# AKASH2907/pi-consistency-activity-detection

Measured on AMD Instinct MI355X. Metric: train clips/sec (bs=8, 16×224×224, I3D+caps+bv cons) at 1/2/4/8 GPU, higher is better.
Workload: dtype f32 (fp32 operands and fp32 accumulation everywhere; 33 of the 79 conv / input-gradient launches and the 3x3x3 / 1x1x1 weight gradients multiply on the bf16 matrix cores: every fp32 operand as the exact sum of 3 bf16 terms, 6 products on v_mfma_f32_32x32x16_bf16, hi / lo fp32 accumulators -- error v

## Files before the change

include/picons.h:

```cpp
#ifndef PICONS_H
#define PICONS_H
#include <stdint.h>
#ifdef __cplusplus
extern "C" {
#endif

typedef void* pc_stream;

#define PC_OK            0
#define PC_E_ARG        -1
#define PC_E_LAUNCH     -2
#define PC_E_NODEVICE   -3

#define PC_ACT_NONE 0
#define PC_ACT_RELU 1
#define PC_ACT_SIGMOID 2

#define PC_F_ACCUM   1
#define PC_F_BIAS    2
#define PC_F_CSCALE  4
#define PC_F_BNPART  8
#define PC_F_NFAST   16
#define PC_F_TOUT    32
#define PC_F_CI3     64

#define PC_F_STRIPS  256
#define PC_F_X6      128

#define PC_VERSION 103
int         pc_version(void);
const char* pc_last_error(void);

typedef struct pc_conv_desc {
    int32_t N;
    int32_t Ti, Hi, Wi, Ci, ldi;
    int32_t Tq, Hq, Wq;
    int32_t To, Ho, Wo, Co, ldo;
    int32_t ostr[3], ooff[3];
    int32_t istr[3], ntap[3], ioff0[3], istep[3];
    int32_t wk0[3], wkstep[3];
    int32_t KT, KH, KW, ldw;
    int32_t act, flags;
    int32_t wgstride, bgstride;
    int32_t act_c0;
    int32_t groups;
} pc_conv_desc;

int pc_conv_fwd(const pc_conv_desc* d, const float* in, const float* w, const float* bias,
                const float* cscale, float* out, float* bnpart, pc_stream s);
int pc_conv_bnpart_rows(const pc_conv_desc* d);

int pc_conv_fwd_x6(const pc_conv_desc* d, const float* in, const uint16_t* wplanes, int64_t plane_stride, const float* bias,
                   const float* cscale, float* out, float* bnpart, pc_stream s);
int64_t pc_conv_x6_ws_floats(const pc_conv_desc* d);
int pc_conv_fwd_x6_ws(const pc_conv_desc* d, const float* in, const uint16_t* wplanes, int64_t plane_stride, const float* bias,
                      const float* cscale, float* out, float* bnpart, float* ws, int64_t ws_floats, pc_stream s);
int pc_conv_x6_ok(const pc_conv_desc* d);
int pc_split_planes(const float* src, uint16_t* planes, int64_t n, int64_t plane_stride, pc_stream s);
typedef struct pc_split_job {
    uint64_t src, planes;
    int64_t  n, plane_stride;
} pc_split_job;
int pc_split_planes_multi(const pc_split_job* jobs, int njobs, pc_stream s);
int pc_conv_work(const pc_conv_desc* d, int ci_real, int co_real, double* out);
int pc_conv_variant(const pc_conv_desc* d, int64_t ws_floats, char* buf, int cap);

typedef struct pc_wino_desc {
    int32_t N, T, H, W;
    int32_t Ci, ldi, Co, ldo;
    int32_t KT;
    int32_t act, flags;
    int32_t Ti;
    int32_t ta, tc, tden;
    int32_t m;
} pc_wino_desc;
int64_t pc_wino_u_floats(int O, int I, int KT);
int pc_wino_weights(const float* w, int64_t sO, int64_t sT, int64_t sI, int O, int I, int KT, int flip, float* U, pc_stream s);
int pc_wino_conv(const pc_wino_desc* d, const float* in, const float* U, const float* bias, float* out, float* bnpart, pc_stream s);
int64_t pc_wino4_u_floats(int O, int I, int KT);
int pc_wino4_weights(const float* w, int64_t sO, int64_t sT, int64_t sI, int O, int I, int KT, int flip, float* U, pc_stream s);
int pc_wino_bnpart_rows(const pc_wino_desc* d);
int pc_wino_work(const pc_wino_desc* d, double* out);
int pc_wino_variant(const pc_wino_desc* d, const float* out, char* buf, int cap);

typedef struct pc_wgrad_desc {
    int32_t N;
    int32_t Tq, Hq, Wq, Cd, ldd;
    int32_t Ts, Hs, Ws, Cs, lds;
    int32_t istr[3], ntap[3], ioff0[3], istep[3];
    int32_t wk0[3];
    int32_t KT, KH, KW;
    int32_t splitk;
    int32_t nbatch;
    int32_t dbstride, sbstride, gbstride;
    int32_t Td, Hd, Wd, doff[3];
    int32_t flags;
    int32_t ws_slices;
} pc_wgrad_desc;
#define PC_WG_CS3    1
#define PC_WG_X6     2
int pc_conv_wgrad(const pc_wgrad_desc* d, const float* D, const float* S, float* g, pc_stream s);
int pc_wgrad_slices(const pc_wgrad_desc* d);
int pc_wgrad_variant(const pc_wgrad_desc* d, char* buf, int cap);
int pc_wgrad_fold_group(void);
int pc_wgrad_fold(float* ws, int64_t image_floats, int nslices, pc_stream s);
int pc_wgrad_work(const pc_wgrad_desc* d, int cd_real, int cs_real, double* out);
int pc_wgrad_uses_x6(const pc_wgrad_desc* d);
typedef struct pc_wgrad_job {
    pc_wgrad_desc d;
    const float* D; const float* S; float* g;
} pc_wgrad_job;
int pc_conv_wgrad_multi(const pc_wgrad_job* jobs, int njobs, pc_stream s);

int pc_bn_finalize(const float* part, int nparts_per_group, int groups, int C, int64_t count_per_group,
                   const float* gamma, const float* beta, float eps, float momentum,
                   float* running_mean, float* running_var, float* stat, pc_stream s);
int64_t pc_bn_finalize_ws_floats(int nparts_per_group, int groups, int C);
int pc_bn_finalize_ws(const float* part, int nparts_per_group, int groups, int C, int64_t count_per_group,
                      const float* gamma, const float* beta, float eps, float momentum,
                      float* running_mean, float* running_var, float* stat, float* ws, pc_stream s);
int pc_bn_apply(const float* z, int ldz, const float* stat, int C, int64_t rows, int groups, float* y,
                int ldy, int relu, pc_stream s);
int pc_bn_finalize_apply_ok(int nparts_per_group, int C);
int pc_bn_finalize_apply(const float* part, int nparts_per_group, int groups, int C, int64_t count_per_group, const float* gamma, const float* beta,
                         float eps, float momentum, float* running_mean, float* running_var, float* stat, const float* z, int ldz, int64_t rows,
                         float* y, int ldy, int relu, pc_stream s);
int pc_bn_eval_stat(const float* gamma, const float* beta, const float* running_mean,
                    const float* running_var, float eps, int C, float* stat, pc_stream s);
int64_t pc_bn_bwd_ws_floats(int64_t rows, int C, int groups);
int pc_bn_bwd(const float* dy, int lddy, const float* z, int ldz, const float* stat, int C,
              int64_t rows, int groups, int relu, float* dz, int lddz, float* dgamma, float* dbeta,
              int accum, float* ws, pc_stream s);

typedef struct pc_pool_desc {
    int32_t N, Ti, Hi, Wi, C, ldi;
    int32_t To, Ho, Wo, ldo;
    int32_t k[3], s[3], padf[3];
} pc_pool_desc;
int pc_maxpool_fwd(const pc_pool_desc* d, const float* x, float* y, uint8_t* argmax, pc_stream s);
int pc_maxpool_bwd(const pc_pool_desc* d, const float* dy, const uint8_t* argmax, float* dx,
                   int accum, pc_stream s);

int pc_channel_scale(const float* x, int ldx, const float* scale, int N, int64_t pos_per_n, int C,
                     float* y, int ldy, int accum, pc_stream s);
int64_t pc_act_bwd_ws_floats(int64_t rows, int C);
int pc_act_bwd(const float* dy, int lddy, const float* y, int ldy, int act, int C, int64_t rows,
               float* dz, int lddz, float* dbias, int accum, float* ws, pc_stream s);
int pc_ncdhw_to_ndhwc(const void* src, int src_is_f64, int N, int C, int64_t thw, int W, int Cpad,
                      int flipw, float* dst, pc_stream s);
int pc_ndhwc_to_ncdhw(const float* src, int ld, int N, int C, int64_t thw, float* dst, pc_stream s);
int pc_transpose_batched(const float* src, int batch, int R, int Cc, int64_t src_batch_stride,
                         int src_ld, float* dst, int64_t dst_batch_stride, int dst_ld, int accum,
                         pc_stream s);
typedef struct pc_transpose_job {
    uint64_t src, dst;
    int64_t  src_batch_stride, dst_batch_stride;
    int32_t  batch, R, C, src_ld, dst_ld, accum;
    int32_t  nslices, reserved;
    int64_t  slice_stride;
} pc_transpose_job;
int pc_transpose_multi(const pc_transpose_job* jobs, int njobs, pc_stream s);
int pc_col2im(const float* cols, int N, int Ho, int Wo, int KH, int KW, int C, float* dx, int lddx,
              int accum, pc_stream s);
// ... 42 lines not shown
                     float* db4, float* dWp, float* dbp, int accum, float* ws, pc_stream s);

typedef struct pc_loss_desc {
    int32_t B, T, H, W;
    int32_t bv, gv, n_frames, predict_maps, jhmdb;
    float   lower_thresh, upper_thresh;
    float   bv_wt, gv_wt, wt_loc, wt_cons, wt_ramp;
} pc_loss_desc;
int64_t pc_loss_ws_floats(const pc_loss_desc* d);
int pc_consistency_loss(const pc_loss_desc* d, const float* output, const float* flip_op,
                        const float* seg, const int32_t* labeled, float* scalars, float* d_output,
                        float* d_flip_op, float* mask_bv, float* mask_gv, float* ws, pc_stream s);
int pc_var_mask(const float* pred, const float* flip_pred, int B, int T, int H, int W, int n_frames,
                int use_sig, float* mask, float* ws, pc_stream s);
int pc_grad_mask(const float* pred, int B, int T, int H, int W, float lower, float upper,
                 float* mask, float* ws, pc_stream s);
int pc_spread_loss(const float* x, const float* cls, const int32_t* labeled, int Bn, int C, float m,
                   float wt, float* out, float* dx, pc_stream s);

int pc_adam_step(float* p, const float* g, float* m, float* v, int64_t n, float lr, float b1,
                 float b2, float eps, int step, float gscale, pc_stream s);

typedef struct pc_axis_desc {
    int32_t R, I, O, C;
    int32_t in_split, out_split, act, act_c0, accum;
    int32_t in_sr, in_hi, in_lo, out_sr, out_hi, out_lo;
} pc_axis_desc;
int pc_axis_linear(const pc_axis_desc* d, const float* in, const float* M, const float* bias, float* out, pc_stream s);
int pc_wspec_fwd(const float* in, const float* tw, int A, int B, int KY, int KX, int U, int Ur, float* out, pc_stream s);
int pc_wspec_bwd(const float* dV, const float* tw, int A, int B, int KY, int KX, int U, int Ur, float* kg, pc_stream s);

int pc_wspec_master_fwd(const float* w, const float* tw, int Acnt, int a0, int Atot, int B, int KY, int KX, int U, int Ur,
                        float* out_f, float* out_t, pc_stream s);
int pc_wspec_master_planes(const float* w, const float* tw, int Acnt, int a0, int Atot, int B, int KY, int KX, int U, int Ur,
                           uint16_t* out_f, uint16_t* out_t, int64_t plane_stride, pc_stream s);
int pc_wspec_master_bwd(const float* dV, const float* tw, int Acnt, int a0, int Atot, int B, int KY, int KX, int U, int Ur,
                        float* dw, int accum, pc_stream s);

int pc_tail6_weights(const float* wf, int N, int Ci, float* W5f, float* W5t, pc_stream s);
int pc_tail6_gather(const float* cols, const float* bc, const float* bsm, int N, int It, int Ih, int Iw, float* out, pc_stream s);
int pc_tail6_scatter(const float* dout, int N, int It, int Ih, int Iw, float* dcols, pc_stream s);
int pc_tail6_wgrad_map(const float* dW5, int N, int Ci, float* Gc, pc_stream s);
int pc_tail6_wgrad_map_slices(float* ws, const int32_t* nslices8, int N, int Ci, float* Gc, pc_stream s);
int pc_tail6_bias_sums(const float* dout, int N, int It, int Ih, int Iw, float* sums, pc_stream s);
int64_t pc_tail6_bias_sums_ws_floats(int N, int It, int Ih, int Iw);
int pc_tail6_bias_sums_ws(const float* dout, int N, int It, int Ih, int Iw, float* sums, float* ws, pc_stream s);

typedef struct pc_op {
    int32_t  kind;
    int32_t  i[48];
    float    f[8];
    int32_t  lane;
    uint64_t p[12];
    int64_t  l[4];
} pc_op;
enum {
    PC_OP_CONV = 1, PC_OP_WGRAD, PC_OP_BN_FINALIZE, PC_OP_BN_APPLY, PC_OP_BN_EVAL_STAT, PC_OP_BN_BWD,
    PC_OP_POOL_FWD, PC_OP_POOL_BWD, PC_OP_CHSCALE, PC_OP_ACT_BWD, PC_OP_TO_NDHWC, PC_OP_TO_NCDHW,
    PC_OP_TRANSPOSE, PC_OP_FILL, PC_OP_AXPY, PC_OP_EM_FWD, PC_OP_EM_BWD, PC_OP_CMASK_FWD,
    PC_OP_CMASK_BWD, PC_OP_TAPSUM_FWD, PC_OP_TAPSUM_BWD, PC_OP_LOSS, PC_OP_SPREAD, PC_OP_ADAM,
    PC_OP_TAIL_COMBINE, PC_OP_TAIL_COLSUM, PC_OP_TAIL_GRADS, PC_OP_COL2IM,
    PC_OP_AXIS,
    PC_OP_WSPEC_FWD,
    PC_OP_WSPEC_BWD,
    PC_OP_WSPEC_MASTER_FWD,
    PC_OP_WSPEC_MASTER_BWD,
    PC_OP_TAIL6_WEIGHTS,
    PC_OP_TAIL6_GATHER,
    PC_OP_TAIL6_SCATTER,
    PC_OP_TAIL6_WGRAD_MAP,
    PC_OP_TAIL6_BIAS_SUMS,
    PC_OP_TRANSPOSE_MULTI,
    PC_OP_FORK,
    PC_OP_JOIN,
    PC_OP_WGRAD_MULTI,
    PC_OP_WINO_CONV,
    PC_OP_WINO_WEIGHTS,
    PC_OP_CONV_X6,
    PC_OP_SPLIT_PLANES,
    PC_OP_SPLIT_PLANES_MULTI,
    PC_OP_WSPEC_MASTER_PLANES,
    PC_OP_BN_FIN_APPLY,
    PC_OP_WGRAD_FOLD,
    PC_OP__COUNT
};
#define PC_MAX_LANES 8
int pc_run_ops(const pc_op* ops, int n, pc_stream s);
int pc_run_ops_lanes(const pc_op* ops, int n, const pc_stream* lanes, int nlanes);
int pc_streams_fanin(pc_stream target, const pc_stream* lanes, int nlanes);
int pc_release_thread_events(void);
int pc_run_ops_timed(const pc_op* ops, int n, int kind, float* ms, int* count, const pc_stream* lanes, int nlanes);
int pc_run_ops_timed_collect(float* ms, int* count);

#ifdef __cplusplus
}
#endif
#endif
```

pi-consistency-activity-detection_amd/capi.py:

```python
import ctypes as C
import os

import numpy as np

_HERE = os.path.dirname(os.path.abspath(__file__))
DIAG = os.environ.get("PICONS_DIAG_LIB", "0") not in ("", "0")
DIAG_SWITCHES = ("PICONS_CONV_ABLATE", "PICONS_WGRAD_ABLATE", "PICONS_WINO_VARIANT")
LIB_PATH = os.path.join(_HERE, "libpicons_diag.so" if DIAG else "libpicons.so")
if os.environ.get("PICONS_LIB_NAME"):
    LIB_PATH = os.path.join(_HERE, os.path.basename(os.environ["PICONS_LIB_NAME"]))
_lib = None

i32, i64, f32, vp = C.c_int32, C.c_int64, C.c_float, C.c_void_p


class ConvDesc(C.Structure):
    _fields_ = [(n, i32) for n in ("N", "Ti", "Hi", "Wi", "Ci", "ldi", "Tq", "Hq", "Wq", "To", "Ho", "Wo", "Co", "ldo")] + \
               [(n, i32 * 3) for n in ("ostr", "ooff", "istr", "ntap", "ioff0", "istep", "wk0", "wkstep")] + \
               [(n, i32) for n in ("KT", "KH", "KW", "ldw", "act", "flags", "wgstride", "bgstride", "act_c0", "groups")]


class WgradDesc(C.Structure):
    _fields_ = [(n, i32) for n in ("N", "Tq", "Hq", "Wq", "Cd", "ldd", "Ts", "Hs", "Ws", "Cs", "lds")] + \
               [(n, i32 * 3) for n in ("istr", "ntap", "ioff0", "istep", "wk0")] + [(n, i32) for n in ("KT", "KH", "KW", "splitk", "nbatch", "dbstride", "sbstride", "gbstride", "Td", "Hd", "Wd")] + [("doff", i32 * 3), ("flags", i32), ("ws_slices", i32)]


AXIS_FIELDS = ["R", "I", "O", "C", "in_split", "out_split", "act", "act_c0", "accum", "in_sr", "in_hi", "in_lo", "out_sr", "out_hi", "out_lo"]


class WinoDesc(C.Structure):
    _fields_ = [(n, i32) for n in ("N", "T", "H", "W", "Ci", "ldi", "Co", "ldo", "KT", "act", "flags", "Ti", "ta", "tc", "tden", "m")]


class AxisDesc(C.Structure):
    _fields_ = [(n, i32) for n in AXIS_FIELDS]


class PoolDesc(C.Structure):
    _fields_ = [(n, i32) for n in ("N", "Ti", "Hi", "Wi", "C", "ldi", "To", "Ho", "Wo", "ldo")] + \
               [(n, i32 * 3) for n in ("k", "s", "padf")]


class LossDesc(C.Structure):
    _fields_ = [(n, i32) for n in ("B", "T", "H", "W", "bv", "gv", "n_frames", "predict_maps", "jhmdb")] + \
               [(n, f32) for n in ("lower_thresh", "upper_thresh", "bv_wt", "gv_wt", "wt_loc", "wt_cons", "wt_ramp")]


OP_DTYPE = np.dtype([("kind", np.int32), ("i", np.int32, 48), ("f", np.float32, 8), ("lane", np.int32),
                     ("p", np.uint64, 12), ("l", np.int64, 4)], align=False)

(OP_CONV, OP_WGRAD, OP_BN_FINALIZE, OP_BN_APPLY, OP_BN_EVAL_STAT, OP_BN_BWD, OP_POOL_FWD, OP_POOL_BWD, OP_CHSCALE,
 OP_ACT_BWD, OP_TO_NDHWC, OP_TO_NCDHW, OP_TRANSPOSE, OP_FILL, OP_AXPY, OP_EM_FWD, OP_EM_BWD, OP_CMASK_FWD, OP_CMASK_BWD,
 OP_TAPSUM_FWD, OP_TAPSUM_BWD, OP_LOSS, OP_SPREAD, OP_ADAM, OP_TAIL_COMBINE, OP_TAIL_COLSUM, OP_TAIL_GRADS, OP_COL2IM,
 OP_AXIS, OP_WSPEC_FWD, OP_WSPEC_BWD, OP_WSPEC_MASTER_FWD, OP_WSPEC_MASTER_BWD, OP_TAIL6_WEIGHTS, OP_TAIL6_GATHER, OP_TAIL6_SCATTER, OP_TAIL6_WGRAD_MAP, OP_TAIL6_BIAS_SUMS,
 OP_TRANSPOSE_MULTI, OP_FORK, OP_JOIN, OP_WGRAD_MULTI, OP_WINO_CONV, OP_WINO_WEIGHTS, OP_CONV_X6, OP_SPLIT_PLANES, OP_SPLIT_PLANES_MULTI, OP_WSPEC_MASTER_PLANES, OP_BN_FIN_APPLY, OP_WGRAD_FOLD) = range(1, 51)
MAX_LANES = 8

WJOB_DTYPE = np.dtype([("d", np.int32, 42), ("D", np.uint64), ("S", np.uint64), ("g", np.uint64)], align=False)

TJOB_DTYPE = np.dtype([("src", np.uint64), ("dst", np.uint64), ("sbs", np.int64), ("dbs", np.int64), ("batch", np.int32), ("R", np.int32),
                       ("C", np.int32), ("sld", np.int32), ("dld", np.int32), ("accum", np.int32), ("nslices", np.int32), ("reserved", np.int32),
                       ("sst", np.int64)], align=False)

SJOB_DTYPE = np.dtype([("src", np.uint64), ("planes", np.uint64), ("n", np.int64), ("pstride", np.int64)], align=False)

ACT_NONE, ACT_RELU, ACT_SIGMOID = 0, 1, 2
F_ACCUM, F_BIAS, F_CSCALE, F_BNPART, F_NFAST, F_TOUT, F_CI3, F_X6, F_STRIPS = 1, 2, 4, 8, 16, 32, 64, 128, 256
WG_CS3, WG_X6 = 1, 2

ABI_VERSION = 103

_SIGS = {
    "pc_version": (i32, []),
    "pc_last_error": (C.c_char_p, []),
    "pc_conv_fwd": (i32, [C.POINTER(ConvDesc), vp, vp, vp, vp, vp, vp, vp]),
    "pc_conv_bnpart_rows": (i32, [C.POINTER(ConvDesc)]),
    "pc_conv_fwd_x6": (i32, [C.POINTER(ConvDesc), vp, vp, i64, vp, vp, vp, vp, vp]),
    "pc_conv_fwd_x6_ws": (i32, [C.POINTER(ConvDesc), vp, vp, i64, vp, vp, vp, vp, vp, i64, vp]),
    "pc_conv_x6_ws_floats": (i64, [C.POINTER(ConvDesc)]),
    "pc_conv_x6_ok": (i32, [C.POINTER(ConvDesc)]),
    "pc_split_planes": (i32, [vp, vp, i64, i64, vp]),
    "pc_split_planes_multi": (i32, [vp, i32, vp]),
    "pc_conv_work": (i32, [C.POINTER(ConvDesc), i32, i32, C.POINTER(C.c_double)]),
    "pc_conv_variant": (i32, [C.POINTER(ConvDesc), i64, C.c_char_p, i32]),
    "pc_wino_variant": (i32, [C.POINTER(WinoDesc), vp, C.c_char_p, i32]),
    "pc_wgrad_variant": (i32, [C.POINTER(WgradDesc), C.c_char_p, i32]),
    "pc_conv_wgrad": (i32, [C.POINTER(WgradDesc), vp, vp, vp, vp]),
    "pc_conv_wgrad_multi": (i32, [vp, i32, vp]),
    "pc_wgrad_slices": (i32, [C.POINTER(WgradDesc)]),
    "pc_wgrad_uses_x6": (i32, [C.POINTER(WgradDesc)]),
    "pc_wgrad_fold_group": (i32, []),
    "pc_wgrad_fold": (i32, [vp, i64, i32, vp]),
    "pc_wgrad_work": (i32, [C.POINTER(WgradDesc), i32, i32, C.POINTER(C.c_double)]),
    "pc_wino_u_floats": (i64, [i32, i32, i32]),
    "pc_wino_weights": (i32, [vp, i64, i64, i64, i32, i32, i32, i32, vp, vp]),
    "pc_wino_conv": (i32, [C.POINTER(WinoDesc), vp, vp, vp, vp, vp, vp]),
    "pc_wino4_u_floats": (i64, [i32, i32, i32]),
    "pc_wino4_weights": (i32, [vp, i64, i64, i64, i32, i32, i32, i32, vp, vp]),
    "pc_wino_bnpart_rows": (i32, [C.POINTER(WinoDesc)]),
    "pc_wino_work": (i32, [C.POINTER(WinoDesc), C.POINTER(C.c_double)]),
    "pc_bn_finalize": (i32, [vp, i32, i32, i32, i64, vp, vp, f32, f32, vp, vp, vp, vp]),
    "pc_bn_finalize_ws": (i32, [vp, i32, i32, i32, i64, vp, vp, f32, f32, vp, vp, vp, vp, vp]),
    "pc_bn_finalize_ws_floats": (i64, [i32, i32, i32]),
    "pc_bn_finalize_apply_ok": (i32, [i32, i32]),
    "pc_bn_finalize_apply": (i32, [vp, i32, i32, i32, i64, vp, vp, f32, f32, vp, vp, vp, vp, i32, i64, vp, i32, i32, vp]),
    "pc_bn_apply": (i32, [vp, i32, vp, i32, i64, i32, vp, i32, i32, vp]),
    "pc_bn_eval_stat": (i32, [vp, vp, vp, vp, f32, i32, vp, vp]),
    "pc_bn_bwd_ws_floats": (i64, [i64, i32, i32]),
    "pc_bn_bwd": (i32, [vp, i32, vp, i32, vp, i32, i64, i32, i32, vp, i32, vp, vp, i32, vp, vp]),
    "pc_maxpool_fwd": (i32, [C.POINTER(PoolDesc), vp, vp, vp, vp]),
    "pc_maxpool_bwd": (i32, [C.POINTER(PoolDesc), vp, vp, vp, i32, vp]),
    "pc_channel_scale": (i32, [vp, i32, vp, i32, i64, i32, vp, i32, i32, vp]),
    "pc_act_bwd_ws_floats": (i64, [i64, i32]),
    "pc_act_bwd": (i32, [vp, i32, vp, i32, i32, i32, i64, vp, i32, vp, i32, vp, vp]),
    "pc_ncdhw_to_ndhwc": (i32, [vp, i32, i32, i32, i64, i32, i32, i32, vp, vp]),
    "pc_ndhwc_to_ncdhw": (i32, [vp, i32, i32, i32, i64, vp, vp]),
    "pc_transpose_batched": (i32, [vp, i32, i32, i32, i64, i32, vp, i64, i32, i32, vp]),
    "pc_col2im": (i32, [vp, i32, i32, i32, i32, i32, i32, vp, i32, i32, vp]),
    "pc_seg_frame_counts": (i32, [vp, vp, i64, i64, vp, vp]),
    "pc_map_accumulate": (i32, [vp, i64, i32, i32, vp, vp, vp, vp, vp]),
    "pc_clip_from_u8": (i32, [vp, i32, i32, i32, C.POINTER(C.c_int32), i32, i32, i32, vp, i32, vp, vp, vp, vp]),
    "pc_clip_from_u8_ndhwc4": (i32, [vp, i32, i32, i32, C.POINTER(C.c_int32), i32, i32, i32, vp, i32, vp, vp, vp, vp]),
    "pc_clip_from_u8_masks": (i32, [vp, i32, i32, i32, C.POINTER(C.c_int32), i32, i32, i32, vp, C.POINTER(C.c_int32), vp, vp, vp, vp, vp]),
    "pc_resize_tables": (i64, [i32, i32, i32, i32, i32, vp, i64]),
    "pc_resize_u8": (i32, [vp, i32, i32, i32, i32, i32, i32, vp, i32, vp, vp]),
    "pc_fill": (i32, [vp, i64, f32, vp]),
    "pc_axpy": (i32, [vp, vp, i64, f32, vp]),
    "pc_em_ws_floats": (i64, [i32, i32, i32]),
    "pc_em_state_floats": (i64, [i32]),
    "pc_em_routing_fwd": (i32, [vp, vp, vp, vp, i32, i32, i32, vp, vp, vp]),
    "pc_em_routing_bwd": (i32, [vp, vp, vp, vp, vp, i32, i32, i32, vp, vp, vp, vp, vp, vp, vp]),
    "pc_class_mask_fwd": (i32, [vp, i32, i32, i32, vp, vp, i32, vp, vp, vp, vp]),
    "pc_class_mask_bwd": (i32, [vp, vp, vp, i32, i32, i32, vp, vp]),
    "pc_tapsum_fwd": (i32, [vp, i32, i32, i32, i32, vp, vp, vp]),
    "pc_tapsum_bwd": (i32, [vp, i32, i32, i32, i32, vp, vp]),
    "pc_loss_ws_floats": (i64, [C.POINTER(LossDesc)]),
    "pc_consistency_loss": (i32, [C.POINTER(LossDesc), vp, vp, vp, vp, vp, vp, vp, vp, vp, vp, vp]),
    "pc_var_mask": (i32, [vp, vp, i32, i32, i32, i32, i32, i32, vp, vp, vp]),
    "pc_grad_mask": (i32, [vp, i32, i32, i32, i32, f32, f32, vp, vp, vp]),
    "pc_spread_loss": (i32, [vp, vp, vp, i32, i32, f32, f32, vp, vp, vp]),
    "pc_adam_step": (i32, [vp, vp, vp, vp, i64, f32, f32, f32, f32, i32, f32, vp]),
    "pc_tail_combine": (i32, [vp, vp, vp, vp, i32, i32, i32, i32, i32, vp, vp, vp, vp]),
    "pc_tail_colsum": (i32, [vp, i32, i64, vp, vp]),
    "pc_tail_grads": (i32, [vp, vp, vp, vp, vp, vp, i32, i32, i32, i32, i32, i32, vp, vp, vp, vp, i32, vp]),
    "pc_tail_grads_ws_floats": (i64, [i32, i32, i32]),
    "pc_tail_grads_ws": (i32, [vp, vp, vp, vp, vp, vp, i32, i32, i32, i32, i32, i32, vp, vp, vp, vp, i32, vp, vp]),
    "pc_axis_linear": (i32, [vp, vp, vp, vp, vp, vp]),
    "pc_wspec_fwd": (i32, [vp, vp, i32, i32, i32, i32, i32, i32, vp, vp]),
    "pc_wspec_bwd": (i32, [vp, vp, i32, i32, i32, i32, i32, i32, vp, vp]),
    "pc_wspec_master_fwd": (i32, [vp, vp, i32, i32, i32, i32, i32, i32, i32, i32, vp, vp, vp]),
    "pc_wspec_master_planes": (i32, [vp, vp, i32, i32, i32, i32, i32, i32, i32, i32, vp, vp, i64, vp]),
    "pc_wspec_master_bwd": (i32, [vp, vp, i32, i32, i32, i32, i32, i32, i32, i32, vp, i32, vp]),
    "pc_tail6_weights": (i32, [vp, i32, i32, vp, vp, vp]),
    "pc_tail6_gather": (i32, [vp, vp, vp, i32, i32, i32, i32, vp, vp]),
    "pc_tail6_scatter": (i32, [vp, i32, i32, i32, i32, vp, vp]),
    "pc_tail6_wgrad_map": (i32, [vp, i32, i32, vp, vp]),
    "pc_tail6_bias_sums": (i32, [vp, i32, i32, i32, i32, vp, vp]),
    "pc_tail6_wgrad_map_slices": (i32, [vp, vp, i32, i32, vp, vp]),
    "pc_tail6_bias_sums_ws_floats": (i64, [i32, i32, i32, i32]),
    "pc_tail6_bias_sums_ws": (i32, [vp, i32, i32, i32, i32, vp, vp, vp]),
    "pc_transpose_multi": (i32, [vp, i32, vp]),
    "pc_run_ops": (i32, [vp, i32, vp]),
    "pc_run_ops_lanes": (i32, [vp, i32, vp, i32]),
    "pc_streams_fanin": (i32, [vp, vp, i32]),
    "pc_release_thread_events": (i32, []),
    "pc_run_ops_timed": (i32, [vp, i32, i32, C.POINTER(f32), C.POINTER(i32), vp, i32]),
    "pc_run_ops_timed_collect": (i32, [C.POINTER(f32), C.POINTER(i32)]),
}
EXPORTS = sorted(_SIGS)


def lib():
    global _lib
    if _lib is None:
        stray = [k for k in DIAG_SWITCHES if os.environ.get(k, "0") not in ("", "0")]
        if stray and not DIAG:
            raise RuntimeError("%s set, but these switches exist only in the diagnostic build of the library (results can be wrong by design): "
                               "`make -C pi-consistency-activity-detection_amd/csrc diag` and PICONS_DIAG_LIB=1, or unset them" % ", ".join(stray))
        if not os.path.exists(LIB_PATH):
            raise RuntimeError("libpicons.so not built (%s): run `python -c 'import __graft_entry__ as g; g.build()'` "
                               "or `make -C pi-consistency-activity-detection_amd/csrc`; there is no CPU fallback" % LIB_PATH)
        L = C.CDLL(LIB_PATH)
        for name, (res, args) in _SIGS.items():
            fn = getattr(L, name)
            fn.restype = res
            fn.argtypes = args
        if L.pc_version() != ABI_VERSION:
            raise RuntimeError("libpicons.so is ABI version %d, this package mirrors include/picons.h version %d: rebuild it "
                               "(`make -C pi-consistency-activity-detection_amd/csrc`)" % (L.pc_version(), ABI_VERSION))
        assert C.sizeof(ConvDesc) == 48 * 4 and OP_DTYPE.itemsize == 4 + 192 + 32 + 4 + 96 + 32
        assert C.sizeof(WgradDesc) == 168 and WJOB_DTYPE.itemsize == 192
        _lib = L
    return _lib


def check(rc):
    if rc != 0:
        raise RuntimeError("libpicons error %d: %s" % (rc, lib().pc_last_error().decode()))


def variant(name, desc, *args):
    buf = C.create_string_buffer(160)
    check(getattr(lib(), name)(desc, *args, buf, 160))
    return buf.value.decode()


def call(name, *args):
    check(getattr(lib(), name)(*args))
```

pi-consistency-activity-detection_amd/csrc/api.hip:

```cpp
#include "common.h"
#include <string.h>
#include <vector>

static thread_local char g_err[512] = "";

void pc_set_error(const char* fmt, ...) {
    va_list ap;
    va_start(ap, fmt);
    vsnprintf(g_err, sizeof(g_err), fmt, ap);
    va_end(ap);
}

extern "C" const char* pc_last_error(void) { return g_err; }
extern "C" int pc_version(void) { return PC_VERSION; }

extern "C" int pc_transpose_batched(const float*, int, int, int, int64_t, int, float*, int64_t, int, int, pc_stream);

#define P(T, k) ((T)(uintptr_t)op.p[k])

static int run_one(const pc_op& op, pc_stream s) {
    switch (op.kind) {
        case PC_OP_CONV: {
            pc_conv_desc d;
            memcpy(&d, op.i, sizeof(d));
// ... 61 lines not shown
            return pc_transpose_batched(P(const float*, 0), op.i[0], op.i[1], op.i[2], op.l[0], op.i[3], P(float*, 1), op.l[1], op.i[4], op.i[5], s);
        case PC_OP_FILL:
            return pc_fill(P(float*, 0), op.l[0], op.f[0], s);
        case PC_OP_AXPY:
            return pc_axpy(P(float*, 0), P(const float*, 1), op.l[0], op.f[0], s);
        case PC_OP_EM_FWD:
            return pc_em_routing_fwd(P(const float*, 0), P(const float*, 1), P(const float*, 2), P(const float*, 3), op.i[0], op.i[1], op.i[2], P(float*, 4), P(float*, 5), s);
        case PC_OP_EM_BWD:
            return pc_em_routing_bwd(P(const float*, 0), P(const float*, 1), P(const float*, 2), P(const float*, 3), P(const float*, 4), op.i[0], op.i[1],
                                     op.i[2], P(float*, 5), P(float*, 6), P(float*, 7), P(float*, 8), P(float*, 9), P(const float*, 10), s);
        case PC_OP_CMASK_FWD:
            return pc_class_mask_fwd(P(const float*, 0), op.i[0], op.i[1], op.i[2], P(const float*, 1), P(const int32_t*, 2), op.i[3], P(float*, 3),
                                     P(float*, 4), P(float*, 5), s);
        case PC_OP_CMASK_BWD:
            return pc_class_mask_bwd(P(const float*, 0), P(const float*, 1), P(const float*, 2), op.i[0], op.i[1], op.i[2], P(float*, 3), s);
        case PC_OP_TAPSUM_FWD:
            return pc_tapsum_fwd(P(const float*, 0), op.i[0], op.i[1], op.i[2], op.i[3], P(const float*, 1), P(float*, 2), s);
        case PC_OP_TAPSUM_BWD:
            return pc_tapsum_bwd(P(const float*, 0), op.i[0], op.i[1], op.i[2], op.i[3], P(float*, 1), s);
        case PC_OP_LOSS: {
            pc_loss_desc d;
            d.B = op.i[0]; d.T = op.i[1]; d.H = op.i[2]; d.W = op.i[3]; d.bv = op.i[4]; d.gv = op.i[5]; d.n_frames = op.i[6];
            d.predict_maps = op.i[7]; d.jhmdb = op.i[8];
            d.lower_thresh = op.f[0]; d.upper_thresh = op.f[1]; d.bv_wt = op.f[2]; d.gv_wt = op.f[3]; d.wt_loc = op.f[4];
            d.wt_cons = op.f[5]; d.wt_ramp = op.f[6];
            return pc_consistency_loss(&d, P(const float*, 0), P(const float*, 1), P(const float*, 2), P(const int32_t*, 3), P(float*, 4), P(float*, 5),
                                       P(float*, 6), P(float*, 7), P(float*, 8), P(float*, 9), s);
        }
        case PC_OP_SPREAD:
            return pc_spread_loss(P(const float*, 0), P(const float*, 1), P(const int32_t*, 2), op.i[0], op.i[1], op.f[0], op.f[1], P(float*, 3), P(float*, 4), s);
        case PC_OP_ADAM:
            return pc_adam_step(P(float*, 0), P(const float*, 1), P(float*, 2), P(float*, 3), op.l[0], op.f[0], op.f[1], op.f[2], op.f[3], op.i[0], op.f[4], s);
        case PC_OP_TAIL_COMBINE:
            return pc_tail_combine(P(const float*, 0), P(const float*, 1), P(const float*, 2), P(const float*, 3), op.i[0], op.i[1], op.i[2], op.i[3],
                                   op.i[4], P(float*, 4), P(float*, 5), P(float*, 6), s);
        case PC_OP_TAIL_COLSUM:
            return pc_tail_colsum(P(const float*, 0), op.i[0], op.l[0], P(float*, 1), s);
        case PC_OP_TAIL_GRADS:
            return pc_tail_grads_ws(P(const float*, 0), P(const float*, 1), P(const float*, 2), P(const float*, 3), P(const float*, 4), P(const float*, 5),
                                    op.i[0], op.i[1], op.i[2], op.i[3], op.i[4], op.i[5], P(float*, 6), P(float*, 7), P(float*, 8), P(float*, 9), op.i[6],
                                    P(float*, 10), s);
        case PC_OP_COL2IM:
            return pc_col2im(P(const float*, 0), op.i[0], op.i[1], op.i[2], op.i[3], op.i[4], op.i[5], P(float*, 1), op.i[6], op.i[7], s);
        case PC_OP_AXIS: {
            pc_axis_desc d;
            memcpy(&d, op.i, sizeof(d));
            return pc_axis_linear(&d, P(const float*, 0), P(const float*, 1), P(const float*, 2), P(float*, 3), s);
        }
        case PC_OP_WSPEC_FWD:
            return pc_wspec_fwd(P(const float*, 0), P(const float*, 1), op.i[0], op.i[1], op.i[2], op.i[3], op.i[4], op.i[5], P(float*, 2), s);
        case PC_OP_WSPEC_BWD:
            return pc_wspec_bwd(P(const float*, 0), P(const float*, 1), op.i[0], op.i[1], op.i[2], op.i[3], op.i[4], op.i[5], P(float*, 2), s);
        case PC_OP_WSPEC_MASTER_FWD:
            return pc_wspec_master_fwd(P(const float*, 0), P(const float*, 1), op.i[0], op.i[1], op.i[2], op.i[3], op.i[4], op.i[5], op.i[6], op.i[7],
                                       P(float*, 2), P(float*, 3), s);
        case PC_OP_WSPEC_MASTER_BWD:
            return pc_wspec_master_bwd(P(const float*, 0), P(const float*, 1), op.i[0], op.i[1], op.i[2], op.i[3], op.i[4], op.i[5], op.i[6], op.i[7],
                                       P(float*, 2), op.i[8], s);
        case PC_OP_TAIL6_WEIGHTS:
            return pc_tail6_weights(P(const float*, 0), op.i[0], op.i[1], P(float*, 1), P(float*, 2), s);
        case PC_OP_TAIL6_GATHER:
            return pc_tail6_gather(P(const float*, 0), P(const float*, 1), P(const float*, 2), op.i[0], op.i[1], op.i[2], op.i[3], P(float*, 3), s);
        case PC_OP_TAIL6_SCATTER:
            return pc_tail6_scatter(P(const float*, 0), op.i[0], op.i[1], op.i[2], op.i[3], P(float*, 1), s);
        case PC_OP_TAIL6_WGRAD_MAP:
            return op.i[2] ? pc_tail6_wgrad_map_slices(P(float*, 0), &op.i[3], op.i[0], op.i[1], P(float*, 1), s)
                           : pc_tail6_wgrad_map(P(const float*, 0), op.i[0], op.i[1], P(float*, 1), s);
        case PC_OP_TAIL6_BIAS_SUMS:
            return pc_tail6_bias_sums_ws(P(const float*, 0), op.i[0], op.i[1], op.i[2], op.i[3], P(float*, 1), P(float*, 2), s);
        case PC_OP_TRANSPOSE_MULTI:
            return pc_transpose_multi(P(const pc_transpose_job*, 0), op.i[0], s);
        case PC_OP_WGRAD_FOLD:
            return pc_wgrad_fold(P(float*, 0), op.l[0], op.i[0], s);
        case PC_OP_WGRAD_MULTI:
            return pc_conv_wgrad_multi(P(const pc_wgrad_job*, 0), op.i[0], s);
        case PC_OP_WINO_CONV: {
            pc_wino_desc d;
            memcpy(&d, op.i, sizeof(d));
            return pc_wino_conv(&d, P(const float*, 0), P(const float*, 1), P(const float*, 2), P(float*, 3), P(float*, 4), s);
        }
        case PC_OP_WINO_WEIGHTS:
            if (op.i[4] == 4) return pc_wino4_weights(P(const float*, 0), op.l[0], op.l[1], op.l[2], op.i[0], op.i[1], op.i[2], op.i[3], P(float*, 1), s);
            return pc_wino_weights(P(const float*, 0), op.l[0], op.l[1], op.l[2], op.i[0], op.i[1], op.i[2], op.i[3], P(float*, 1), s);
        default:
            pc_set_error("pc_run_ops: unknown op kind %d", op.kind);
            return PC_E_ARG;
    }
}

static thread_local hipEvent_t g_ev[PC_MAX_LANES];
static thread_local bool g_ev_init = false;

static thread_local std::vector<hipEvent_t> g_pending;
thread_local hipEvent_t pc_tl_ev_start = nullptr, pc_tl_ev_stop = nullptr;
static thread_local std::vector<hipEvent_t> g_ev_pool;
static hipEvent_t take_event() {
    if (!g_ev_pool.empty()) { hipEvent_t e = g_ev_pool.back(); g_ev_pool.pop_back(); return e; }
    hipEvent_t e = nullptr;
    (void)hipEventCreate(&e);
    return e;
}

static int run_list(const pc_op* ops, int n, const pc_stream* lanes, int nlanes, int kind, float* ms, int* count) {
    if (!ops && n > 0) { pc_set_error("pc_run_ops: null ops"); return PC_E_ARG; }
    if (nlanes < 1 || nlanes > PC_MAX_LANES || !lanes) { pc_set_error("pc_run_ops: nlanes=%d (1..%d)", nlanes, PC_MAX_LANES); return PC_E_ARG; }
    if (nlanes > 1 && !g_ev_init) {
        for (int i = 0; i < PC_MAX_LANES; ++i)
            if (hipEventCreateWithFlags(&g_ev[i], hipEventDisableTiming) != hipSuccess) { pc_set_error("hipEventCreate failed"); return PC_E_LAUNCH; }
        g_ev_init = true;
    }
    int cnt = 0;
    hipEvent_t* ev = nullptr;
    const int sub = kind > 0 ? kind >> 16 : 0;
    if (kind > 0) kind &= 0xffff;
    auto timed_op = [&](const pc_op& op) {
        if (kind <= 0 || op.kind != kind) return false;
        if (!sub || kind != PC_OP_WGRAD) return true;
        pc_wgrad_desc d;
        memcpy(&d, op.i, sizeof(d));
        const bool x6 = pc_wgrad_uses_x6(&d) != 0;
        return sub == 1 ? x6 : !x6;
    };
    if (kind > 0) {
        for (int k = 0; k < n; ++k) cnt += timed_op(ops[k]);
        ev = (hipEvent_t*)malloc(sizeof(hipEvent_t) * 2 * (cnt > 0 ? cnt : 1));
        for (int i = 0; i < 2 * cnt; ++i) ev[i] = take_event();
    }
    int j = 0, rc = PC_OK, k = 0;
    for (; k < n && rc == PC_OK; ++k) {
        const pc_op& op = ops[k];
        if (op.kind == PC_OP_FORK || op.kind == PC_OP_JOIN) {
            if (nlanes == 1) continue;
            const bool fork = op.kind == PC_OP_FORK;
            const int src = (fork && op.i[1] > 0 && op.i[1] < nlanes) ? op.i[1] : 0;
            hipError_t he = hipSuccess;
            if (fork) he = hipEventRecord(g_ev[src], (hipStream_t)lanes[src]);
            for (int q = 0; q < nlanes && he == hipSuccess; ++q) {
                if (!((op.i[0] >> q) & 1) || (fork && q == src) || (!fork && q == 0)) continue;
                if (fork) {
                    he = hipStreamWaitEvent((hipStream_t)lanes[q], g_ev[src], 0);
                } else {
                    he = hipEventRecord(g_ev[q], (hipStream_t)lanes[q]);
                    if (he == hipSuccess) he = hipStreamWaitEvent((hipStream_t)lanes[0], g_ev[q], 0);
                }
            }
            if (he != hipSuccess) { pc_set_error("%s: event record / wait failed: %s", fork ? "FORK" : "JOIN", hipGetErrorString(he)); rc = PC_E_LAUNCH; ++k; break; }
            continue;
        }
        const int ln = (op.lane > 0 && op.lane < nlanes) ? op.lane : 0;
        const pc_stream s = lanes[ln];
        const bool t = timed_op(op);
        const bool ext = t && (op.kind == PC_OP_CONV || op.kind == PC_OP_CONV_X6 || op.kind == PC_OP_WINO_CONV || op.kind == PC_OP_WGRAD);
        if (ext) { pc_tl_ev_start = ev[2 * j]; pc_tl_ev_stop = ev[2 * j + 1]; }
        else if (t) (void)hipEventRecord(ev[2 * j], (hipStream_t)s);
        rc = run_one(op, s);
        if (ext) { pc_tl_ev_start = pc_tl_ev_stop = nullptr; ++j; }
        else if (t) { (void)hipEventRecord(ev[2 * j + 1], (hipStream_t)s); ++j; }
    }
    if (rc != PC_OK) {
        char tmp[400];
        snprintf(tmp, sizeof(tmp), "%s", g_err);
        pc_set_error("op %d (kind %d): %s", k - 1, ops[k - 1].kind, tmp);
    }
    if (kind > 0 && !ms) {
        for (int i = 0; i < 2 * j; ++i) g_pending.push_back(ev[i]);
        for (int i = 2 * j; i < 2 * cnt; ++i) g_ev_pool.push_back(ev[i]);
// ... 73 lines not shown
```

pi-consistency-activity-detection_amd/csrc/conv_x6.hip:

```cpp
#include "conv_common.h"
#include <stdlib.h>
#include <type_traits>
#include <mutex>

namespace {

typedef __attribute__((ext_vector_type(8))) __bf16 bf16x8;
typedef __attribute__((ext_vector_type(4))) uint32_t u32x4;

__device__ __forceinline__ void split2(float x0, float x1, uint32_t& h, uint32_t& m, uint32_t& l) { x6_split2(x0, x1, h, m, l); }

__global__ __launch_bounds__(256) void split_planes_kernel(const float* __restrict__ src, uint16_t* __restrict__ dst, long long n, long long pstride) {
    for (long long i = ((long long)blockIdx.x * 256 + threadIdx.x) * 4; i < n; i += (long long)gridDim.x * 1024) {
        const f32x4 v = *(const f32x4*)(src + i);
        uint32_t h0, m0, l0, h1, m1, l1;
        split2(v[0], v[1], h0, m0, l0);
        split2(v[2], v[3], h1, m1, l1);
        *(uint2*)(dst + i) = make_uint2(h0, h1);
        *(uint2*)(dst + pstride + i) = make_uint2(m0, m1);
        *(uint2*)(dst + 2 * pstride + i) = make_uint2(l0, l1);
    }
}

constexpr int SP_JOBS = 48;
struct SplitJobK { const float* src; uint16_t* dst; long long n, pstride; };
struct SplitPack { SplitJobK j[SP_JOBS]; int first[SP_JOBS + 1]; int n; };
__global__ __launch_bounds__(256) void split_planes_multi_kernel(const SplitPack pk) {
    int k = 0;
    while (k + 1 < pk.n && (int)blockIdx.x >= pk.first[k + 1]) ++k;
    const SplitJobK& J = pk.j[k];
    const long long i = ((long long)(blockIdx.x - pk.first[k]) * 256 + threadIdx.x) * 4;
    if (i >= J.n) return;
    const f32x4 v = *(const f32x4*)(J.src + i);
    uint32_t h0, m0, l0, h1, m1, l1;
    split2(v[0], v[1], h0, m0, l0);
    split2(v[2], v[3], h1, m1, l1);
    *(uint2*)(J.dst + i) = make_uint2(h0, h1);
    *(uint2*)(J.dst + J.pstride + i) = make_uint2(m0, m1);
    *(uint2*)(J.dst + 2 * J.pstride + i) = make_uint2(l0, l1);
}

__device__ __forceinline__ dma_rsrc_t dma_rsrc_h(const uint16_t* base) {
    return __builtin_amdgcn_make_buffer_rsrc((void*)base, 0, (int)0xffffff00u, 0x00020000);
}
__device__ __forceinline__ void glds16h(dma_rsrc_t rs, unsigned voff, uint8_t* l) {
    __builtin_amdgcn_raw_ptr_buffer_load_lds(rs, (__attribute__((address_space(3))) void*)l, 16, voff, 0, 0, 0);
}

struct ConvX6 { ConvK k; const uint16_t* wp; long long wpstride; int full, rem, ksplit; float* ws; unsigned* ctr; int mfast; };

#define PC_MFX6(X, Y, Cc) Cc = __builtin_amdgcn_mfma_f32_32x32x16_bf16(__builtin_bit_cast(bf16x8, X), __builtin_bit_cast(bf16x8, Y), Cc, 0, 0, 0)

template <int BM, int BN, int WM, int WN>
__global__ __launch_bounds__(64 * WM * WN, 1) void conv_x6_kernel(const ConvX6 px) {
    const ConvK& p = px.k;
    constexpr int NW = WM * WN, NT = 64 * NW;
    constexpr int TM = BM / WM / 32, TN = BN / WN / 32, NM = 6 * TM * TN, NU = 4 * TM;
    static_assert(TM >= 1 && TN >= 1 && BM % (WM * 32) == 0 && BN % (WN * 32) == 0, "wave tiles");
    constexpr int APIECES = BM / 8, BPIECES = 3 * BN / 16;
    constexpr int AR = (APIECES + NW - 1) / NW, BR = (BPIECES + NW - 1) / NW;
    static_assert(APIECES % NW == 0, "A pieces per wave");
    constexpr int ABYTES = BM * BK * 4, BPLANE = BN * BK * 2, BBYTES = 3 * BPLANE;
    constexpr int OPBYTES = 2 * (ABYTES + BBYTES);
    constexpr int EH = (BM * BN * 4 <= OPBYTES) ? 1 : 2;
    static_assert(BM * BN * 4 / EH <= OPBYTES, "output tile fits the operand buffers");
    extern __shared__ __attribute__((aligned(16))) uint8_t smem8[];
    uint8_t* As0 = smem8;
    uint8_t* Bs0 = smem8 + 2 * ABYTES;
    int* rinfo = (int*)(smem8 + OPBYTES);
    int* rout = rinfo + BM * 4;
    unsigned* tile_or = (unsigned*)(rout + BM);

    const int tid = threadIdx.x, lane = tid & 63, wave = __builtin_amdgcn_readfirstlane(tid >> 6);
    const int wm = wave / WN, wn = wave % WN;
    int bid, ks = 0, tl = 0;
    const bool split = (int)blockIdx.x >= px.full;
    if (!split) bid = xcd_remap(blockIdx.x, px.full);
    else {
        const int q = xcd_remap((int)blockIdx.x - px.full, px.rem * px.ksplit);
        tl = q / px.ksplit; ks = q % px.ksplit;
        bid = px.full + tl;
    }
    int nt, g, lt;
    if (px.mfast) { lt = bid % p.mtiles_g; const int q = bid / p.mtiles_g; nt = q % p.ntiles; g = q / p.ntiles; }
    else { nt = bid % p.ntiles; const int mtl = bid / p.ntiles; g = mtl / p.mtiles_g; lt = mtl % p.mtiles_g; }
    const int n0 = nt * BN;
    const uint16_t* wbase = px.wp + (size_t)g * p.wgstride;
    const float* bbase = p.bias + (size_t)g * p.bgstride;
    if (tid == 0) *tile_or = 0u;

    for (int r = tid; r < BM; r += NT) {
        const int lm = lt * BM + r;
        int4 info = make_int4(-1, 0, 0, 0);
        int op = -1;
        if (lm < p.Mg) {
            int m = g * p.Mg + lm;
            int n = 0;
            if (p.flags & PC_F_NFAST) { const int ng = p.N / p.groups; n = g * ng + lm % ng; m = lm / ng; }
            const int wq = m % p.Wq; m /= p.Wq;
            const int hq = m % p.Hq; m /= p.Hq;
            const int tq = m % p.Tq;
            if (!(p.flags & PC_F_NFAST)) n = m / p.Tq;
            info = make_int4(n, tq * p.istr[0] + p.ioff0[0], hq * p.istr[1] + p.ioff0[1], wq * p.istr[2] + p.ioff0[2]);
            op = ((n * p.To + tq * p.ostr[0] + p.ooff[0]) * p.Ho + hq * p.ostr[1] + p.ooff[1]) * p.Wo + wq * p.ostr[2] + p.ooff[2];
        }
        ((int4*)rinfo)[r] = info;
        rout[r] = op;
    }
    __syncthreads();

    unsigned adma[AR], amask[AR], bdma[BR];
    const long long apos0 = ((long long)min(p.ioff0[0], 0) * p.Hi + min(p.ioff0[1], 0)) * p.Wi + min(p.ioff0[2], 0);
    const long long abias = -apos0 * p.ldi;
#pragma unroll
    for (int j = 0; j < AR; ++j) {
        const int row = (wave + NW * j) * 8 + (lane >> 3);
        const int4 ri = ((int4*)rinfo)[row];
        const int ks = ((lane & 7) ^ ((row >> 1) & 7)) * 4;
        unsigned m = 0;
        if (ri.x >= 0) {
            for (int a = 0; a < p.ntap[0]; ++a) m |= ((unsigned)(ri.y + a * p.istep[0]) < (unsigned)p.Ti ? 1u : 0u) << a;
            for (int a = 0; a < p.ntap[1]; ++a) m |= ((unsigned)(ri.z + a * p.istep[1]) < (unsigned)p.Hi ? 1u : 0u) << (10 + a);
            for (int a = 0; a < p.ntap[2]; ++a) m |= ((unsigned)(ri.w + a * p.istep[2]) < (unsigned)p.Wi ? 1u : 0u) << (20 + a);
        }
        amask[j] = m;
        const long long pos = ((long long)(ri.x * p.Ti + ri.y) * p.Hi + ri.z) * p.Wi + ri.w;
        adma[j] = (unsigned)(((pos - apos0) * p.ldi + ks) * 4);
    }
#pragma unroll
    for (int j = 0; j < BR; ++j) {
        const int pc = wave + NW * j, pl = pc / (BN / 16), q = pc % (BN / 16);
        const int row = q * 16 + (lane >> 2), co = n0 + row;
        const int sl = (lane & 3) ^ ((row >> 2) & 3);
        bdma[j] = (pc < BPIECES && co < p.Co) ? (unsigned)(((size_t)pl * px.wpstride + (size_t)co * p.wtaps * p.ldw + sl * 8) * 2) : DMA_OOB;
    }
    {
        unsigned mo = 0;
#pragma unroll
        for (int j = 0; j < AR; ++j) mo |= amask[j];
        atomicOr(tile_or, mo);
    }
    __syncthreads();
    const unsigned bo = __builtin_amdgcn_readfirstlane(*tile_or);
    const unsigned bt = bo & 0x3ffu, bh = (bo >> 10) & 0x3ffu, bw = (bo >> 20) & 0x3ffu;
    const bool any_tap = bt && bh && bw;
    const int a_lo = any_tap ? __builtin_ctz(bt) : 0, a_hi = any_tap ? 31 - __builtin_clz(bt) : -1;
    const int b_lo = any_tap ? __builtin_ctz(bh) : 0, b_hi = any_tap ? 31 - __builtin_clz(bh) : -1;
    const int c_lo = any_tap ? __builtin_ctz(bw) : 0, c_hi = any_tap ? 31 - __builtin_clz(bw) : -1;
    const int nb_ = b_hi - b_lo + 1, nc_ = c_hi - c_lo + 1;
    const int nchunks_tile = (a_hi - a_lo + 1) * nb_ * nc_ * (p.Ci / BK);
    struct Walk { int a, b, c, ci; };
    Walk wa = {a_lo, b_lo, c_lo, 0}, wb = wa;
    auto advance = [&](Walk& w) {
        w.ci += BK;
        if (w.ci >= p.Ci) { w.ci = 0; if (++w.c > c_hi) { w.c = c_lo; if (++w.b > b_hi) { w.b = b_lo; ++w.a; } } }
    };
    int nchunks = nchunks_tile;
    if (split) {
        const int c0 = (int)((long long)nchunks_tile * ks / px.ksplit), c1 = (int)((long long)nchunks_tile * (ks + 1) / px.ksplit);
        for (int i = 0; i < c0; ++i) advance(wa);
        wb = wa;
        nchunks = c1 - c0;
    }
    auto fetchA = [&](int buf) {
        const long long da = ((long long)(wa.a * p.istep[0] * p.Hi + wa.b * p.istep[1]) * p.Wi + wa.c * p.istep[2]) * p.ldi + wa.ci;
        const unsigned sel = (1u << wa.a) | (1u << (10 + wa.b)) | (1u << (20 + wa.c));
        const dma_rsrc_t ra = dma_rsrc(p.in + (da - abias));
#pragma unroll
        for (int j = 0; j < AR; ++j) glds16b(ra, ((amask[j] & sel) == sel) ? adma[j] : DMA_OOB, (float*)(As0 + buf * ABYTES + (wave + NW * j) * 1024));
        advance(wa);
    };
    auto fetchB = [&](int buf) {
        const int wtap = ((p.wk0[0] + wb.a * p.wkstep[0]) * p.KH + p.wk0[1] + wb.b * p.wkstep[1]) * p.KW + p.wk0[2] + wb.c * p.wkstep[2];
        const dma_rsrc_t rb = dma_rsrc_h(wbase + (long long)wtap * p.ldw + wb.ci);
#pragma unroll
        for (int j = 0; j < BR; ++j)
            if (BPIECES % NW == 0 || wave + NW * j < BPIECES) glds16h(rb, bdma[j], Bs0 + buf * BBYTES + (wave + NW * j) * 1024);
        advance(wb);
    };

    static_assert(TM == 1 && BM == 32 * WM, "one 32-row tile per wave (every configuration of pc_x6_tile)");
    const bool wave_live = __builtin_amdgcn_readfirstlane(lt * BM + wm * 32 < p.Mg ? 1 : 0) != 0;
    f32x16 acc_hi[TN], acc_lo[TN];
#pragma unroll
    for (int j = 0; j < TN; ++j)
#pragma unroll
        for (int r = 0; r < 16; ++r) { acc_hi[j][r] = 0.f; acc_lo[j][r] = 0.f; }

    const int kh = lane >> 5;
    unsigned abase, bbas[TN];
    {
        const int r = wm * (BM / WM) + (lane & 31);
        abase = (unsigned)(r * BK * 4) + (unsigned)(((kh * 2) ^ ((r >> 1) & 7)) << 4);
    }
#pragma unroll
    for (int j = 0; j < TN; ++j) {
        const int r = wn * (BN / WN) + (lane & 31) + j * 32;
        bbas[j] = (unsigned)(2 * ABYTES) + (unsigned)(r * 64) + (unsigned)((kh ^ ((r >> 2) & 3)) << 4);
    }
    f32x4 raw[2];
    u32x4 pa[2][3], pb[TN][3], pbl[2][3];
    auto rdA = [&](int half, int s, int buf) {
        raw[half] = *(const f32x4*)(smem8 + ((abase ^ (unsigned)(s * 64) ^ (unsigned)(half * 16)) + (unsigned)(buf * ABYTES)));
    };
    auto ldB = [&](int j, int pl, int s, int buf) {
        return *(const u32x4*)(smem8 + ((bbas[j] ^ (unsigned)(s * 32)) + (unsigned)(buf * BBYTES + pl * BPLANE)));
    };
    auto unit = [&](int q, int set) {
        float x0 = raw[q >> 1][(q & 1) * 2], x1 = raw[q >> 1][(q & 1) * 2 + 1];
        asm volatile("" : "+v"(x0), "+v"(x1));
        uint32_t h, m, l;
        split2(x0, x1, h, m, l);
        asm volatile("" : "+v"(h), "+v"(m), "+v"(l));
        pa[set][0][q] = h; pa[set][1][q] = m; pa[set][2][q] = l;
    };
    static_assert(NU == 4, "four split units per step");
    auto phase = [&](auto ph, int t) {
        constexpr int PH = decltype(ph)::value;
        constexpr int s = PH & 1, buf = PH >> 1, cur = PH & 1;
        constexpr int s1 = s ^ 1, b1 = s ? (buf ^ 1) : buf;
        if constexpr (s == 1) {
            PC_SYNC_DMA();
            if ((t + 3) / 2 < nchunks) { fetchA(buf); fetchB(buf); }
        }
        __builtin_amdgcn_sched_barrier(0);
        if (!wave_live) return;
#pragma unroll
        for (int m = 0; m < NM; ++m) {
            const int j = m / 6, pr = m % 6;
            constexpr int PA[6] = {0, 2, 1, 0, 1, 0}, PB[6] = {2, 0, 1, 1, 0, 0};
            if (j == TN - 1) {
                if (pr < 5) PC_MFX6(pa[cur][PA[pr]], pbl[cur][PB[pr]], acc_lo[j]);
                else PC_MFX6(pa[cur][PA[pr]], pbl[cur][PB[pr]], acc_hi[j]);
            } else {
                if (pr < 5) PC_MFX6(pa[cur][PA[pr]], pb[j][PB[pr]], acc_lo[j]);
                else PC_MFX6(pa[cur][PA[pr]], pb[j][PB[pr]], acc_hi[j]);
            }
            if (m < 2) rdA(m, s1, b1);
            if (m >= NM - 3) pbl[cur ^ 1][m - (NM - 3)] = ldB(TN - 1, m - (NM - 3), s1, b1);
            else if (m >= 6 && (m - 6) % 6 < 3 && (m - 6) / 6 < TN - 1) pb[(m - 6) / 6][(m - 6) % 6] = ldB((m - 6) / 6, (m - 6) % 6, s1, b1);
#pragma unroll
            for (int u = 0; u < 4; ++u)
                if (2 + (u * (NM - 2)) / 4 == m) unit(u, cur ^ 1);
            __builtin_amdgcn_sched_barrier(0);
        }
    };
    using P0 = std::integral_constant<int, 0>; using P1 = std::integral_constant<int, 1>;
    using P2 = std::integral_constant<int, 2>; using P3 = std::integral_constant<int, 3>;
    if (nchunks > 0) { fetchA(0); fetchB(0); }
    if (nchunks > 1) { fetchA(1); fetchB(1); }
    PC_SYNC_DMA();
    if (nchunks > 0 && wave_live) {
        rdA(0, 0, 0); rdA(1, 0, 0);
#pragma unroll
        for (int j = 0; j < TN - 1; ++j)
#pragma unroll
            for (int pl = 0; pl < 3; ++pl) pb[j][pl] = ldB(j, pl, 0, 0);
#pragma unroll
        for (int pl = 0; pl < 3; ++pl) pbl[0][pl] = ldB(TN - 1, pl, 0, 0);
#pragma unroll
        for (int u = 0; u < 4; ++u) unit(u, 0);
    }
    const int nph = 2 * nchunks;
    for (int t = 0; t < nph; t += 4) {
        phase(P0{}, t);
        phase(P1{}, t + 1);
        if (t + 2 < nph) {
            phase(P2{}, t + 2);
            phase(P3{}, t + 3);
        }
    }
    f32x16 acc[TM][TN];
#pragma unroll
    for (int j = 0; j < TN; ++j) acc[0][j] = acc_hi[j] + acc_lo[j];
    __syncthreads();
    if (split) {
        const dma_rsrc_t rsw = dma_rsrc(px.ws + (size_t)tl * px.ksplit * (BM * BN));
        const unsigned o_own = (unsigned)((ks * (BM * BN) + wave * (TN * 16 * 64) + lane) * 4);
#pragma unroll
        for (int j = 0; j < TN; ++j)
#pragma unroll
            for (int r = 0; r < 16; ++r) {
                const float v = acc[0][j][r];
                __builtin_amdgcn_raw_buffer_store_b32(__float_as_int(v), rsw, o_own + (unsigned)((j * 16 + r) * 256), 0, 17);
            }
        asm volatile("s_waitcnt vmcnt(0)" ::: "memory");
        __syncthreads();
        if (tid == 0) *tile_or = __hip_atomic_fetch_add(px.ctr + tl, 1u, __ATOMIC_RELAXED, __HIP_MEMORY_SCOPE_AGENT) == (unsigned)(px.ksplit - 1) ? 1u : 0u;
        __syncthreads();
        if (!*tile_or) return;
        const unsigned o_all = (unsigned)((wave * (TN * 16 * 64) + lane) * 4);
#pragma unroll
        for (int j = 0; j < TN; ++j) {
            f32x16 sum;
#pragma unroll
            for (int r = 0; r < 16; ++r) sum[r] = 0.f;
            for (int k = 0; k < px.ksplit; ++k) {
                float t[16];
#pragma unroll
                for (int r = 0; r < 16; ++r)
                    t[r] = __int_as_float(__builtin_amdgcn_raw_buffer_load_b32(rsw, o_all + (unsigned)(k * (BM * BN) * 4 + (j * 16 + r) * 256), 0, 17));
#pragma unroll
                for (int r = 0; r < 16; ++r) sum[r] += t[r];
            }
            acc[0][j] = sum;
        }
        if (tid == 0) __hip_atomic_store(px.ctr + tl, 0u, __ATOMIC_RELAXED, __HIP_MEMORY_SCOPE_AGENT);
        __syncthreads();
    }

    const bool has_bias = p.flags & PC_F_BIAS, has_cs = p.flags & PC_F_CSCALE, accum = p.flags & PC_F_ACCUM;
    if (p.flags & PC_F_BNPART) {
        float* part = p.bnpart + ((size_t)(g * p.mtiles_g + lt) * WM + wm) * 2 * p.Co;
#pragma unroll
        for (int j = 0; j < TN; ++j) {
            float s = 0.f, s2 = 0.f;
#pragma unroll
            for (int i = 0; i < TM; ++i)
#pragma unroll
                for (int r = 0; r < 16; ++r) { const float v = acc[i][j][r]; s += v; s2 += v * v; }
            s += __shfl_xor(s, 32, 64);
            s2 += __shfl_xor(s2, 32, 64);
            const int col = n0 + wn * (BN / WN) + j * 32 + (lane & 31);
            if (lane < 32 && col < p.Co) { part[col] = s; part[p.Co + col] = s2; }
        }
    }
    float* T = (float*)smem8;
    if (p.flags & PC_F_TOUT) { store_tile_cols<BM, BN, WM, WN, TM, TN, NT, EH>(acc, T, rout, rinfo, p, n0, wm, wn, lane, tid); return; }
    if (store_tile_rows<BM, BN, WM, WN, TM, TN, NT, EH>(acc, T, rout, rinfo, p, bbase, n0, wm, wn, lane, tid)) return;
#pragma unroll
    for (int i = 0; i < TM; ++i) {
#pragma unroll
        for (int r = 0; r < 16; ++r) {
            const int row = wm * (BM / WM) + i * 32 + (r & 3) + 8 * (r >> 2) + 4 * (lane >> 5);
            const int op = rout[row];
            if (op < 0) continue;
            const int nb = rinfo[row * 4];
#pragma unroll
            for (int j = 0; j < TN; ++j) {
                const int col = n0 + wn * (BN / WN) + j * 32 + (lane & 31);
                if (col >= p.Co) continue;
                float v = acc[i][j][r];
                if (has_bias) v += bbase[col];
                if (col >= p.act_c0) {
                    if (p.act == PC_ACT_RELU) v = fmaxf(v, 0.f);
                    else if (p.act == PC_ACT_SIGMOID) v = 1.0f / (1.0f + expf(-v));
                }
                if (has_cs) v *= p.cscale[(size_t)nb * p.Co + col];
                float* o = p.out + (size_t)op * p.ldo + col;
                if (accum) v += *o;
                *o = v;
            }
        }
    }
}

inline bool x6_mfast(int mtiles_g, int K, int bn) {
    return mtiles_g <= 8 && mtiles_g > 1 && (long long)K * bn * 6 >= (2ll << 20);
}

template <int BM, int BN, int WM, int WN>
int launch_x6(const ConvX6& kx, hipStream_t s) {
    constexpr int OPBYTES = 2 * (BM * BK * 4 + 3 * BN * BK * 2);
    const size_t lds = (size_t)OPBYTES + (size_t)(BM * 5 + 4) * sizeof(int);
    PC_SET_LDS_ONCE((conv_x6_kernel<BM, BN, WM, WN>), lds, "conv_x6_kernel");
    ConvX6 p = kx;
    p.k.mtiles_g = cdiv(p.k.Mg, BM);
    p.k.ntiles = cdiv(p.k.Co, BN);
    const int tiles = p.k.groups * p.k.mtiles_g * p.k.ntiles;
    if (p.ksplit <= 1 || p.rem <= 0 || !p.ws) { p.full = tiles; p.rem = 0; p.ksplit = 1; }
    p.mfast = x6_mfast(p.k.mtiles_g, p.k.K, BN);
    const dim3 grid(p.full + p.rem * p.ksplit), block(64 * WM * WN);
    if (pc_tl_ev_start) hipExtLaunchKernelGGL((conv_x6_kernel<BM, BN, WM, WN>), grid, block, lds, s, pc_tl_ev_start, pc_tl_ev_stop, 0, p);
    else hipLaunchKernelGGL((conv_x6_kernel<BM, BN, WM, WN>), grid, block, lds, s, p);
    PC_CHECK_LAUNCH("conv_x6_kernel");
    return PC_OK;
}

inline int x6_slots(const X6Tile& t) { return 256 * (t.bm == 256 ? 1 : (t.bm == 64 && t.bn == 64 ? 3 : 2)); }

struct X6Split { int tiles, full, rem, ksplit; long long ws_floats; };
inline X6Split x6_split(const pc_conv_desc* d, int groups, const X6Tile& t) {
    const long long Mg = (long long)(d->N / groups) * d->Tq * d->Hq * d->Wq;
    X6Split r;
    r.tiles = (int)(groups * cdiv(Mg, t.bm) * cdiv(d->Co, t.bn));
    r.full = r.tiles; r.rem = 0; r.ksplit = 1; r.ws_floats = 0;
    const int S = x6_slots(t);
    const int rem = r.tiles % S;
    if (rem == 0 || rem * 10 > S * 6) return r;
    const int chunks = d->ntap[0] * d->ntap[1] * d->ntap[2] * (d->Ci / BK);
    int ks = S / rem;
    if (ks > 8) ks = 8;
    if (ks > chunks / 12) ks = chunks / 12;
    if (ks < 2) return r;
    r.full = r.tiles - rem; r.rem = rem; r.ksplit = ks;
    r.ws_floats = (long long)rem * ks * t.bm * t.bn + ((rem + 3) / 4) * 4;
    return r;
}

inline bool x6_splits(const X6Split& sp, bool have_ws) { return have_ws && sp.ksplit > 1; }

}

X6Tile pc_x6_tile(const pc_conv_desc* d, int groups) {
    const long long Mg = (long long)(d->N / groups) * d->Tq * d->Hq * d->Wq;
    bool rows64 = false;
    if (d->flags & PC_F_NFAST) {
        const long long per_row = (long long)d->Wq * (d->N / groups);
        rows64 = per_row % 128 != 0 && per_row % 64 == 0;
    }
    if (d->Co <= 32 && !rows64) return X6Tile{128, 32, 4, 1};
    struct Cand { X6Tile t; int bpc; double eff; };
    const Cand cand[] = {{{256, 128, 8, 1}, 1, 1.0}, {{128, 64, 4, 1}, 2, 0.9}, {{64, 128, 2, 2}, 2, 0.85}, {{64, 64, 2, 2}, 3, 0.7}};
    double best = 1e300;
    X6Tile bt = cand[3].t;
    for (const Cand& c : cand) {
        if (rows64 && c.t.bm != 64) continue;
        if (c.t.bn == 128 && d->Co <= 64) continue;
        const long long blocks = (long long)groups * cdiv(Mg, c.t.bm) * cdiv(d->Co, c.t.bn);
        const long long per_round = 256ll * c.bpc;
        const long long full = blocks / per_round, rem = blocks % per_round;
        const double t = (double)(full * c.bpc + cdiv(rem, 256)) * c.t.bm * c.t.bn / c.eff;
        if (t < best) { best = t; bt = c.t; }
    }
    return bt;
}

bool pc_x6_eligible(const pc_conv_desc* d) {
    return d && (d->flags & PC_F_X6) && d->Ci % BK == 0 && d->Ci >= BK && d->ldi % 4 == 0 && d->ldw % 8 == 0 && d->ntap[0] >= 1 && d->ntap[0] <= 10 &&
           d->ntap[1] >= 1 && d->ntap[1] <= 10 && d->ntap[2] >= 1 && d->ntap[2] <= 10 && d->N % (d->groups > 0 ? d->groups : 1) == 0;
}

extern "C" int pc_conv_x6_ok(const pc_conv_desc* d) {
    if (!pc_x6_eligible(d)) return 0;
    const int groups = d->groups > 0 ? d->groups : 1;
    const X6Tile t = pc_x6_tile(d, groups);
    const long long Mg = (long long)(d->N / groups) * d->Tq * d->Hq * d->Wq;
    const int chunks = d->ntap[0] * d->ntap[1] * d->ntap[2] * (d->Ci / BK);
    if (chunks < 5 && t.bm != 256) return 0;
    return (long long)groups * cdiv(Mg, t.bm) * cdiv(d->Co, t.bn) >= 150 ? 1 : 0;
}

extern "C" int pc_split_planes(const float* src, uint16_t* planes, int64_t n, int64_t plane_stride, pc_stream s) {
    PC_CHECK_ARG(src && planes && n > 0 && n % 4 == 0 && plane_stride >= n && plane_stride % 4 == 0, "pc_split_planes: n and the plane stride must be multiples of 4 (n=%lld stride=%lld)",
                 (long long)n, (long long)plane_stride);
    PC_CHECK_ARG(((uintptr_t)src % 16 == 0) && ((uintptr_t)planes % 8 == 0), "pc_split_planes: src must be 16-byte, planes 8-byte aligned");
    const long long blocks = (n / 4 + 255) / 256;
    hipLaunchKernelGGL(split_planes_kernel, dim3((unsigned)(blocks < 4096 ? blocks : 4096)), dim3(256), 0, (hipStream_t)s, src, planes, (long long)n, (long long)plane_stride);
    PC_CHECK_LAUNCH("split_planes_kernel");
    return PC_OK;
}

extern "C" int pc_split_planes_multi(const pc_split_job* jobs, int njobs, pc_stream s) {
    PC_CHECK_ARG(jobs && njobs >= 1, "pc_split_planes_multi: bad args");
    for (int j0 = 0; j0 < njobs; j0 += SP_JOBS) {
        SplitPack pk;
        pk.n = njobs - j0 < SP_JOBS ? njobs - j0 : SP_JOBS;
        long long blocks = 0;
        for (int q = 0; q < pk.n; ++q) {
            const pc_split_job& a = jobs[j0 + q];
            PC_CHECK_ARG(a.src && a.planes && a.n > 0 && a.n % 4 == 0 && a.plane_stride >= a.n && a.plane_stride % 4 == 0 && a.src % 16 == 0 && a.planes % 8 == 0,
                         "pc_split_planes_multi: bad job %d (n=%lld stride=%lld)", j0 + q, (long long)a.n, (long long)a.plane_stride);
            pk.j[q].src = (const float*)(uintptr_t)a.src; pk.j[q].dst = (uint16_t*)(uintptr_t)a.planes; pk.j[q].n = a.n; pk.j[q].pstride = a.plane_stride;
            pk.first[q] = (int)blocks;
            blocks += (a.n / 4 + 255) / 256;
            PC_CHECK_ARG(blocks < (1ll << 31), "pc_split_planes_multi: too many elements");
        }
        pk.first[pk.n] = (int)blocks;
        hipLaunchKernelGGL(split_planes_multi_kernel, dim3((unsigned)blocks), dim3(256), 0, (hipStream_t)s, pk);
        PC_CHECK_LAUNCH("split_planes_multi_kernel");
    }
    return PC_OK;
}

extern "C" int64_t pc_conv_x6_ws_floats(const pc_conv_desc* d) {
    if (!pc_x6_eligible(d)) return 0;
    const int groups = d->groups > 0 ? d->groups : 1;
    return x6_split(d, groups, pc_x6_tile(d, groups)).ws_floats;
}

int pc_x6_variant(const pc_conv_desc* d, int64_t ws_floats, char* buf, int cap) {
    PC_CHECK_ARG(pc_x6_eligible(d), "pc_conv_variant: the descriptor does not take the bf16-split kernel (Ci=%d ldi=%d ldw=%d flags=%d)", d->Ci, d->ldi, d->ldw, d->flags);
    const int groups = d->groups > 0 ? d->groups : 1;
    const X6Tile c = pc_x6_tile(d, groups);
    const X6Split sp = x6_split(d, groups, c);
    const bool split = x6_splits(sp, ws_floats > 0);
    PC_CHECK_ARG(!split || ws_floats >= sp.ws_floats, "pc_conv_variant: the workspace holds %lld floats, this launch needs %lld (pc_conv_x6_ws_floats)",
                 (long long)ws_floats, (long long)sp.ws_floats);
    const long long Mg = (long long)(d->N / groups) * d->Tq * d->Hq * d->Wq;
    const bool mfast = x6_mfast((int)cdiv(Mg, c.bm), d->ntap[0] * d->ntap[1] * d->ntap[2] * d->Ci, c.bn);
    const int n = snprintf(buf, (size_t)cap, "x6:%dx%d:w%dx%d:ks%d%s", c.bm, c.bn, c.wm, c.wn, split ? sp.ksplit : 1, mfast ? ":mfast" : "");
    PC_CHECK_ARG(n > 0 && n < cap, "pc_conv_variant: the buffer holds %d bytes", cap);
    return PC_OK;
}

extern "C" int pc_conv_fwd_x6(const pc_conv_desc* d, const float* in, const uint16_t* wplanes, int64_t plane_stride, const float* bias,
                              const float* cscale, float* out, float* bnpart, pc_stream s) {
    return pc_conv_fwd_x6_ws(d, in, wplanes, plane_stride, bias, cscale, out, bnpart, nullptr, 0, s);
}

extern "C" int pc_conv_fwd_x6_ws(const pc_conv_desc* d, const float* in, const uint16_t* wplanes, int64_t plane_stride, const float* bias,
                                 const float* cscale, float* out, float* bnpart, float* ws, int64_t ws_floats, pc_stream s) {
    PC_CHECK_ARG(d && in && wplanes && out, "pc_conv_fwd_x6: null pointer");
    PC_CHECK_ARG(pc_x6_eligible(d), "pc_conv_fwd_x6: the descriptor does not take the bf16-split kernel (PC_F_X6, Ci %% 32 == 0, ldw %% 8 == 0, <= 10 taps per dimension; "
                 "Ci=%d ldi=%d ldw=%d flags=%d)", d->Ci, d->ldi, d->ldw, d->flags);
    const int groups = d->groups > 0 ? d->groups : 1;
    PC_CHECK_ARG(d->N % groups == 0, "pc_conv_fwd_x6: N %% groups");
    PC_CHECK_ARG(!(d->flags & PC_F_BIAS) || bias, "pc_conv_fwd_x6: bias flag without pointer");
    PC_CHECK_ARG(!(d->flags & PC_F_CSCALE) || cscale, "pc_conv_fwd_x6: cscale flag without pointer");
    PC_CHECK_ARG(!(d->flags & PC_F_BNPART) || bnpart, "pc_conv_fwd_x6: bnpart flag without pointer");
    PC_CHECK_ARG(!(d->flags & PC_F_NFAST) || !(d->flags & (PC_F_BNPART | PC_F_CSCALE)), "pc_conv_fwd_x6: NFAST cannot be combined with BN partials / cscale");
    PC_CHECK_ARG(!(d->flags & PC_F_TOUT) || (!(d->flags & (PC_F_BNPART | PC_F_CSCALE | PC_F_BIAS | PC_F_ACCUM | PC_F_NFAST)) && d->act == PC_ACT_NONE),
                 "pc_conv_fwd_x6: channel-major output (PC_F_TOUT) is for plain launches only");
    PC_CHECK_ARG(((uintptr_t)in % 16 == 0) && ((uintptr_t)wplanes % 16 == 0) && plane_stride % 8 == 0 && d->wgstride % 8 == 0,
                 "pc_conv_fwd_x6: in / wplanes must be 16-byte aligned, plane and group strides multiples of 8 elements");
    ConvX6 kx;
    ConvK& k = kx.k;
    kx.wp = wplanes; kx.wpstride = plane_stride;
    k.in = in; k.w = nullptr; k.bias = bias; k.cscale = cscale; k.out = out; k.bnpart = bnpart;
    k.N = d->N; k.Ti = d->Ti; k.Hi = d->Hi; k.Wi = d->Wi; k.Ci = d->Ci; k.ldi = d->ldi;
    k.Tq = d->Tq; k.Hq = d->Hq; k.Wq = d->Wq; k.To = d->To; k.Ho = d->Ho; k.Wo = d->Wo; k.Co = d->Co; k.ldo = d->ldo;
    for (int i = 0; i < 3; ++i) {
        k.ostr[i] = d->ostr[i]; k.ooff[i] = d->ooff[i]; k.istr[i] = d->istr[i]; k.ntap[i] = d->ntap[i];
        k.ioff0[i] = d->ioff0[i]; k.istep[i] = d->istep[i]; k.wk0[i] = d->wk0[i]; k.wkstep[i] = d->wkstep[i];
    }
    k.KH = d->KH; k.KW = d->KW; k.wtaps = d->KT * d->KH * d->KW; k.ldw = d->ldw;
    k.K = d->ntap[0] * d->ntap[1] * d->ntap[2] * d->Ci;
    const int64_t M = (int64_t)d->N * d->Tq * d->Hq * d->Wq;
    PC_CHECK_ARG(M > 0 && M < (1ll << 31) && (int64_t)d->N * d->To * d->Ho * d->Wo < (1ll << 31) && (int64_t)d->N * d->Ti * d->Hi * d->Wi < (1ll << 31), "pc_conv_fwd_x6: position count out of range");
    k.M = (int)M; k.groups = groups; k.Mg = (int)(M / groups);
    k.act = d->act; k.flags = d->flags & ~F_SCALAR_EPI; k.act_c0 = d->act_c0; k.wgstride = d->wgstride; k.bgstride = d->bgstride;
    {
        const long long halo = ((long long)(k.ioff0[0] < 0 ? -k.ioff0[0] : 0) * k.Hi + (k.ioff0[1] < 0 ? -k.ioff0[1] : 0)) * k.Wi + (k.ioff0[2] < 0 ? -k.ioff0[2] : 0);
        const long long in_bytes = ((long long)k.N * k.Ti * k.Hi * k.Wi + 2 * halo) * k.ldi * 4;
        const long long w_bytes = (2 * plane_stride + (long long)k.Co * k.wtaps * k.ldw) * 2;
        PC_CHECK_ARG(in_bytes < DMA_MAX_BYTES && w_bytes < DMA_MAX_BYTES,
                     "pc_conv_fwd_x6: input (%lld B) or weight planes (%lld B per group) exceed the 4 GiB the LDS-DMA gather addresses", in_bytes, w_bytes);
    }
    const X6Tile c = pc_x6_tile(d, groups);
    const X6Split sp = x6_split(d, groups, c);
    kx.full = sp.tiles; kx.rem = 0; kx.ksplit = 1; kx.ws = nullptr; kx.ctr = nullptr;
    if (x6_splits(sp, ws != nullptr)) {
        PC_CHECK_ARG(ws_floats >= sp.ws_floats && (uintptr_t)ws % 16 == 0, "pc_conv_fwd_x6_ws: the workspace holds %lld floats, this launch needs %lld (pc_conv_x6_ws_floats)",
                     (long long)ws_floats, (long long)sp.ws_floats);
        kx.full = sp.full; kx.rem = sp.rem; kx.ksplit = sp.ksplit; kx.ws = ws;
        kx.ctr = (unsigned*)(ws + (long long)sp.rem * sp.ksplit * c.bm * c.bn);
    }
    if (c.bm == 256) return launch_x6<256, 128, 8, 1>(kx, (hipStream_t)s);
    if (c.bm == 128 && c.bn == 64) return launch_x6<128, 64, 4, 1>(kx, (hipStream_t)s);
    if (c.bm == 128 && c.bn == 32) return launch_x6<128, 32, 4, 1>(kx, (hipStream_t)s);
    if (c.bm == 64 && c.bn == 128) return launch_x6<64, 128, 2, 2>(kx, (hipStream_t)s);
    return launch_x6<64, 64, 2, 2>(kx, (hipStream_t)s);
}
```

pi-consistency-activity-detection_amd/csrc/wino.hip:

```cpp
#include "common.h"
#include <stdlib.h>
#include <type_traits>

namespace {

constexpr unsigned DMA_OOB = 0xffffffffu;
typedef __amdgpu_buffer_rsrc_t dma_rsrc_t;
__device__ __forceinline__ dma_rsrc_t dma_rsrc(const float* base) {
    return __builtin_amdgcn_make_buffer_rsrc((void*)base, 0, (int)0xffffff00u, 0x00020000);
}
template <bool ON = true>
__device__ __forceinline__ void glds16b(dma_rsrc_t rs, unsigned voff, float* l) {
    if (ON) __builtin_amdgcn_raw_ptr_buffer_load_lds(rs, (__attribute__((address_space(3))) void*)l, 16, voff, 0, 0, 0);
}

__host__ __device__ inline bool wino_vec_epilogue(int ldo, int Co, uintptr_t out, int scalar_epi) { return !scalar_epi && ldo % 4 == 0 && Co % 4 == 0 && out % 16 == 0; }

struct WinoK {
    const float* in; const float* U; const float* bias; float* out; float* bnpart;
    int N, T, H, W, Ci, ldi, Co, ldo;
    int TH, TW, BTH, BTW, nbh, nbw, nct, nc8;
    int scalar_epi;
    int KT, act, flags;
    int Ti, ta, tc, tden;
    int btw_magic;
    int rpitch, rhalf;
    int strip, nsp;
};

constexpr int WT = 64;
constexpr int WC = 64;
constexpr int WK = 8;
constexpr int PLANE = 16 * 2 * 64 * 4;

__global__ void wino_weights_kernel(const float* __restrict__ w, long long sO, long long sT, long long sI, int O, int I, int KT, int flip,
                                    float* __restrict__ U, int nct, int nc8) {
    const long long e = (long long)blockIdx.x * blockDim.x + threadIdx.x;
    const long long total = (long long)KT * nct * 64 * I;
    if (e >= total) return;
    const int i = (int)(e % I);
    long long r = e / I;
    const int o = (int)(r % (nct * 64));
    const int kt = (int)(r / (nct * 64));
    float g[3][3];
#pragma unroll
    for (int a = 0; a < 3; ++a)
#pragma unroll
        for (int b = 0; b < 3; ++b) {
            const int ks = flip ? KT - 1 - kt : kt, as = flip ? 2 - a : a, bs = flip ? 2 - b : b;
            g[a][b] = o < O ? w[(long long)o * sO + (long long)((ks * 3 + as) * 3 + bs) * sT + (long long)i * sI] : 0.f;
        }
    float t[4][3];
#pragma unroll
    for (int b = 0; b < 3; ++b) {
        t[0][b] = g[0][b];
        t[1][b] = 0.5f * (g[0][b] + g[1][b] + g[2][b]);
        t[2][b] = 0.5f * (g[0][b] - g[1][b] + g[2][b]);
        t[3][b] = g[2][b];
    }
    float* dst = U + ((((long long)kt * nct + o / 64) * nc8 + i / 8) * 16) * (2 * 64 * 4) + ((long long)((i & 7) >> 2) * 64 + (o & 63)) * 4 + (i & 3);
#pragma unroll
    for (int x = 0; x < 4; ++x) {
        const float u0 = t[x][0], u1 = 0.5f * (t[x][0] + t[x][1] + t[x][2]), u2 = 0.5f * (t[x][0] - t[x][1] + t[x][2]), u3 = t[x][2];
        dst[(x * 4 + 0) * (2 * 64 * 4)] = u0;
        dst[(x * 4 + 1) * (2 * 64 * 4)] = u1;
        dst[(x * 4 + 2) * (2 * 64 * 4)] = u2;
        dst[(x * 4 + 3) * (2 * 64 * 4)] = u3;
    }
}

constexpr int RMAX = 12;
constexpr int RPLANE = RMAX * 256;

template <int VAR, bool STRIP = false>
__global__ __launch_bounds__(256, 1) void wino_conv_kernel(const WinoK p) {
    extern __shared__ __attribute__((aligned(16))) float smem[];
    float* Vs = smem;
    float* Us = smem + 2 * PLANE;
    float* Rs = smem + 4 * PLANE;
    const int tid = threadIdx.x, lane = tid & 63;
    const int wave = __builtin_amdgcn_readfirstlane(tid >> 6);
    const int wm = wave >> 1, wn = wave & 1;
    int sb = xcd_remap(blockIdx.x, gridDim.x);
    const int ct = sb % p.nct; sb /= p.nct;
    const int sblock = sb;
    const int bw = sb % p.nbw; sb /= p.nbw;
    int bh = 0, t, n, dn = 0, tia = 0, tib = 0;
    if constexpr (STRIP) {
        const int sp = sb % p.nsp; sb /= p.nsp;
        t = sb % p.T;
        const int ga = 2 * sp, gb = ga + 1, pa = ga >= p.nsp ? 1 : 0, pb = gb >= p.nsp ? 1 : 0;
        n = 2 * (sb / p.T) + pa; dn = pb - pa;
        tia = 2 * (ga - pa * p.nsp); tib = 2 * (gb - pb * p.nsp);
    } else {
        bh = sb % p.nbh; sb /= p.nbh;
        t = sb % p.T; n = sb / p.T;
    }
    const int PW = 2 * p.BTW + 2, PH = STRIP ? 12 : 2 * p.BTH + 2, npos = PH * PW;
    const int h0 = 2 * bh * p.BTH - 1, w0 = 2 * bw * p.BTW - 1;
    const unsigned dn_in = (unsigned)((size_t)dn * p.Ti * p.H * p.W * p.ldi * 4);

    unsigned roff[3];
#pragma unroll
    for (int j = 0; j < 3; ++j) {
        const int q = (wave + 4 * j) * 32 + (lane >> 1);
        const int pr = q / p.rpitch, rem = q - pr * p.rpitch;
        const int odd = rem >= p.rhalf ? 1 : 0, idx = rem - odd * p.rhalf;
        const int pc = 2 * idx + odd;
        const int second = (STRIP && pr >= 6) ? 1 : 0;
        const int h = STRIP ? 2 * (second ? tib : tia) - 1 + (pr - 6 * second) : h0 + pr, w = w0 + pc;
        const bool ok = pr < PH && idx < p.BTW + 1 && (unsigned)h < (unsigned)p.H && (unsigned)w < (unsigned)p.W;
        roff[j] = ok ? (unsigned)(((h * p.W + w) * p.ldi + (lane & 1) * 4) * 4) + (second ? dn_in : 0u) : DMA_OOB;
    }
    const unsigned uoff = lane * 16;

    const int ttile = (wave & 1) * 32 + (lane >> 1), tkh = lane & 1, thalf = wave >> 1;
    const int tli = ttile / p.BTW, tlj = ttile - tli * p.BTW;
    const bool tval = ttile < p.BTH * p.BTW;
    const int rbase = tval ? (((2 * tli + thalf + (STRIP ? 2 * (tli >> 1) : 0)) * p.rpitch + tlj) * 2 + tkh) * 4 : tkh * 4;
    int nkt = 0, ktl0 = 0, ktl1 = 0, ktl2 = 0, ttl0 = 0, ttl1 = 0, ttl2 = 0;
    for (int kt = 0; kt < p.KT; ++kt) {
        const int num = t * p.ta + kt + p.tc;
        if (num < 0 || num % p.tden) continue;
        const int tt = num / p.tden;
        if (tt >= p.Ti) continue;
        if (nkt == 0) { ktl0 = kt; ttl0 = tt; } else if (nkt == 1) { ktl1 = kt; ttl1 = tt; } else { ktl2 = kt; ttl2 = tt; }
        ++nkt;
    }
    const int nchunks = nkt * p.nc8;
    const size_t plane_in = (size_t)p.H * p.W * p.ldi;
    const float* rtap0 = p.in + ((size_t)n * p.Ti + ttl0) * plane_in;
    const float* rtap1 = p.in + ((size_t)n * p.Ti + ttl1) * plane_in;
    const float* rtap2 = p.in + ((size_t)n * p.Ti + ttl2) * plane_in;
    const float* utap0 = p.U + (((size_t)ktl0 * p.nct + ct) * p.nc8) * PLANE + wave * 8 * 256;
    const float* utap1 = p.U + (((size_t)ktl1 * p.nct + ct) * p.nc8) * PLANE + wave * 8 * 256;
    const float* utap2 = p.U + (((size_t)ktl2 * p.nct + ct) * p.nc8) * PLANE + wave * 8 * 256;
    auto advance = [&](int& q, int& c8) {
        const bool wrap = c8 + 1 == p.nc8, last = wrap && q + 1 >= nkt;
        c8 = last ? c8 : (wrap ? 0 : c8 + 1);
        q = (wrap && !last) ? q + 1 : q;
    };
    auto r_base = [&](int q, int c8) -> const float* { return (q == 0 ? rtap0 : (q == 1 ? rtap1 : rtap2)) + c8 * WK; };
    auto u_base = [&](int q, int c8) -> const float* { return (q == 0 ? utap0 : (q == 1 ? utap1 : utap2)) + (size_t)c8 * PLANE; };
    int uq = 0, uc8 = 0, rq = 0, rc8 = 0;

    const float* rnext = nullptr;
    auto issue_r = [&](const float* base, int rb) {
        float* rl = Rs + rb * RPLANE + wave * 256;
        const dma_rsrc_t rs = dma_rsrc(base);
#pragma unroll
        for (int j = 0; j < 3; ++j) glds16b<!(VAR & 1)>(rs, roff[j], rl + j * 4 * 256);
// ... 367 lines not shown
```

pi-consistency-activity-detection_amd/csrc/wino4.hip:

```cpp
#include "common.h"
#include <stdlib.h>
#include <type_traits>

namespace {

constexpr unsigned DMA_OOB = 0xffffffffu;
typedef __amdgpu_buffer_rsrc_t dma_rsrc_t;
__device__ __forceinline__ dma_rsrc_t dma_rsrc(const float* base) {
    return __builtin_amdgcn_make_buffer_rsrc((void*)base, 0, (int)0xffffff00u, 0x00020000);
}
template <bool ON = true>
__device__ __forceinline__ void glds16b(dma_rsrc_t rs, unsigned voff, float* l) {
    if (ON) __builtin_amdgcn_raw_ptr_buffer_load_lds(rs, (__attribute__((address_space(3))) void*)l, 16, voff, 0, 0, 0);
}

typedef float f32x2 __attribute__((ext_vector_type(2)));

template <int N, class F>
__device__ __forceinline__ void static_for(F&& f) {
    if constexpr (N > 0) {
        static_for<N - 1>(f);
        f(std::integral_constant<int, N - 1>{});
    }
}

__host__ __device__ inline bool wino4_vec_epilogue(int ldo, int Co, uintptr_t out) { return ldo % 4 == 0 && Co % 4 == 0 && out % 16 == 0; }

struct Wino4K {
    const float* in; const float* U; const float* bias; float* out; float* bnpart;
    int N, T, H, W, Ci, ldi, Co, ldo;
    int TH, TW, BTH, BTW, nbh, nbw, nct, nc4;
    int KT, act, flags;
    int Ti, ta, tc, tden;
    int btw_magic;
    int rpitch, rq;
};

constexpr float PA = 0.70710678118654752f, PB = 1.41421356237309505f;
constexpr float PA2 = PA * PA, PB2 = PB * PB, PA3 = PA2 * PA, PB3 = PB2 * PB, P0 = PA2 * PB2, PS = PA2 + PB2;
constexpr int XT = 32;
constexpr int XC = 64;
constexpr int XK = 4;
constexpr int VPLANE = 18 * 2 * XT * 4;
constexpr int UPLANE = 18 * 2 * XC * 4;
constexpr int RPIECES = 12;
constexpr int RPLANE = RPIECES * 256;

__global__ void wino4_weights_kernel(const float* __restrict__ w, long long sO, long long sT, long long sI, int O, int I, int KT, int flip,
                                     float* __restrict__ U, int nct, int nc4) {
    const long long e = (long long)blockIdx.x * blockDim.x + threadIdx.x;
    const long long total = (long long)KT * nct * 64 * I;
    if (e >= total) return;
    const int i = (int)(e % I);
    long long r = e / I;
    const int o = (int)(r % (nct * 64));
    const int kt = (int)(r / (nct * 64));
    double g[3][3];
#pragma unroll
    for (int a = 0; a < 3; ++a)
#pragma unroll
        for (int b = 0; b < 3; ++b) {
            const int ks = flip ? KT - 1 - kt : kt, as = flip ? 2 - a : a, bs = flip ? 2 - b : b;
            g[a][b] = o < O ? (double)w[(long long)o * sO + (long long)((ks * 3 + as) * 3 + bs) * sT + (long long)i * sI] : 0.0;
        }
    constexpr double A_ = 0.70710678118654752440, B_ = 1.41421356237309504880, A2 = 0.5, B2 = 2.0;
    constexpr double g0 = 1.0 / (A2 * B2), na = 1.0 / (2.0 * A2 * (A2 - B2)), nb = 1.0 / (2.0 * B2 * (B2 - A2));
    static_assert(PA2 > 0.4999f && PA2 < 0.5001f && PB2 > 1.9999f && PB2 < 2.0001f, "wino4_weights_kernel holds a = 1/sqrt(2), b = sqrt(2) in double");
    double t[6][3];
#pragma unroll
    for (int b = 0; b < 3; ++b) {
        t[0][b] = g0 * g[0][b];
        t[1][b] = na * (g[0][b] + A_ * g[1][b] + A2 * g[2][b]);
        t[2][b] = na * (g[0][b] - A_ * g[1][b] + A2 * g[2][b]);
        t[3][b] = nb * (g[0][b] + B_ * g[1][b] + B2 * g[2][b]);
        t[4][b] = nb * (g[0][b] - B_ * g[1][b] + B2 * g[2][b]);
        t[5][b] = g[2][b];
    }
    const int k = i & 3;
    float* dst = U + (((long long)kt * nct + o / 64) * nc4 + i / 4) * UPLANE + ((long long)(k >> 1) * 64 + (o & 63)) * 4 + (k & 1);
#pragma unroll
    for (int x = 0; x < 6; ++x) {
        double u[6];
        u[0] = g0 * t[x][0];
        u[1] = na * (t[x][0] + A_ * t[x][1] + A2 * t[x][2]);
        u[2] = na * (t[x][0] - A_ * t[x][1] + A2 * t[x][2]);
        u[3] = nb * (t[x][0] + B_ * t[x][1] + B2 * t[x][2]);
        u[4] = nb * (t[x][0] - B_ * t[x][1] + B2 * t[x][2]);
        u[5] = t[x][2];
#pragma unroll
        for (int nu = 0; nu < 6; ++nu) {
            const int P = (nu / 3) * 18 + x * 3 + nu % 3;
            dst[(P >> 1) * (2 * 64 * 4) + (P & 1) * 2] = (float)u[nu];
        }
    }
}

template <int VAR>
__global__ __launch_bounds__(256, 1) void wino4_conv_kernel(const Wino4K p) {
    extern __shared__ __attribute__((aligned(16))) float smem[];
    float* Rs = smem;
    float* Vs = smem + 2 * RPLANE;
    const int tid = threadIdx.x, lane = tid & 63;
    const int wave = __builtin_amdgcn_readfirstlane(tid >> 6);
    const int nh = wave >> 1, wn = wave & 1;
    int sb = xcd_remap(blockIdx.x, gridDim.x);
    const int ct = sb % p.nct; sb /= p.nct;
    const int sblock = sb;
    const int bw = sb % p.nbw; sb /= p.nbw;
    const int bh = sb % p.nbh; sb /= p.nbh;
    const int t = sb % p.T, n = sb / p.T;
    const int PW = 4 * p.BTW + 2, PH = 4 * p.BTH + 2;
    const int h0 = 4 * bh * p.BTH - 1, w0 = 4 * bw * p.BTW - 1;

    unsigned roff[RPIECES];
#pragma unroll
    for (int i = 0; i < RPIECES; ++i) {
        const int q = i * 64 + lane;
        const int pr = q / p.rpitch, rem = q - pr * p.rpitch;
        const int cm = rem / p.rq, idx = rem - cm * p.rq;
        const int pc = 4 * idx + cm;
        const int h = h0 + pr, w = w0 + pc;
        const bool ok = pr < PH && cm < 4 && pc < PW && (unsigned)h < (unsigned)p.H && (unsigned)w < (unsigned)p.W;
        roff[i] = ok ? (unsigned)(((h * p.W + w) * p.ldi) * 4) : DMA_OOB;
    }
    const unsigned uoff = (unsigned)(((nh * 18 + (lane >> 5)) * XC + wn * 32 + (lane & 31)) * 16);

    const int ttile = lane & 31;
    const int xi = wave == 2 ? (lane >> 5) * 5 : 1 + 2 * (wave & 1) + (lane >> 5);
    const int tli = ttile / p.BTW, tlj = ttile - tli * p.BTW;
    const bool tval = ttile < p.BTH * p.BTW;
    int prow[4];
    float ca[4];
    {
        const bool edge = xi == 0 || xi == 5;
        const int r0 = xi == 0 ? 0 : 1, rs = edge ? 2 : 1;
        prow[0] = r0; prow[1] = r0 + rs; prow[2] = r0 + 2 * rs; prow[3] = edge ? r0 + 2 * rs : r0 + 3;
        ca[0] = edge ? P0 : (xi == 1 ? -PA * PB2 : (xi == 2 ? PA * PB2 : (xi == 3 ? -PA2 * PB : PA2 * PB)));
        ca[1] = edge ? -PS : (xi <= 2 ? -PB2 : -PA2);
        ca[2] = edge ? 1.f : (xi == 1 ? PA : (xi == 2 ? -PA : (xi == 3 ? PB : -PB)));
        ca[3] = edge ? 0.f : 1.f;
    }
    int ro[4];
#pragma unroll
    for (int i = 0; i < 4; ++i) ro[i] = tval ? ((4 * tli + prow[i]) * p.rpitch + tlj) * 4 : 0;
    int colo[6];
#pragma unroll
    for (int c = 0; c < 6; ++c) colo[c] = ((c & 3) * p.rq + (c >> 2)) * 4;
    int vo[6];
#pragma unroll
    for (int nu = 0; nu < 6; ++nu) {
        const int P = (nu / 3) * 18 + xi * 3 + nu % 3;
        vo[nu] = ((P >> 1) * 2 * XT + ttile) * 4 + (P & 1) * 2;
    }

    int nkt = 0, ktl0 = 0, ktl1 = 0, ktl2 = 0, ttl0 = 0, ttl1 = 0, ttl2 = 0;
    for (int kt = 0; kt < p.KT; ++kt) {
        const int num = t * p.ta + kt + p.tc;
        if (num < 0 || num % p.tden) continue;
        const int tt = num / p.tden;
        if (tt >= p.Ti) continue;
        if (nkt == 0) { ktl0 = kt; ttl0 = tt; } else if (nkt == 1) { ktl1 = kt; ttl1 = tt; } else { ktl2 = kt; ttl2 = tt; }
        ++nkt;
    }
    const int nchunks = nkt * p.nc4;
    const size_t plane_in = (size_t)p.H * p.W * p.ldi;
    const float* rtap0 = p.in + ((size_t)n * p.Ti + ttl0) * plane_in;
    const float* rtap1 = p.in + ((size_t)n * p.Ti + ttl1) * plane_in;
    const float* rtap2 = p.in + ((size_t)n * p.Ti + ttl2) * plane_in;
    const float* utap0 = p.U + (((size_t)ktl0 * p.nct + ct) * p.nc4) * UPLANE;
    const float* utap1 = p.U + (((size_t)ktl1 * p.nct + ct) * p.nc4) * UPLANE;
    const float* utap2 = p.U + (((size_t)ktl2 * p.nct + ct) * p.nc4) * UPLANE;
    auto advance = [&](int& q, int& c4) {
        const bool wrap = c4 + 1 == p.nc4, last = wrap && q + 1 >= nkt;
        c4 = last ? c4 : (wrap ? 0 : c4 + 1);
        q = (wrap && !last) ? q + 1 : q;
    };
    auto r_base = [&](int q, int c4) -> const float* { return (q == 0 ? rtap0 : (q == 1 ? rtap1 : rtap2)) + c4 * XK; };
// ... 279 lines not shown
        float* part = p.bnpart + ((size_t)sblock * 2 + nh) * 2 * p.Co;
        if (lane < 32 && cval) { part[co] = s1; part[p.Co + co] = s2; }
    }
}

void choose_block(int TH, int TW, int& bth, int& btw) {
    double best = 1e30;
    bth = 4; btw = 8;
    for (int w = 1; w <= XT && w <= TW; ++w) {
        int h = XT / w;
        if (h > TH) h = TH;
        if (h < 1) continue;
        if ((4 * h + 2) * (4 * (w + 1)) > RPIECES * 64) continue;
        const double blocks = (double)cdiv(TH, h) * cdiv(TW, w);
        const double waste = blocks * XT / ((double)TH * TW);
        const double aspect = (double)(4 * w + 2) * (4 * h + 2) / (16.0 * w * h);
        const double cost = waste * (1.0 + 0.05 * aspect);
        if (cost < best - 1e-9) { best = cost; bth = h; btw = w; }
    }
}

void choose_pitch(int bth, int btw, int& rpitch, int& rq) {
    const int PH = 4 * bth + 2;
    rq = btw + 1;
    static const int lanes[2][16] = {{0, 1, 2, 3, 12, 13, 14, 15, 20, 21, 22, 23, 24, 25, 26, 27}, {4, 5, 6, 7, 8, 9, 10, 11, 16, 17, 18, 19, 28, 29, 30, 31}};
    int best = 1 << 30;
    rpitch = 4 * rq;
    for (int pitch = 4 * rq; pitch <= 4 * rq + 15 && PH * pitch <= RPIECES * 64; ++pitch) {
        int cost = 0;
        for (int gset = 0; gset < 2; ++gset) {
            int cnt[16] = {0}, mx = 0;
            for (int q = 0; q < 16; ++q) {
                const int tile = lanes[gset][q];
                if (tile >= bth * btw) continue;
                const int ti = tile / btw, tj = tile - ti * btw;
                const int c = ++cnt[(4 * ti * pitch + tj) & 15];
                mx = c > mx ? c : mx;
            }
            cost += mx > 1 ? mx - 1 : 0;
        }
        if (cost < best) { best = cost; rpitch = pitch; }
    }
}

int fill(const pc_wino_desc* d, Wino4K& k) {
    PC_CHECK_ARG(d, "pc_wino: null descriptor");
    PC_CHECK_ARG(d->N >= 1 && d->T >= 1 && d->H >= 4 && d->W >= 4 && d->H % 4 == 0 && d->W % 4 == 0, "pc_wino (m = 4): H, W must be multiples of 4 (H=%d W=%d)", d->H, d->W);
    PC_CHECK_ARG(d->Ci >= 8 && d->Ci % 8 == 0 && d->ldi % 4 == 0 && d->ldi >= d->Ci && d->Co >= 1 && d->ldo >= d->Co,
                 "pc_wino (m = 4): Ci %% 8, ldi %% 4, ldi >= Ci, ldo >= Co (Ci=%d ldi=%d Co=%d ldo=%d)", d->Ci, d->ldi, d->Co, d->ldo);
    PC_CHECK_ARG(d->KT == 1 || d->KT == 3, "pc_wino: KT must be 1 or 3");
    PC_CHECK_ARG((int64_t)d->N * (d->T > d->Ti ? d->T : d->Ti) * d->H * d->W * (int64_t)(d->ldi > d->ldo ? d->ldi : d->ldo) < (1ll << 40), "pc_wino: tensor too large");
    PC_CHECK_ARG((int64_t)d->H * d->W * d->ldi * 4 < 0xff000000ll, "pc_wino: plane too large (the LDS-DMA lane offsets are 32-bit byte offsets inside one frame)");
    k.N = d->N; k.T = d->T; k.H = d->H; k.W = d->W; k.Ci = d->Ci; k.ldi = d->ldi; k.Co = d->Co; k.ldo = d->ldo;
    k.TH = d->H / 4; k.TW = d->W / 4;
    choose_block(k.TH, k.TW, k.BTH, k.BTW);
    choose_pitch(k.BTH, k.BTW, k.rpitch, k.rq);
    PC_CHECK_ARG((4 * k.BTH + 2) * k.rpitch <= RPIECES * 64, "pc_wino (m = 4): no block rectangle fits H=%d W=%d", d->H, d->W);
    k.nbh = cdiv(k.TH, k.BTH); k.nbw = cdiv(k.TW, k.BTW);
    k.btw_magic = (65536 + k.BTW - 1) / k.BTW;
    k.nct = cdiv(d->Co, XC); k.nc4 = d->Ci / XK;
    k.KT = d->KT; k.act = d->act; k.flags = d->flags;
    PC_CHECK_ARG(d->Ti >= 1 && d->ta >= 1 && d->tden >= 1, "pc_wino: Ti / ta / tden must be >= 1 (Ti=%d ta=%d tden=%d)", d->Ti, d->ta, d->tden);
    k.Ti = d->Ti; k.ta = d->ta; k.tc = d->tc; k.tden = d->tden;
    return PC_OK;
}

}

extern "C" int64_t pc_wino4_u_floats(int O, int I, int KT) {
    if (O < 1 || I < 8 || I % 8 || (KT != 1 && KT != 3)) return -1;
    return (int64_t)KT * cdiv(O, XC) * (I / XK) * UPLANE;
}

extern "C" int pc_wino4_weights(const float* w, int64_t sO, int64_t sT, int64_t sI, int O, int I, int KT, int flip, float* U, pc_stream s) {
    PC_CHECK_ARG(w && U, "pc_wino4_weights: null pointer");
    PC_CHECK_ARG(O >= 1 && I >= 8 && I % 8 == 0 && (KT == 1 || KT == 3), "pc_wino4_weights: O=%d I=%d KT=%d", O, I, KT);
    const int nct = cdiv(O, XC), nc4 = I / XK;
    const long long total = (long long)KT * nct * 64 * I;
    hipLaunchKernelGGL(wino4_weights_kernel, dim3((unsigned)((total + 255) / 256)), dim3(256), 0, (hipStream_t)s, w, (long long)sO, (long long)sT, (long long)sI, O, I, KT, flip, U, nct, nc4);
    PC_CHECK_LAUNCH("wino4_weights_kernel");
    return PC_OK;
}

int pc_wino4_bnpart_rows_impl(const pc_wino_desc* d) {
    Wino4K k;
    if (fill(d, k) != PC_OK) return -1;
    return k.N * k.T * k.nbh * k.nbw * 2;
}

int pc_wino4_work_impl(const pc_wino_desc* d, double* out) {
    Wino4K k;
    const int rc = fill(d, k);
    if (rc != PC_OK) return rc;
    PC_CHECK_ARG(out, "pc_wino_work: null pointer");
    double taps = 0;
    for (int t = 0; t < k.T; ++t)
        for (int a = 0; a < k.KT; ++a) { const int num = t * k.ta + a + k.tc; taps += num >= 0 && num % k.tden == 0 && num / k.tden < k.Ti; }
    const double blocks = (double)k.N * k.nbh * k.nbw * k.nct;
    out[0] = blocks * taps * 36.0 * XT * XC * k.Ci;
    out[1] = (double)k.N * taps * 36.0 * ((double)k.TH * k.TW) * k.Co * k.Ci;
    out[2] = blocks * k.T;
    return PC_OK;
}

int pc_wino4_variant_impl(const pc_wino_desc* d, const float* out, char* buf, int cap) {
    Wino4K k;
    const int rc = fill(d, k);
    if (rc != PC_OK) return rc;
    const int n = snprintf(buf, (size_t)cap, "wino4:%dx%d:%s", k.BTH, k.BTW, wino4_vec_epilogue(k.ldo, k.Co, (uintptr_t)out) ? "vec" : "scalar");
    PC_CHECK_ARG(n > 0 && n < cap, "pc_wino_variant: the buffer holds %d bytes", cap);
    return PC_OK;
}

int pc_wino4_conv_impl(const pc_wino_desc* d, const float* in, const float* U, const float* bias, float* out, float* bnpart, pc_stream s) {
    Wino4K k;
    const int rc = fill(d, k);
    if (rc != PC_OK) return rc;
    PC_CHECK_ARG(in && U && out, "pc_wino_conv: null pointer");
    PC_CHECK_ARG(((uintptr_t)in % 16 == 0) && ((uintptr_t)U % 16 == 0), "pc_wino_conv: in / U must be 16-byte aligned");
    PC_CHECK_ARG(!(d->flags & PC_F_BIAS) || bias, "pc_wino_conv: bias flag without pointer");
    PC_CHECK_ARG(!(d->flags & PC_F_BNPART) || bnpart, "pc_wino_conv: bnpart flag without pointer");
    PC_CHECK_ARG(!(d->flags & ~(PC_F_BIAS | PC_F_ACCUM | PC_F_BNPART)), "pc_wino_conv: unsupported flag");
    PC_CHECK_ARG(d->act == PC_ACT_NONE || d->act == PC_ACT_RELU, "pc_wino_conv: activation");
    k.in = in; k.U = U; k.bias = bias; k.out = out; k.bnpart = bnpart;
#ifdef PICONS_DIAG
    static const int var = getenv("PICONS_WINO_VARIANT") ? atoi(getenv("PICONS_WINO_VARIANT")) : 0;
    PC_CHECK_ARG(var != 32 || bnpart, "pc_wino_conv: variant 32 writes its stamps through bnpart");
#endif
    const size_t lds = (size_t)(16 * XT * XC) * sizeof(float);
    static_assert(2 * RPLANE + 2 * VPLANE <= 16 * XT * XC, "the operand images must fit the staging image");
    const dim3 grid((unsigned)((int64_t)k.N * k.T * k.nbh * k.nbw * k.nct));
#define WINO_LAUNCH(V)                                                                                                            \
    {                                                                                                                             \
        PC_SET_LDS_ONCE(wino4_conv_kernel<V>, lds, "wino4_conv_kernel");                                                          \
        if (pc_tl_ev_start) hipExtLaunchKernelGGL(wino4_conv_kernel<V>, grid, dim3(256), lds, (hipStream_t)s, pc_tl_ev_start, pc_tl_ev_stop, 0, k); \
        else hipLaunchKernelGGL(wino4_conv_kernel<V>, grid, dim3(256), lds, (hipStream_t)s, k);                                  \
    }
#ifdef PICONS_DIAG
    switch (var) {
        case 1: WINO_LAUNCH(1) break;
        case 2: WINO_LAUNCH(2) break;
        case 3: WINO_LAUNCH(3) break;
        case 4: WINO_LAUNCH(4) break;
        case 7: WINO_LAUNCH(7) break;
        case 8: WINO_LAUNCH(8) break;
        case 15: WINO_LAUNCH(15) break;
        case 32: WINO_LAUNCH(32) break;
        case 64: WINO_LAUNCH(64) break;
        default: WINO_LAUNCH(0) break;
    }
#else
    WINO_LAUNCH(0)
#endif
#undef WINO_LAUNCH
    PC_CHECK_LAUNCH("wino4_conv_kernel");
    return PC_OK;
}
```

pi-consistency-activity-detection_amd/ops.py:

```python
import ctypes as C

import numpy as np
import torch

from . import capi, desc as D


def stream():
    return C.c_void_p(torch.cuda.current_stream().cuda_stream)


def ptr(t):
    if t is None:
        return None
    if not t.is_cuda:
        raise RuntimeError("picons ops need CUDA/HIP tensors (no CPU fallback)")
    return C.c_void_p(t.data_ptr())


def _fill_struct(st, d):
    for name, ctype in st._fields_:
        v = d[name]
        if isinstance(v, (list, tuple)):
            setattr(st, name, (C.c_int32 * 3)(*[int(x) for x in v]))
        else:
            setattr(st, name, ctype(v))
    return st


def conv_desc(d):
    return _fill_struct(capi.ConvDesc(), d)


def conv_bnpart_rows(d):
    return capi.lib().pc_conv_bnpart_rows(C.byref(conv_desc(d)))


def conv_fwd(d, x, w, out, bias=None, cscale=None, bnpart=None):
    capi.call("pc_conv_fwd", C.byref(conv_desc(d)), ptr(x), ptr(w), ptr(bias), ptr(cscale), ptr(out), ptr(bnpart), stream())
    return out


def split_planes(w):
    n = w.numel()
    planes = torch.empty(3, n, device=w.device, dtype=torch.int16)
    capi.call("pc_split_planes", ptr(w), ptr(planes), n, n, stream())
    return planes


def conv_x6_ws_floats(d):
    dd = dict(d)
    dd["flags"] = int(dd.get("flags", 0)) | capi.F_X6
    return int(capi.lib().pc_conv_x6_ws_floats(C.byref(conv_desc(dd))))


def conv_fwd_x6(d, x, wplanes, out, bias=None, cscale=None, bnpart=None, ws=None):
    dd = dict(d)
    dd["flags"] = int(dd.get("flags", 0)) | capi.F_X6
    if ws is None:
        capi.call("pc_conv_fwd_x6", C.byref(conv_desc(dd)), ptr(x), ptr(wplanes), wplanes.shape[1], ptr(bias), ptr(cscale), ptr(out), ptr(bnpart), stream())
    else:
        capi.call("pc_conv_fwd_x6_ws", C.byref(conv_desc(dd)), ptr(x), ptr(wplanes), wplanes.shape[1], ptr(bias), ptr(cscale), ptr(out), ptr(bnpart),
                  ptr(ws), ws.numel(), stream())
    return out


def wino_desc(N, T, H, W, Ci, ldi, Co, ldo, KT=3, act=0, flags=0, Ti=None, ta=1, tc=None, tden=1, m=2):
    st = capi.WinoDesc()
    st.m = m
    st.N, st.T, st.H, st.W, st.Ci, st.ldi, st.Co, st.ldo, st.KT, st.act, st.flags = N, T, H, W, Ci, ldi, Co, ldo, KT, act, flags
    st.Ti, st.ta, st.tc, st.tden = (T if Ti is None else Ti), ta, (-(KT // 2) if tc is None else tc), tden
    return st


def wino_weights(w, O, I, KT=3, flip=False, strides=None, out=None, m=2):
    sO, sT, sI = strides if strides is not None else (I * KT * 9, 1, KT * 9)
    fam = "pc_wino4" if m == 4 else "pc_wino"
    n = getattr(capi.lib(), fam + "_u_floats")(O, I, KT)
    U = out if out is not None else torch.empty(n, device=w.device, dtype=torch.float32)
    capi.call(fam + "_weights", ptr(w), int(sO), int(sT), int(sI), O, I, KT, int(flip), ptr(U), stream())
    return U


def wino_conv(d, x, U, out, bias=None, bnpart=None):
    capi.call("pc_wino_conv", C.byref(d), ptr(x), ptr(U), ptr(bias), ptr(out), ptr(bnpart), stream())
    return out


def conv_wgrad(d, Dt, St, g):
    capi.call("pc_conv_wgrad", C.byref(_fill_struct(capi.WgradDesc(), d)), ptr(Dt), ptr(St), ptr(g), stream())
    return g


def wgrad_slices(d):
    n = capi.lib().pc_wgrad_slices(C.byref(_fill_struct(capi.WgradDesc(), dict(d, ws_slices=0))))
    if n < 1:
        raise RuntimeError("pc_wgrad_slices: %s" % capi.lib().pc_last_error().decode())
    return int(n)


def conv_wgrad_ordered(d, Dt, St, ws=None):
    n = wgrad_slices(d)
    taps = d["KT"] * d["KH"] * d["KW"]
    image = d["gbstride"] * d["nbatch"] if d.get("nbatch", 0) > 1 else d["Cd"] * taps * d["Cs"]
    if ws is None:
        ws = torch.zeros(n * image, device=Dt.device, dtype=torch.float32)
    conv_wgrad(dict(d, ws_slices=n), Dt, St, ws)
    g = ws.view(n, image)[0].clone()
    for k in range(1, n):
        g += ws.view(n, image)[k]
    return g, ws


def wgrad_fold(ws, image_floats, nslices):
    capi.call("pc_wgrad_fold", ptr(ws), int(image_floats), int(nslices), stream())
    return ws


def wgrad_job_table(jobs):
    tab = np.zeros(len(jobs), dtype=capi.WJOB_DTYPE)
    for q, (d, Dp, Sp, gp) in enumerate(jobs):
        tab[q]["d"][:] = D.flatten(d, D.WGRAD_FIELDS)
        tab[q]["D"], tab[q]["S"], tab[q]["g"] = Dp, Sp, gp
    return tab


def conv_wgrad_multi(jobs):
    tab = wgrad_job_table([(d, Dt.data_ptr(), St.data_ptr(), g.data_ptr()) for d, Dt, St, g in jobs])
    for _d, Dt, St, g in jobs:
        ptr(Dt); ptr(St); ptr(g)
    capi.call("pc_conv_wgrad_multi", C.c_void_p(tab.ctypes.data), len(jobs), stream())


def bn_finalize(part, npg, groups, C_, count, gamma, beta, eps, momentum, rmean=None, rvar=None, two_stage=False):
    stat = torch.empty(groups, 4, C_, device=part.device, dtype=torch.float32)
    if two_stage:
        n = capi.lib().pc_bn_finalize_ws_floats(npg, groups, C_)
        ws = torch.empty(max(int(n), 1), device=part.device, dtype=torch.float32)
        capi.call("pc_bn_finalize_ws", ptr(part), npg, groups, C_, int(count), ptr(gamma), ptr(beta), eps, momentum, ptr(rmean), ptr(rvar),
                  ptr(stat), ptr(ws) if n > 0 else None, stream())
    else:
        capi.call("pc_bn_finalize", ptr(part), npg, groups, C_, int(count), ptr(gamma), ptr(beta), eps, momentum, ptr(rmean), ptr(rvar),
                  ptr(stat), stream())
    return stat


def bn_finalize_apply(part, npg, groups, C_, count, gamma, beta, eps, momentum, rmean, rvar, z, ldz, rows, y, ldy, relu=True):
    stat = torch.empty(groups, 4, C_, device=part.device, dtype=torch.float32)
    capi.call("pc_bn_finalize_apply", ptr(part), npg, groups, C_, int(count), ptr(gamma), ptr(beta), eps, momentum, ptr(rmean), ptr(rvar), ptr(stat),
              ptr(z), ldz, int(rows), ptr(y), ldy, int(relu), stream())
    return stat


def bn_apply(z, ldz, stat, C_, rows, groups, y, ldy, relu=True):
    capi.call("pc_bn_apply", ptr(z), ldz, ptr(stat), C_, int(rows), groups, ptr(y), ldy, int(relu), stream())
    return y


def bn_eval_stat(gamma, beta, rm, rv, eps):
    stat = torch.empty(1, 4, gamma.numel(), device=gamma.device, dtype=torch.float32)
    capi.call("pc_bn_eval_stat", ptr(gamma), ptr(beta), ptr(rm), ptr(rv), eps, gamma.numel(), ptr(stat), stream())
    return stat


# ... 323 lines not shown
```

pi-consistency-activity-detection_amd/plan.py:

```python
from dataclasses import dataclass, field

import os

import numpy as np

from . import capi, desc as D, spec, spectral, switches as sw, tail6

ALIGN = 256


@dataclass
class TR:
    ref: tuple
    N: int
    thw: tuple
    C: int
    ld: int
    name: str = ""

    @property
    def rows(self):
        return self.N * self.thw[0] * self.thw[1] * self.thw[2]

    def slice(self, c0, c):
# ... 814 lines not shown
            dxpl = self.alloc(SL.G * SL.x_g)
            self.alg_dgrad(SL.flops())
            self.conv_op(SL.dgrad(), dtpl, w["wvt"], dxpl, alg=0)
            self.emit(capi.OP_AXIS, i=D.flatten(SL.planes_to_dx(dx.ld, acc), capi.AXIS_FIELDS), p=[dxpl, sm["Ft"], None, dx.ref])
        self.tape.append(bwd)

    def build_forward(self):
        N, hw, C = self.N, self.hw, self.C
        self.cur = "fwd"
        T = spec.FRAMES
        self.in_data = self.alloc(self.n * 3 * T * hw * hw)
        self.in_aug = self.alloc(self.n * 3 * T * hw * hw)
        self.in_cls = self.alloc(N)
        self.in_labeled = self.alloc(N)
        self.in_drop832 = self.alloc(N * spec.TRUNK_OUT_CH)
        self.in_drop128 = self.alloc(N * 128)
        x = self.tensor(N, (T, hw, hw), 4, "img")
        self.img = x
        self.op_to_ndhwc = []
        for g in range(self.groups):
            self.op_to_ndhwc.append(len(self.lists["fwd"]))
            src = self.in_data if g == 0 else self.in_aug
            self.emit(capi.OP_TO_NDHWC, i=[0, self.n, 3, hw, 4, 0], l=[T * hw * hw], p=[src, off(x.ref, g * self.n * T * hw * hw * 4)])
        out56 = out112 = None
        first = True
        s28e = hw // 8
        if self.skip_lane:
            cat56 = self.tensor(N, (2, 2 * s28e, 2 * s28e), 128, "cat56")
            cat112 = self.tensor(N, (4, 4 * s28e, 4 * s28e), 128, "cat112")
        pending_skip, skip_after = [], sw.exp("PICONS_SKIP_FWD_AFTER", "", self.exp)
        for ent in spec.TRUNK:
            name = "conv1." + ent[0]
            if ent[0] == "Mixed_3b" and self.late_prep:
                self.join(1 << self.wg_lane)
            if ent[1] == "conv":
                x = self.unit3d(name, x, ent[3], ent[4], ent[5], need_dx=not first)
                first = False
            elif ent[1] == "pool":
                x = self.maxpool(x, ent[2], ent[3], name)
            else:
                x = self.inception(name, x, ent[3])
            if ent[0] == "Conv3d_2c_3x3":
                out56 = x
                if self.skip_lane:
                    pending_skip.append(("conv56", out56, cat56))
            if ent[0] == "Conv3d_1a_7x7":
                out112 = x
                if self.skip_lane:
                    pending_skip.append(("conv112", out112, cat112))
            if pending_skip and (not skip_after or ent[0] == skip_after or ent is spec.TRUNK[-1]):
                for nm_, t_, c_ in pending_skip:
                    self._skip_conv(nm_, t_, c_)
                pending_skip = []
            if ent[0] == "MaxPool3d_3a_3x3" and self.skip_lane:
                inner = self.tape.pop()
                self.tape.append(lambda inner=inner: (self.join(1 << self.skip_lane), inner()))
        self.named["trunk_out"] = x
        s28 = x.thw[1]
        if self.training:
            xd = self.tensor(N, x.thw, x.C, "x832d")
            self.emit(capi.OP_CHSCALE, i=[x.ld, N, x.C, xd.ld, 0], l=[x.rows // N], p=[x.ref, self.in_drop832, xd.ref])
            xin = x

            def bwd_drop():
                dxd = self.grad_of(xd)
                dx, acc = self.grad_for_write(xin)
                self.emit(capi.OP_CHSCALE, i=[dxd.ld, N, xin.C, dx.ld, int(acc)], l=[xin.rows // N], p=[dxd.ref, self.in_drop832, dx.ref])
            self.tape.append(bwd_drop)
        else:
            xd = x
        cat28 = self.tensor(N, (1, s28, s28), 128, "cat28")
        conv28_early = bool(self.conv28_aside and self.skip_lane)
        if conv28_early:
            self.fork(1 << self.skip_lane)
            self.lane = self.skip_lane
            self.conv_layer("conv28", xd, 64, (1, 3, 3), (0, 1, 1), capi.ACT_RELU, cat28.slice(64, 64))
            self.lane = 0
            self.skip_bwd["conv28"] = self.tape.pop()
        KP = spec.PRIMARY_K
        s20 = s28 - KP + 1
        npose = spec.IN_CAPS * spec.POSE
        caps_in = self.tensor(N, (1, s20, s20), npose + spec.IN_CAPS, "caps_in")
        spectral_pc = self.spectral_pc and xd.thw[0] == 1
        Cpc = npose + spec.IN_CAPS
        pc_names = [("primary_caps.pose.weight", 0, npose), ("primary_caps.a.weight", npose, spec.IN_CAPS)]
        if spectral_pc:
            SL = spectral.Layout(N, xd.thw[1], xd.thw[2], xd.C, xd.ld, Cpc, caps_in.ld, KP, KP)
            sm = {k: self.const(v) for k, v in spectral.matrices(xd.thw[2], KP).items()}
            pl = self.next_prep_lane()
            nW = SL.G * SL.w_g
            x6_pc = self.x6 and sw.get("PICONS_SPLIT_SPECTRAL", "1") != "0" and all(capi.lib().pc_conv_x6_ok(_cdesc(dict(D.trim_conv(dd), flags=dd["flags"] | capi.F_X6))) for dd in [SL.conv()] + SL.dgrad())
            if x6_pc:
                wpc = dict(wv=("V", 0), wvt=("V", 4 * nW))
                pf, pt = self.alloc((3 * nW + 1) // 2), self.alloc((3 * nW + 1) // 2)
                self.wbufs.append(dict(ref=wpc["wv"], n=nW, lst=None, lane=None, planes=pf))
                self.wbufs.append(dict(ref=wpc["wvt"], n=nW, lst=None, lane=None, planes=pt))
                for nm, a0, cnt in pc_names:
                    self.emit(capi.OP_WSPEC_MASTER_PLANES, i=[cnt, a0, Cpc, xd.C, KP, KP, SL.nu, SL.Ur], l=[nW], p=[self.P(nm), sm["tw"], pf, pt],
                              lst=self.prep_target, lane=pl)
            else:
                wpc = dict(wv=self.alloc(nW),
                           wvt=self.alloc(nW))
                for nm, a0, cnt in pc_names:
                    self.emit(capi.OP_WSPEC_MASTER_FWD, i=[cnt, a0, Cpc, xd.C, KP, KP, SL.nu, SL.Ur], p=[self.P(nm), sm["tw"], wpc["wv"], wpc["wvt"]],
                              lst=self.prep_target, lane=pl)
        else:
            wpc = self.prep_conv_weight([nm for nm, _a, _c in pc_names], [cnt for _n, _a, cnt in pc_names], xd.C, (1, KP, KP), True)
            wpc["tio"] = self.alloc(KP * KP * xd.C * Cpc)
            self.emit(capi.OP_TRANSPOSE, i=[1, Cpc, KP * KP * xd.C, KP * KP * xd.C, Cpc, 0], l=[0, 0],
                      p=[wpc["fwd"], wpc["tio"]], lst=self.prep_target)
        pc_bias = self.alloc(npose + spec.IN_CAPS)
        self.emit(capi.OP_TRANSPOSE, i=[1, 1, npose, npose, 1, 0], l=[0, 0], p=[self.P("primary_caps.pose.bias"), pc_bias], lst=self.prep_target)
        self.emit(capi.OP_TRANSPOSE, i=[1, 1, spec.IN_CAPS, spec.IN_CAPS, 1, 0], l=[0, 0], p=[self.P("primary_caps.a.bias"), off(pc_bias, npose)], lst=self.prep_target)
        pc_dbias = self.alloc(npose + spec.IN_CAPS)
        if spectral_pc:
            xpl = self.alloc(SL.G * SL.x_g)
            tpl = self.alloc(SL.G * SL.t_g)
            self.emit(capi.OP_AXIS, i=D.flatten(SL.x_to_planes(), capi.AXIS_FIELDS), p=[xd.ref, sm["F"], None, xpl])
            self.conv_op(SL.conv(), xpl, wpc["wv"], tpl)
            self.emit(capi.OP_AXIS, i=D.flatten(SL.planes_to_y(capi.ACT_SIGMOID, npose), capi.AXIS_FIELDS), p=[tpl, sm["G"], pc_bias, caps_in.ref])
        else:
            self.conv_bias_act("", xd, Cpc, (1, KP, KP), (0, 0, 0), capi.ACT_SIGMOID, caps_in, act_c0=npose,
                               bias_ref=pc_bias, wkey="primary_caps.pose.weight")
        npos = N * s20 * s20
        comb = self.tensor(N, (1, s20, s20), C * 17, "comb")
        Wc, bu, ba = self.P("conv_caps.weights"), self.P("conv_caps.beta_u"), self.P("conv_caps.beta_a")
        em_state = self.alloc(capi.lib().pc_em_state_floats(int(npos))) if self.training else None
        self.emit(capi.OP_EM_FWD, i=[npos, spec.IN_CAPS, C], p=[caps_in.ref, Wc, bu, ba, comb.ref, em_state])
        self.pred = self.alloc(N * C)
        cmask = self.alloc(N * C)
        masked = self.tensor(N, (1, s20, s20), C * 16, "masked")
        self.op_cmask = len(self.lists["fwd"])
        self.emit(capi.OP_CMASK_FWD, i=[N, s20 * s20, C, 0 if self.training else 2], p=[comb.ref, self.in_cls, self.in_labeled, self.pred, cmask, masked.ref])

        def bwd_caps():
            dmasked = self.grad_of(masked)
            dcomb = self.tensor(N, (1, s20, s20), C * 17, "d_comb")
            self.emit(capi.OP_CMASK_BWD, i=[N, s20 * s20, C], p=[dmasked.ref, self.dpred, cmask, dcomb.ref])
            dcaps = self.tensor(N, (1, s20, s20), npose + spec.IN_CAPS, "d_caps_in")
            ws = self.alloc(_em_ws(npos, spec.IN_CAPS, C))
            for nm in ("conv_caps.weights", "conv_caps.beta_u", "conv_caps.beta_a"):
                if not self.acc:
                    self.emit(capi.OP_FILL, p=[self.G(nm)], l=[int(np.prod(self.pshape[nm]))], f=[0.0])
            self.emit(capi.OP_EM_BWD, i=[npos, spec.IN_CAPS, C],
                      p=[caps_in.ref, Wc, bu, ba, dcomb.ref, dcaps.ref, self.G("conv_caps.weights"), self.G("conv_caps.beta_u"), self.G("conv_caps.beta_a"), ws, em_state])
            self.release_deferred()
            ws2 = self.alloc(_act_bwd_ws(caps_in.rows, npose))
            a_sl, da_sl = caps_in.slice(npose, spec.IN_CAPS), dcaps.slice(npose, spec.IN_CAPS)
            self.emit(capi.OP_ACT_BWD, i=[dcaps.ld, caps_in.ld, capi.ACT_SIGMOID, spec.IN_CAPS, dcaps.ld, self.acc], l=[caps_in.rows],
                      p=[da_sl.ref, a_sl.ref, da_sl.ref, self.G("primary_caps.a.bias"), ws2])
            self.emit(capi.OP_ACT_BWD, i=[dcaps.ld, caps_in.ld, capi.ACT_NONE, npose, dcaps.ld, self.acc], l=[caps_in.rows],
                      p=[dcaps.ref, caps_in.ref, None, self.G("primary_caps.pose.bias"), ws2])
            if spectral_pc:
                dtpl = self.alloc(SL.G * SL.t_g)
                dwv = self.alloc(SL.G * SL.w_g)
                self.emit(capi.OP_AXIS, i=D.flatten(SL.dy_to_planes(dcaps.ld), capi.AXIS_FIELDS), p=[dcaps.ref, sm["Gt"], None, dtpl])
                def pc_wgrad():
                    self.wgrad_op(SL.wgrad(), [dtpl, xpl, dwv])
                    for nm, a0, cnt in pc_names:
                        self.emit(capi.OP_WSPEC_MASTER_BWD, i=[cnt, a0, Cpc, xd.C, KP, KP, SL.nu, SL.Ur, self.acc], p=[dwv, sm["tw"], self.G(nm)])
                    self.mark_final(*[nm for nm, _a, _c in pc_names])
                self.on_wgrad_lane(pc_wgrad)
            else:
                self.wgrad_op(D.trim_wgrad(D.wgrad(N, caps_in.thw, caps_in.C, dcaps.ld, xd.thw, xd.C, xd.ld, (1, KP, KP), (1, 1, 1), (0, 0, 0))),
                              [dcaps.ref, xd.ref, wpc["kg"]], wpc)
            if not spectral_pc:
                self.flush_grad(wpc)
            self.mark_final("conv_caps.weights", "conv_caps.beta_u", "conv_caps.beta_a", "primary_caps.pose.bias", "primary_caps.a.bias")
            dx, acc = self.grad_for_write(xd)
            F_pc = 2 * caps_in.rows * caps_in.C * xd.C * KP * KP
            if spectral_pc:
                dxpl = self.alloc(SL.G * SL.x_g)
                self.alg_dgrad(SL.flops())
                for dd in SL.dgrad():
                    self.conv_op(dd, dtpl, wpc["wvt"], dxpl, alg=0)
                self.emit(capi.OP_AXIS, i=D.flatten(SL.planes_to_dx(dx.ld, acc), capi.AXIS_FIELDS), p=[dxpl, sm["Ft"], None, dx.ref])
            elif xd.thw[0] == 1 and caps_in.thw[1] + KP - 1 == xd.thw[1]:
                cols = self.alloc(caps_in.rows * KP * KP * xd.C)
                dg = D.conv_fwd(N, caps_in.thw, caps_in.C, dcaps.ld, KP * KP * xd.C, KP * KP * xd.C, (1, 1, 1), (1, 1, 1), (0, 0, 0),
                                caps_in.thw, ldw=caps_in.C)
                self.conv_op(dg, dcaps.ref, wpc["tio"], cols, alg=F_pc)
                self.emit(capi.OP_COL2IM, i=[N, caps_in.thw[1], caps_in.thw[2], KP, KP, xd.C, dx.ld, int(acc)], p=[cols, dx.ref])
            else:
                self.alg_dgrad(F_pc)
                for dd in D.transposed_classes(N, caps_in.thw, caps_in.C, dcaps.ld, xd.thw, xd.C, dx.ld, (1, KP, KP), (1, 1, 1), (0, 0, 0),
                                               flags=(capi.F_ACCUM if acc else 0) | capi.F_NFAST, ldw=caps_in.C):
                    self.conv_op(dd, dcaps.ref, wpc["tr"], dx.ref, alg=0)
        self.tape.append(bwd_caps)
        self.convT_layer("upsample1", masked, 64, (1, KP, KP), (1, 1, 1), (0, 0, 0), (0, 0, 0), capi.ACT_RELU, cat28.slice(0, 64))
        if conv28_early:
            self.tape.append(self.skip_bwd["conv28"])
            self.join(1 << self.skip_lane)
        else:
            self.conv_layer("conv28", xd, 64, (1, 3, 3), (0, 1, 1), capi.ACT_RELU, cat28.slice(64, 64))
        if not self.skip_lane:
            cat56 = self.tensor(N, (2, 2 * s28, 2 * s28), 128, "cat56")
        self.convT_layer("upsample2", cat28, 64, (3, 3, 3), (2, 2, 2), (1, 1, 1), (1, 1, 1), capi.ACT_RELU, cat56.slice(0, 64))
        if self.skip_lane:
            self.tape.append(self._on_skip_lane(self.skip_bwd["conv56"]))
            self.join(1 << self.skip_lane)
        else:
            self.conv_layer("conv56", out56, 64, (3, 3, 3), (1, 1, 1), capi.ACT_RELU, cat56.slice(64, 64))
            cat112 = self.tensor(N, (4, 4 * s28, 4 * s28), 128, "cat112")
        self.convT_layer("upsample3", cat56, 64, (3, 3, 3), (2, 2, 2), (1, 1, 1), (1, 1, 1), capi.ACT_RELU, cat112.slice(0, 64))
        if self.skip_lane:
            self.tape.append(self._on_skip_lane(self.skip_bwd["conv112"]))
        else:
            self.conv_layer("conv112", out112, 64, (3, 3, 3), (1, 1, 1), capi.ACT_RELU, cat112.slice(64, 64))
        othw = (8, 8 * s28, 8 * s28)
        k3, s2, p1 = (3, 3, 3), (2, 2, 2), (1, 1, 1)
        J = 27
        wt = self.alloc(N * 128 * 27 * 32)
        wf = self.alloc(N * 32 * 27 * 128)
        bc = self.alloc(N * 32)
        cs_ref = self.in_drop128 if self.training else None
        W4, b4, Wp = self.P("upsample4.weight"), self.P("upsample4.bias"), self.P("smooth.weight")
        self.emit(capi.OP_TAIL_COMBINE, i=[N, 128, 128, 27, J], p=[W4, b4, cs_ref, Wp, wt, wf, bc])
        if self.merged_tail:
            return self._merged_tail(cat112, othw, wf, bc, cs_ref, W4, b4, Wp, J)
        proj = self.tensor(N, othw, 32, "proj")
        F_tail = 0
        for dd in D.transposed_classes(N, cat112.thw, 128, cat112.ld, othw, 32, 32, k3, s2, p1, flags=capi.F_BIAS, groups=N):
            dd["wgstride"] = 32 * 27 * 128
            dd["bgstride"] = 32
            dd["Co_real"] = J
            F_tail += _conv_flops(dd)
            self.conv_op(dd, cat112.ref, wf, proj.ref, bias=bc)
        out = self.tensor(N, othw, 1, "out")
        self.emit(capi.OP_TAPSUM_FWD, i=[N, othw[0], othw[1], othw[2]], p=[proj.ref, self.P("smooth.bias"), out.ref])
        self.out = out

        def bwd_smooth():
            dproj = self.tensor(N, othw, 32, "d_proj")
            self.emit(capi.OP_TAPSUM_BWD, i=[N, othw[0], othw[1], othw[2]], p=[self.dout, dproj.ref])
            sums = self.alloc(N * 32)
            per_n = othw[0] * othw[1] * othw[2]
            self.emit(capi.OP_TAIL_COLSUM, i=[N], l=[per_n], p=[dproj.ref, sums])
            Gc = self.alloc(N * 128 * 27 * 32)
            self.emit(capi.OP_FILL, p=[Gc], l=[N * 128 * 27 * 32], f=[0.0])
            xin_per = cat112.thw[0] * cat112.thw[1] * cat112.thw[2] * cat112.ld
            wd = D.trim_wgrad(D.wgrad(1, cat112.thw, 128, cat112.ld, othw, 32, 32, k3, s2, p1))
            wd.update(nbatch=N, dbstride=xin_per, sbstride=per_n * 32, gbstride=128 * 27 * 32, Cs_real=J)
            self.wgrad_op(wd, [cat112.ref, dproj.ref, Gc])
            self.emit(capi.OP_TAIL_GRADS, i=[N, 128, 128, 27, J, 13, self.acc],
                      p=[Gc, sums, W4, b4, cs_ref, Wp, self.G("upsample4.weight"), self.G("upsample4.bias"), self.G("smooth.weight"), self.G("smooth.bias")])
            self.mark_final("upsample4.weight", "upsample4.bias", "smooth.weight", "smooth.bias")
            dx, acc = self.grad_for_write(cat112)
            dd = D.conv_fwd(N, othw, 32, 32, 128, dx.ld, k3, s2, p1, cat112.thw, flags=capi.F_ACCUM if acc else 0, groups=N, ldw=32)
            dd["wgstride"] = 128 * 27 * 32
            dd["Ci_real"] = J
            self.conv_op(dd, dproj.ref, wt, dx.ref, alg=F_tail)
        self.tape.append(bwd_smooth)
        return out

    def _merged_tail(self, cat112, othw, wf, bc, cs_ref, W4, b4, Wp, J):
        N = cat112.N
        It, Ih, Iw = cat112.thw
# ... 190 lines not shown
            if j is None:
                raise RuntimeError("gradient of %s is finalised on lane %d and never joined" % (nm, lane))
            return j
        buckets, cur_end, cur_ready, cur_size = [], self.nparams, 0, 0
        for nm in reversed(names):
            cur_ready = max(cur_ready, ready_of(nm))
            cur_size = cur_end - self.poff[nm]
            if cur_size >= target_floats:
                buckets.append((cur_ready, self.poff[nm], cur_end))
                cur_end, cur_ready = self.poff[nm], 0
        if cur_end > 0:
            buckets.append((max(cur_ready, max(ready_of(nm) for nm in names) if cur_ready == 0 else cur_ready), 0, cur_end))
        buckets.sort(key=lambda b: b[0])
        return buckets

    def build_adam(self):
        self.op_adam = 0
        self.emit(capi.OP_ADAM, i=[1], f=[1e-4, 0.9, 0.999, 1e-6, 1.0], l=[self.nparams], p=[("P", 0), ("G", 0), ("M", 0), ("V", 0)], lst="adam")

    def finalize(self):
        lst = self.lists["prep"]
        if self.lanes > 1 and lst and lst[0][0] != capi.OP_FORK:
            first = lambda op: op[0] == capi.OP_FILL or op[3][0][0] == "P"
            lvl0 = [op for op in lst if first(op)]
            lvl1 = [op[:5] + (0,) for op in lst if not first(op)]
            mask = [(1 << self.lanes) - 2]
            lst[:] = [(capi.OP_FORK, mask, [], [], [], 0)] + lvl0 + [(capi.OP_JOIN, mask, [], [], [], 0)] + lvl1
        late = self.lists["prep_late"]
        if late and late[0][0] != capi.OP_FORK:
            mine = set()
            for nm in ("conv56.weight", "conv112.weight"):
                if nm in self.kw:
                    mine |= {self.kw[nm].get("fwd"), self.kw[nm].get("tr"), self.kw[nm].get("wino_fwd"), self.kw[nm].get("wino_tr")}
            mine.discard(None)
            lane_of = lambda op: self.skip_lane if (self.skip_lane and any(r in mine for r in op[3] if r is not None)) else self.wg_lane
            late[:] = [(capi.OP_FORK, [(1 << self.wg_lane | 1 << self.skip_lane) & ~1, 0], [], [], [], 0)] + [op[:5] + (lane_of(op),) for op in late]

    def resolve(self, bases):
        self.finalize()
        out = {}
        keep = out["_tjobs"] = []
        for name, lst in self.lists.items():
            if name in ("prep", "prep_late"):
                lst = self._merge_prep_transposes(lst, bases, keep)
            arr = np.zeros(len(lst), dtype=capi.OP_DTYPE)
            for j, (kind, i, f, p, l, lane) in enumerate(lst):
                arr[j]["kind"] = kind
                arr[j]["lane"] = lane
                arr[j]["i"][:len(i)] = i
                arr[j]["f"][:len(f)] = f
                arr[j]["l"][:len(l)] = l
                for q, r in enumerate(p):
                    if r is not None and r[0] == "JOBS":
                        tab = self._job_table(self.multi_jobs[r[1]], bases)
                        keep.append(tab)
                        r = ("HOST", tab.ctypes.data)
                    if r is not None and r[0] == "SJOBS":
                        tab = np.zeros(len(r[1]), dtype=capi.SJOB_DTYPE)
                        for w, (src, dst, n_, ps) in enumerate(r[1]):
                            tab[w] = (bases[src[0]] + src[1], bases[dst[0]] + dst[1], n_, ps)
                        keep.append(tab)
                        r = ("HOST", tab.ctypes.data)
                    if r is not None and r[0] == "WJOBS":
                        tab = np.zeros(len(self.wjobs[r[1]]), dtype=capi.WJOB_DTYPE)
                        for w, (wd, wp) in enumerate(self.wjobs[r[1]]):
                            tab[w]["d"][:] = D.flatten(wd, D.WGRAD_FIELDS)
                            tab[w]["D"], tab[w]["S"], tab[w]["g"] = [bases[x[0]] + x[1] for x in wp]
                        keep.append(tab)
                        r = ("HOST", tab.ctypes.data)
                    arr[j]["p"][q] = 0 if r is None else (r[1] if r[0] == "HOST" else bases[r[0]] + r[1])
            out[name] = arr
        return out

    @staticmethod
    def _job_table(jobs, bases):
        tab = np.zeros(len(jobs), dtype=capi.TJOB_DTYPE)
        for q, op in enumerate(jobs):
            _kind, i, _f, p, l = op[:5]
            ns, sst = (i[6], l[2]) if len(i) > 6 else (0, 0)
            tab[q] = (bases[p[0][0]] + p[0][1], bases[p[1][0]] + p[1][1], l[0], l[1], i[0], i[1], i[2], i[3], i[4], i[5], ns, 0, sst)
        return tab

    def _merge_prep_transposes(self, lst, bases, keep):
        res, pending, splits = [], {}, {}

        def flush():
            for lane in sorted(pending):
                jobs = pending[lane]
                tab = self._job_table(jobs, bases)
                keep.append(tab)
                res.append((capi.OP_TRANSPOSE_MULTI, [len(jobs)], [], [("HOST", tab.ctypes.data)], [], lane))
            pending.clear()
            for lane in sorted(splits):
                res.append((capi.OP_SPLIT_PLANES_MULTI, [len(splits[lane])], [], [("SJOBS", splits[lane])], [], lane))
            splits.clear()
        for op in lst:
            if op[0] == capi.OP_SPLIT_PLANES:
                splits.setdefault(op[5], []).append((op[3][0], op[3][1], op[4][0], op[4][1]))
            elif op[0] == capi.OP_TRANSPOSE and op[3][0][0] == "P":
                pending.setdefault(op[5], []).append(op)
            elif op[0] in (capi.OP_FILL, capi.OP_FORK, capi.OP_WSPEC_MASTER_FWD, capi.OP_WSPEC_MASTER_PLANES, capi.OP_WINO_WEIGHTS):
                res.append(op)
            else:
                flush()
                res.append(op)
        flush()
        return res

    def conv_flops_executed(self):
        return {name: {k: self.work.get((name, k), 0) for k in ("mfma", "executed", "valid")} for name in self.lists}

    def x6_flops_executed(self):
        return {name: {k: self.work.get((name, "x6_" + k), 0) for k in ("mfma", "executed", "valid")} for name in self.lists}

    def wgrad_flops_executed(self):
        return {name: {k: self.work.get((name, "wg_" + k), 0) for k in ("mfma", "executed", "valid")} for name in self.lists}

    def wgrad_flops_by_family(self):
        return tuple({k: sum(self.work.get((name, pre + k), 0) for name in self.lists) for k in ("mfma", "executed", "valid")} for pre in ("wgx6_", "wgf32_"))

    def flops(self, only_kind=None):
        kinds = (capi.OP_CONV, capi.OP_WGRAD) if only_kind is None else (only_kind,)
        return {name: sum(self.issued.get((name, k), 0) for k in kinds) for name in self.lists}

    def flops_reference_counted(self):
        return {name: self.alg_flops.get(name, 0) for name in self.lists}

    def flops_reference_counted_wino(self):
        return {name: self.alg_flops_wino.get(name, 0) for name in self.lists}


def _conv_flops(d):
    return 2 * d["N"] * d["Tq"] * d["Hq"] * d["Wq"] * d.get("Co_real", d["Co"]) * d.get("Ci_real", d["Ci"]) * d["ntap"][0] * d["ntap"][1] * d["ntap"][2]


def conv_work(d):
    import ctypes as C
    out = (C.c_double * 7)()
    capi.check(capi.lib().pc_conv_work(_cdesc(d), int(d.get("Ci_real", 0)), int(d.get("Co_real", 0)), out))
    return dict(issued=out[0], executed=out[1], valid=out[2], blocks=int(out[3]), bm=int(out[4]), bn=int(out[5]), glds=bool(out[6]))


def _wdesc(d):
    import ctypes as C
    st = capi.WgradDesc()
    for name, ctype in st._fields_:
        v = d.get(name, 0)
        setattr(st, name, (C.c_int32 * 3)(*[int(x) for x in v]) if isinstance(v, (list, tuple)) else ctype(v))
    return C.byref(st)


def wgrad_work(d):
    import ctypes as C
    out = (C.c_double * 5)()
    capi.check(capi.lib().pc_wgrad_work(_wdesc(d), int(d.get("Cd_real", 0)), int(d.get("Cs_real", 0)), out))
    return dict(issued=out[0], executed=out[1], valid=out[2], route=int(out[3]), launches=int(out[4]))


def _wgrad_flops(d):
    return (2 * d["N"] * d["Tq"] * d["Hq"] * d["Wq"] * d.get("Cd_real", d["Cd"]) * d.get("Cs_real", d["Cs"]) * d["ntap"][0] * d["ntap"][1] * d["ntap"][2]
            * max(1, d.get("nbatch", 0)))


def _bnpart_rows(d):
    return capi.lib().pc_conv_bnpart_rows(_cdesc(d))


def _cdesc(d):
    import ctypes as C
    st = capi.ConvDesc()
    for name, ctype in st._fields_:
        v = d[name]
        setattr(st, name, (C.c_int32 * 3)(*[int(x) for x in v]) if isinstance(v, (list, tuple)) else ctype(v))
    return C.byref(st)


def _bn_bwd_ws(rows, C_, groups):
    return capi.lib().pc_bn_bwd_ws_floats(int(rows), int(C_), int(groups))


def _act_bwd_ws(rows, C_):
    return capi.lib().pc_act_bwd_ws_floats(int(rows), int(C_))

# ... 11 lines not shown
```

pi-consistency-activity-detection_amd/spectral.py:

```python
import numpy as np

from . import capi, desc as D


def n_freq(P):
    return P // 2 + 1


def dft_matrix(P):
    u = np.arange(n_freq(P), dtype=np.float64)[:, None]
    x = np.arange(P, dtype=np.float64)[None, :]
    th = 2.0 * np.pi * u * x / P
    F = np.empty((2 * n_freq(P), P), dtype=np.float64)
    F[0::2] = np.cos(th)
    F[1::2] = -np.sin(th)
    return F


def twiddles(P, KX):
    F = dft_matrix(P)[:, :KX]
    return np.stack([F[0::2], F[1::2]], axis=-1).astype(np.float32)


def idft_matrix(P, OW):
# ... 9 lines not shown
    G[:, 0::2] = c * np.cos(th) / P
    G[:, 1::2] = -c * np.sin(th) / P
    return G


def freq_order(P):
    nu = n_freq(P)
    real = [0] + ([nu - 1] if P % 2 == 0 else [])
    cplx = [u for u in range(nu) if u not in real]
    return cplx, real


def n_planes(P):
    c, r = freq_order(P)
    return 3 * len(c) + len(r)


def matrices(P, KX):
    OW = P - KX + 1
    cplx, real = freq_order(P)
    F2, G2 = dft_matrix(P), idft_matrix(P, OW)
    Fr, Fi = F2[0::2], F2[1::2]
    Gr, Gi = G2[:, 0::2], G2[:, 1::2]
    Frows, Gcols = [], []
    for u in cplx:
        Frows += [Fr[u] + Fi[u], Fi[u], Fr[u]]
        Gcols += [Gr[:, u] + Gi[:, u], -Gr[:, u], -Gi[:, u]]
    for u in real:
        Frows.append(Fr[u])
        Gcols.append(Gr[:, u])
    F = np.stack(Frows, 0)
    G = np.stack(Gcols, 1)
    tw = twiddles(P, KX)[cplx + real]
    f32 = lambda a: np.ascontiguousarray(a, dtype=np.float32)
    return dict(F=f32(F), Ft=f32(F.T), G=f32(G), Gt=f32(G.T), tw=f32(tw))


def matrices_full(P, W, KX):
    assert W + KX - 1 == P
    m = matrices(P, 1)
    F = np.ascontiguousarray(m["F"][:, :W])
    cplx, real = freq_order(P)
    tw = twiddles(P, KX)[cplx + real].copy()
    tw[..., 1] = -tw[..., 1]
    return dict(F=F, Ft=np.ascontiguousarray(F.T), G=m["G"], Gt=m["Gt"], tw=np.ascontiguousarray(tw, dtype=np.float32))


def axis(R, I, O, C, in_sr, in_hi, in_lo, in_split, out_sr, out_hi, out_lo, out_split, act=0, act_c0=0, accum=0):
    return dict(R=R, I=I, O=O, C=C, in_split=in_split, out_split=out_split, act=act, act_c0=act_c0, accum=accum,
                in_sr=in_sr, in_hi=in_hi, in_lo=in_lo, out_sr=out_sr, out_hi=out_hi, out_lo=out_lo)


class Layout:

    def __init__(self, N, H, W, Ci, ldx, Co, ldy, KY, KX):
        self.N, self.H, self.W, self.Ci, self.ldx, self.Co, self.ldy, self.KY, self.KX = N, H, W, Ci, ldx, Co, ldy, KY, KX
        self.OH, self.OW = H - KY + 1, W - KX + 1
        self.nu = n_freq(W)
        self.Ur = len(freq_order(W)[1])
        self.G = n_planes(W)
        self.x_g = N * H * Ci
        self.t_g = N * self.OH * Co
        self.w_g = Co * KY * Ci

    def x_to_planes(self):
        return axis(self.N * self.H, self.W, self.G, self.Ci, self.W * self.ldx, self.ldx, 0, 1, self.Ci, self.x_g, 0, 1)

    def planes_to_y(self, act, act_c0):
        return axis(self.N * self.OH, self.G, self.OW, self.Co, self.Co, self.t_g, 0, 1, self.OW * self.ldy, self.ldy, 0, 1,
                    act=act, act_c0=act_c0)

    def dy_to_planes(self, lddy):
        return axis(self.N * self.OH, self.OW, self.G, self.Co, self.OW * lddy, lddy, 0, 1, self.Co, self.t_g, 0, 1)

    def planes_to_dx(self, lddx, accum):
        return axis(self.N * self.H, self.G, self.W, self.Ci, self.Ci, self.x_g, 0, 1, self.W * lddx, lddx, 0, 1, accum=int(accum))

    def conv(self):
        d = D.conv_fwd(self.G * self.N, (1, self.H, 1), self.Ci, self.Ci, self.Co, self.Co, (1, self.KY, 1), (1, 1, 1), (0, 0, 0),
                       (1, self.OH, 1), groups=self.G)
        d["wgstride"] = self.w_g
        return d

    def dgrad(self):
        out = D.transposed_classes(self.G * self.N, (1, self.OH, 1), self.Co, self.Co, (1, self.H, 1), self.Ci, self.Ci,
                                   (1, self.KY, 1), (1, 1, 1), (0, 0, 0), groups=self.G, ldw=self.Co, flags=capi.F_NFAST)
        for d in out:
            d["wgstride"] = self.w_g
        return out

    def wgrad(self):
        d = D.wgrad(self.N, (1, 1, self.OH), self.Co, self.Co, (1, 1, self.H), self.Ci, self.Ci, (1, 1, self.KY), (1, 1, 1), (0, 0, 0),
                    splitk=-1)
        d.update(nbatch=self.G, dbstride=self.t_g, sbstride=self.x_g, gbstride=self.w_g)
        return d

    def flops(self):
        return 2 * self.G * self.N * self.OH * self.Co * self.KY * self.Ci


class LayoutT:

    def __init__(self, N, H, W, Ci, ldx, Co, ldy, KY, KX):
        self.N, self.H, self.W, self.Ci, self.ldx, self.Co, self.ldy, self.KY, self.KX = N, H, W, Ci, ldx, Co, ldy, KY, KX
        self.OH, self.OW = H + KY - 1, W + KX - 1
        self.P = self.OW
        self.nu = n_freq(self.P)
        self.Ur = len(freq_order(self.P)[1])
        self.G = n_planes(self.P)
        self.x_g = N * H * Ci
        self.t_g = N * self.OH * Co
        self.w_g = Co * KY * Ci

    def matrices(self):
        return matrices_full(self.P, self.W, self.KX)

    def x_to_planes(self):
        return axis(self.N * self.H, self.W, self.G, self.Ci, self.W * self.ldx, self.ldx, 0, 1, self.Ci, self.x_g, 0, 1)

    def planes_to_y(self, act, act_c0):
        return axis(self.N * self.OH, self.G, self.OW, self.Co, self.Co, self.t_g, 0, 1, self.OW * self.ldy, self.ldy, 0, 1,
                    act=act, act_c0=act_c0)

    def dy_to_planes(self, lddy):
        return axis(self.N * self.OH, self.OW, self.G, self.Co, self.OW * lddy, lddy, 0, 1, self.Co, self.t_g, 0, 1)

    def planes_to_dx(self, lddx, accum):
        return axis(self.N * self.H, self.G, self.W, self.Ci, self.Ci, self.x_g, 0, 1, self.W * lddx, lddx, 0, 1, accum=int(accum))

    def convT(self):
        out = D.transposed_classes(self.G * self.N, (1, self.H, 1), self.Ci, self.Ci, (1, self.OH, 1), self.Co, self.Co,
                                   (1, self.KY, 1), (1, 1, 1), (0, 0, 0), groups=self.G, flags=capi.F_NFAST)
        for d in out:
            d["wgstride"] = self.w_g
        return out

    def dgrad(self):
        d = D.conv_fwd(self.G * self.N, (1, self.OH, 1), self.Co, self.Co, self.Ci, self.Ci, (1, self.KY, 1), (1, 1, 1), (0, 0, 0),
                       (1, self.H, 1), groups=self.G, ldw=self.Co)
        d["wgstride"] = self.w_g
        return d

    def wgrad(self):
        d = D.wgrad(self.N, (1, 1, self.H), self.Ci, self.Ci, (1, 1, self.OH), self.Co, self.Co, (1, 1, self.KY), (1, 1, 1), (0, 0, 0),
                    splitk=-1)
        d.update(nbatch=self.G, dbstride=self.x_g, sbstride=self.t_g, gbstride=self.w_g)
        return d

    def flops(self):
        return 2 * self.G * self.N * self.H * self.Co * self.KY * self.Ci


def conv_transpose_fwd_bwd(x, w, bias, dy):
    import torch
    from . import ops
    dev = x.device
    N, H, W, Ci = x.shape
    _, Co, KY, KX = w.shape
    L = LayoutT(N, H, W, Ci, Ci, Co, Co, KY, KX)
    m = {k: torch.from_numpy(v).to(dev) for k, v in L.matrices().items()}
    wf = w.reshape(Ci, Co, KY * KX).permute(1, 2, 0).contiguous()
    wt = w.reshape(Ci, Co, KY * KX).permute(0, 2, 1).contiguous()
    f32 = dict(device=dev, dtype=torch.float32)
    xp = torch.empty(L.G * L.x_g, **f32)
    ops.axis_linear(L.x_to_planes(), x, m["F"], xp)
    wv = torch.empty(L.G * L.w_g, **f32)
    ops.wspec_fwd(wf, m["tw"], Co, Ci, KY, KX, L.nu, L.Ur, wv)
    tp = torch.zeros(L.G * L.t_g, **f32)
    for dd in L.convT():
# ... 54 lines not shown
```

Before: 429.1.

## Read forward weight planes K-major in spectral dgrad and batch Winograd weight transforms

Adds a K-major B-tile mode to the bf16-split conv kernel. It loads weight planes with transposed LDS reads (ds_read_tr16), so the spectral primary-caps input-gradient can reuse the forward weight planes. This drops the separately built transposed plane buffer along with its master-plane writes and memory. Separately, per-layer Winograd weight-transform launches in the prep list are merged into a single multi-job kernel to cut launch count. The cost is a new kernel template variant with different LDS access patterns, restricted to three tile shapes and Co%8==0.

```diff
diff --git a/include/picons.h b/include/picons.h
--- a/include/picons.h
+++ b/include/picons.h
@@ -26,8 +26,9 @@
 
 #define PC_F_STRIPS  256
 #define PC_F_X6      128
-
-#define PC_VERSION 103
+#define PC_F_BKMAJOR 512
+
+#define PC_VERSION 104
 int         pc_version(void);
 const char* pc_last_error(void);
 
@@ -79,6 +80,12 @@
 int pc_wino_conv(const pc_wino_desc* d, const float* in, const float* U, const float* bias, float* out, float* bnpart, pc_stream s);
 int64_t pc_wino4_u_floats(int O, int I, int KT);
 int pc_wino4_weights(const float* w, int64_t sO, int64_t sT, int64_t sI, int O, int I, int KT, int flip, float* U, pc_stream s);
+typedef struct pc_wino_weights_job {
+    uint64_t w, U;
+    int64_t  sO, sT, sI;
+    int32_t  O, I, KT, flip, m, reserved;
+} pc_wino_weights_job;
+int pc_wino_weights_multi(const pc_wino_weights_job* jobs, int njobs, pc_stream s);
 int pc_wino_bnpart_rows(const pc_wino_desc* d);
 int pc_wino_work(const pc_wino_desc* d, double* out);
 int pc_wino_variant(const pc_wino_desc* d, const float* out, char* buf, int cap);
@@ -287,6 +294,7 @@
     PC_OP_WSPEC_MASTER_PLANES,
     PC_OP_BN_FIN_APPLY,
     PC_OP_WGRAD_FOLD,
+    PC_OP_WINO_WEIGHTS_MULTI,
     PC_OP__COUNT
 };
 #define PC_MAX_LANES 8
diff --git a/pi-consistency-activity-detection_amd/capi.py b/pi-consistency-activity-detection_amd/capi.py
--- a/pi-consistency-activity-detection_amd/capi.py
+++ b/pi-consistency-activity-detection_amd/capi.py
@@ -53,7 +53,7 @@
  OP_ACT_BWD, OP_TO_NDHWC, OP_TO_NCDHW, OP_TRANSPOSE, OP_FILL, OP_AXPY, OP_EM_FWD, OP_EM_BWD, OP_CMASK_FWD, OP_CMASK_BWD,
  OP_TAPSUM_FWD, OP_TAPSUM_BWD, OP_LOSS, OP_SPREAD, OP_ADAM, OP_TAIL_COMBINE, OP_TAIL_COLSUM, OP_TAIL_GRADS, OP_COL2IM,
  OP_AXIS, OP_WSPEC_FWD, OP_WSPEC_BWD, OP_WSPEC_MASTER_FWD, OP_WSPEC_MASTER_BWD, OP_TAIL6_WEIGHTS, OP_TAIL6_GATHER, OP_TAIL6_SCATTER, OP_TAIL6_WGRAD_MAP, OP_TAIL6_BIAS_SUMS,
- OP_TRANSPOSE_MULTI, OP_FORK, OP_JOIN, OP_WGRAD_MULTI, OP_WINO_CONV, OP_WINO_WEIGHTS, OP_CONV_X6, OP_SPLIT_PLANES, OP_SPLIT_PLANES_MULTI, OP_WSPEC_MASTER_PLANES, OP_BN_FIN_APPLY, OP_WGRAD_FOLD) = range(1, 51)
+ OP_TRANSPOSE_MULTI, OP_FORK, OP_JOIN, OP_WGRAD_MULTI, OP_WINO_CONV, OP_WINO_WEIGHTS, OP_CONV_X6, OP_SPLIT_PLANES, OP_SPLIT_PLANES_MULTI, OP_WSPEC_MASTER_PLANES, OP_BN_FIN_APPLY, OP_WGRAD_FOLD, OP_WINO_WEIGHTS_MULTI) = range(1, 52)
 MAX_LANES = 8
 
 WJOB_DTYPE = np.dtype([("d", np.int32, 42), ("D", np.uint64), ("S", np.uint64), ("g", np.uint64)], align=False)
@@ -64,11 +64,15 @@
 
 SJOB_DTYPE = np.dtype([("src", np.uint64), ("planes", np.uint64), ("n", np.int64), ("pstride", np.int64)], align=False)
 
+WWJOB_DTYPE = np.dtype([("w", np.uint64), ("U", np.uint64), ("sO", np.int64), ("sT", np.int64), ("sI", np.int64), ("O", np.int32), ("I", np.int32),
+                        ("KT", np.int32), ("flip", np.int32), ("m", np.int32), ("reserved", np.int32)], align=False)
+
 ACT_NONE, ACT_RELU, ACT_SIGMOID = 0, 1, 2
 F_ACCUM, F_BIAS, F_CSCALE, F_BNPART, F_NFAST, F_TOUT, F_CI3, F_X6, F_STRIPS = 1, 2, 4, 8, 16, 32, 64, 128, 256
+F_BKMAJOR = 512
 WG_CS3, WG_X6 = 1, 2
 
-ABI_VERSION = 103
+ABI_VERSION = 104
 
 _SIGS = {
     "pc_version": (i32, []),
@@ -94,6 +98,7 @@
     "pc_wgrad_work": (i32, [C.POINTER(WgradDesc), i32, i32, C.POINTER(C.c_double)]),
     "pc_wino_u_floats": (i64, [i32, i32, i32]),
     "pc_wino_weights": (i32, [vp, i64, i64, i64, i32, i32, i32, i32, vp, vp]),
+    "pc_wino_weights_multi": (i32, [vp, i32, vp]),
     "pc_wino_conv": (i32, [C.POINTER(WinoDesc), vp, vp, vp, vp, vp, vp]),
     "pc_wino4_u_floats": (i64, [i32, i32, i32]),
     "pc_wino4_weights": (i32, [vp, i64, i64, i64, i32, i32, i32, i32, vp, vp]),
@@ -189,7 +194,7 @@
             raise RuntimeError("libpicons.so is ABI version %d, this package mirrors include/picons.h version %d: rebuild it "
                                "(`make -C pi-consistency-activity-detection_amd/csrc`)" % (L.pc_version(), ABI_VERSION))
         assert C.sizeof(ConvDesc) == 48 * 4 and OP_DTYPE.itemsize == 4 + 192 + 32 + 4 + 96 + 32
-        assert C.sizeof(WgradDesc) == 168 and WJOB_DTYPE.itemsize == 192
+        assert C.sizeof(WgradDesc) == 168 and WJOB_DTYPE.itemsize == 192 and WWJOB_DTYPE.itemsize == 64
         _lib = L
     return _lib
 
@@ -205,5 +210,9 @@
     return buf.value.decode()
 
 
+def variant_ok(name, desc, *args):
+    return getattr(lib(), name)(desc, *args, C.create_string_buffer(160), 160) == 0
+
+
 def call(name, *args):
     check(getattr(lib(), name)(*args))
diff --git a/pi-consistency-activity-detection_amd/csrc/api.hip b/pi-consistency-activity-detection_amd/csrc/api.hip
--- a/pi-consistency-activity-detection_amd/csrc/api.hip
+++ b/pi-consistency-activity-detection_amd/csrc/api.hip
@@ -167,6 +167,8 @@
         case PC_OP_WINO_WEIGHTS:
             if (op.i[4] == 4) return pc_wino4_weights(P(const float*, 0), op.l[0], op.l[1], op.l[2], op.i[0], op.i[1], op.i[2], op.i[3], P(float*, 1), s);
             return pc_wino_weights(P(const float*, 0), op.l[0], op.l[1], op.l[2], op.i[0], op.i[1], op.i[2], op.i[3], P(float*, 1), s);
+        case PC_OP_WINO_WEIGHTS_MULTI:
+            return pc_wino_weights_multi(P(const pc_wino_weights_job*, 0), op.i[0], s);
         default:
             pc_set_error("pc_run_ops: unknown op kind %d", op.kind);
             return PC_E_ARG;
diff --git a/pi-consistency-activity-detection_amd/csrc/conv_x6.hip b/pi-consistency-activity-detection_amd/csrc/conv_x6.hip
--- a/pi-consistency-activity-detection_amd/csrc/conv_x6.hip
+++ b/pi-consistency-activity-detection_amd/csrc/conv_x6.hip
@@ -7,6 +7,7 @@
 
 typedef __attribute__((ext_vector_type(8))) __bf16 bf16x8;
 typedef __attribute__((ext_vector_type(4))) uint32_t u32x4;
+typedef __attribute__((ext_vector_type(4))) short v4s16;
 
 __device__ __forceinline__ void split2(float x0, float x1, uint32_t& h, uint32_t& m, uint32_t& l) { x6_split2(x0, x1, h, m, l); }
 
@@ -51,7 +52,7 @@
 
 #define PC_MFX6(X, Y, Cc) Cc = __builtin_amdgcn_mfma_f32_32x32x16_bf16(__builtin_bit_cast(bf16x8, X), __builtin_bit_cast(bf16x8, Y), Cc, 0, 0, 0)
 
-template <int BM, int BN, int WM, int WN>
+template <int BM, int BN, int WM, int WN, bool KM = false>
 __global__ __launch_bounds__(64 * WM * WN, 1) void conv_x6_kernel(const ConvX6 px) {
     const ConvK& p = px.k;
     constexpr int NW = WM * WN, NT = 64 * NW;
@@ -67,6 +68,9 @@
     extern __shared__ __attribute__((aligned(16))) uint8_t smem8[];
     uint8_t* As0 = smem8;
     uint8_t* Bs0 = smem8 + 2 * ABYTES;
+    constexpr int RB = 2 * BN;
+    static_assert(!KM || BN == 64 || BN == 128, "K-major B tiles: 128- or 256-byte rows");
+    auto km_swz = [](int k) { return BN == 128 ? (k & 3) << 2 : ((k >> 1) & 1) << 2; };
     int* rinfo = (int*)(smem8 + OPBYTES);
     int* rout = rinfo + BM * 4;
     unsigned* tile_or = (unsigned*)(rout + BM);
@@ -130,9 +134,14 @@
 #pragma unroll
     for (int j = 0; j < BR; ++j) {
         const int pc = wave + NW * j, pl = pc / (BN / 16), q = pc % (BN / 16);
-        const int row = q * 16 + (lane >> 2), co = n0 + row;
-        const int sl = (lane & 3) ^ ((row >> 2) & 3);
-        bdma[j] = (pc < BPIECES && co < p.Co) ? (unsigned)(((size_t)pl * px.wpstride + (size_t)co * p.wtaps * p.ldw + sl * 8) * 2) : DMA_OOB;
+        if constexpr (KM) {
+            const int k = q * (1024 / RB) + lane / (BN / 8), co = n0 + ((lane % (BN / 8)) ^ km_swz(k)) * 8;
+            bdma[j] = (pc < BPIECES && co < p.Co) ? (unsigned)(((size_t)pl * px.wpstride + (size_t)k * p.wtaps * p.ldw + co) * 2) : DMA_OOB;
+        } else {
+            const int row = q * 16 + (lane >> 2), co = n0 + row;
+            const int sl = (lane & 3) ^ ((row >> 2) & 3);
+            bdma[j] = (pc < BPIECES && co < p.Co) ? (unsigned)(((size_t)pl * px.wpstride + (size_t)co * p.wtaps * p.ldw + sl * 8) * 2) : DMA_OOB;
+        }
     }
     {
         unsigned mo = 0;
@@ -172,7 +181,7 @@
     };
     auto fetchB = [&](int buf) {
         const int wtap = ((p.wk0[0] + wb.a * p.wkstep[0]) * p.KH + p.wk0[1] + wb.b * p.wkstep[1]) * p.KW + p.wk0[2] + wb.c * p.wkstep[2];
-        const dma_rsrc_t rb = dma_rsrc_h(wbase + (long long)wtap * p.ldw + wb.ci);
+        const dma_rsrc_t rb = dma_rsrc_h(wbase + (KM ? ((long long)wb.ci * p.wtaps + wtap) * p.ldw : (long long)wtap * p.ldw + wb.ci));
 #pragma unroll
         for (int j = 0; j < BR; ++j)
             if (BPIECES % NW == 0 || wave + NW * j < BPIECES) glds16h(rb, bdma[j], Bs0 + buf * BBYTES + (wave + NW * j) * 1024);
@@ -195,8 +204,14 @@
     }
 #pragma unroll
     for (int j = 0; j < TN; ++j) {
-        const int r = wn * (BN / WN) + (lane & 31) + j * 32;
-        bbas[j] = (unsigned)(2 * ABYTES) + (unsigned)(r * 64) + (unsigned)((kh ^ ((r >> 2) & 3)) << 4);
+        if constexpr (KM) {
+            const int gq = lane >> 4, q = (lane >> 2) & 3, pp = lane & 3;
+            const int k = 8 * (gq >> 1) + q, ch = (wn * (BN / WN) + j * 32 + 16 * (gq & 1)) / 8 + (pp >> 1);
+            bbas[j] = (unsigned)(2 * ABYTES) + (unsigned)(k * RB) + (unsigned)((ch ^ km_swz(k)) << 4) + (unsigned)((pp & 1) << 3);
+        } else {
+            const int r = wn * (BN / WN) + (lane & 31) + j * 32;
+            bbas[j] = (unsigned)(2 * ABYTES) + (unsigned)(r * 64) + (unsigned)((kh ^ ((r >> 2) & 3)) << 4);
+        }
     }
     f32x4 raw[2];
     u32x4 pa[2][3], pb[TN][3], pbl[2][3];
@@ -204,7 +219,16 @@
         raw[half] = *(const f32x4*)(smem8 + ((abase ^ (unsigned)(s * 64) ^ (unsigned)(half * 16)) + (unsigned)(buf * ABYTES)));
     };
     auto ldB = [&](int j, int pl, int s, int buf) {
-        return *(const u32x4*)(smem8 + ((bbas[j] ^ (unsigned)(s * 32)) + (unsigned)(buf * BBYTES + pl * BPLANE)));
+        if constexpr (KM) {
+            typedef __attribute__((address_space(3))) v4s16* lp_t;
+            const unsigned a = bbas[j] + (unsigned)(buf * BBYTES + pl * BPLANE + s * 16 * RB);
+            const uint2 lo = __builtin_bit_cast(uint2, __builtin_amdgcn_ds_read_tr16_b64_v4i16((lp_t)(smem8 + a)));
+            const uint2 hi = __builtin_bit_cast(uint2, __builtin_amdgcn_ds_read_tr16_b64_v4i16((lp_t)(smem8 + a + 4 * RB)));
+            u32x4 r;
+            r[0] = lo.x; r[1] = lo.y; r[2] = hi.x; r[3] = hi.y;
+            return r;
+        } else
+            return *(const u32x4*)(smem8 + ((bbas[j] ^ (unsigned)(s * 32)) + (unsigned)(buf * BBYTES + pl * BPLANE)));
     };
     auto unit = [&](int q, int set) {
         float x0 = raw[q >> 1][(q & 1) * 2], x1 = raw[q >> 1][(q & 1) * 2 + 1];
@@ -359,11 +383,11 @@
     return mtiles_g <= 8 && mtiles_g > 1 && (long long)K * bn * 6 >= (2ll << 20);
 }
 
-template <int BM, int BN, int WM, int WN>
+template <int BM, int BN, int WM, int WN, bool KM = false>
 int launch_x6(const ConvX6& kx, hipStream_t s) {
     constexpr int OPBYTES = 2 * (BM * BK * 4 + 3 * BN * BK * 2);
     const size_t lds = (size_t)OPBYTES + (size_t)(BM * 5 + 4) * sizeof(int);
-    PC_SET_LDS_ONCE((conv_x6_kernel<BM, BN, WM, WN>), lds, "conv_x6_kernel");
+    PC_SET_LDS_ONCE((conv_x6_kernel<BM, BN, WM, WN, KM>), lds, "conv_x6_kernel");
     ConvX6 p = kx;
     p.k.mtiles_g = cdiv(p.k.Mg, BM);
     p.k.ntiles = cdiv(p.k.Co, BN);
@@ -371,8 +395,8 @@
     if (p.ksplit <= 1 || p.rem <= 0 || !p.ws) { p.full = tiles; p.rem = 0; p.ksplit = 1; }
     p.mfast = x6_mfast(p.k.mtiles_g, p.k.K, BN);
     const dim3 grid(p.full + p.rem * p.ksplit), block(64 * WM * WN);
-    if (pc_tl_ev_start) hipExtLaunchKernelGGL((conv_x6_kernel<BM, BN, WM, WN>), grid, block, lds, s, pc_tl_ev_start, pc_tl_ev_stop, 0, p);
-    else hipLaunchKernelGGL((conv_x6_kernel<BM, BN, WM, WN>), grid, block, lds, s, p);
+    if (pc_tl_ev_start) hipExtLaunchKernelGGL((conv_x6_kernel<BM, BN, WM, WN, KM>), grid, block, lds, s, pc_tl_ev_start, pc_tl_ev_stop, 0, p);
+    else hipLaunchKernelGGL((conv_x6_kernel<BM, BN, WM, WN, KM>), grid, block, lds, s, p);
     PC_CHECK_LAUNCH("conv_x6_kernel");
     return PC_OK;
 }
@@ -398,6 +422,13 @@
     return r;
 }
 
+inline bool x6_bkmajor_tile(const X6Tile& t) { return (t.bm == 64 && t.bn == 128) || (t.bm == 128 && t.bn == 64) || (t.bm == 64 && t.bn == 64); }
+inline int x6_bkmajor_check(const pc_conv_desc* d, const X6Tile& t, const char* who) {
+    PC_CHECK_ARG(d->Co % 8 == 0 && d->ldw >= d->Co, "%s: PC_F_BKMAJOR needs Co %% 8 == 0 and ldw >= Co (Co=%d ldw=%d)", who, d->Co, d->ldw);
+    PC_CHECK_ARG(x6_bkmajor_tile(t), "%s: PC_F_BKMAJOR is not built for the %d x %d tile this descriptor takes (64 x 128, 128 x 64, 64 x 64 are)", who, t.bm, t.bn);
+    return PC_OK;
+}
+
 inline bool x6_splits(const X6Split& sp, bool have_ws) { return have_ws && sp.ksplit > 1; }
 
 }
@@ -483,6 +514,7 @@
     PC_CHECK_ARG(pc_x6_eligible(d), "pc_conv_variant: the descriptor does not take the bf16-split kernel (Ci=%d ldi=%d ldw=%d flags=%d)", d->Ci, d->ldi, d->ldw, d->flags);
     const int groups = d->groups > 0 ? d->groups : 1;
     const X6Tile c = pc_x6_tile(d, groups);
+    if (d->flags & PC_F_BKMAJOR) { const int rc = x6_bkmajor_check(d, c, "pc_conv_variant"); if (rc != PC_OK) return rc; }
     const X6Split sp = x6_split(d, groups, c);
     const bool split = x6_splits(sp, ws_floats > 0);
     PC_CHECK_ARG(!split || ws_floats >= sp.ws_floats, "pc_conv_variant: the workspace holds %lld floats, this launch needs %lld (pc_conv_x6_ws_floats)",
@@ -514,6 +546,9 @@
                  "pc_conv_fwd_x6: channel-major output (PC_F_TOUT) is for plain launches only");
     PC_CHECK_ARG(((uintptr_t)in % 16 == 0) && ((uintptr_t)wplanes % 16 == 0) && plane_stride % 8 == 0 && d->wgstride % 8 == 0,
                  "pc_conv_fwd_x6: in / wplanes must be 16-byte aligned, plane and group strides multiples of 8 elements");
+    const bool km = (d->flags & PC_F_BKMAJOR) != 0;
+    const X6Tile c = pc_x6_tile(d, groups);
+    if (km) { const int rc = x6_bkmajor_check(d, c, "pc_conv_fwd_x6"); if (rc != PC_OK) return rc; }
     ConvX6 kx;
     ConvK& k = kx.k;
     kx.wp = wplanes; kx.wpstride = plane_stride;
@@ -533,11 +568,10 @@
     {
         const long long halo = ((long long)(k.ioff0[0] < 0 ? -k.ioff0[0] : 0) * k.Hi + (k.ioff0[1] < 0 ? -k.ioff0[1] : 0)) * k.Wi + (k.ioff0[2] < 0 ? -k.ioff0[2] : 0);
         const long long in_bytes = ((long long)k.N * k.Ti * k.Hi * k.Wi + 2 * halo) * k.ldi * 4;
-        const long long w_bytes = (2 * plane_stride + (long long)k.Co * k.wtaps * k.ldw) * 2;
+        const long long w_bytes = (2 * plane_stride + (long long)(km ? k.Ci : k.Co) * k.wtaps * k.ldw) * 2;
         PC_CHECK_ARG(in_bytes < DMA_MAX_BYTES && w_bytes < DMA_MAX_BYTES,
                      "pc_conv_fwd_x6: input (%lld B) or weight planes (%lld B per group) exceed the 4 GiB the LDS-DMA gather addresses", in_bytes, w_bytes);
     }
-    const X6Tile c = pc_x6_tile(d, groups);
     const X6Split sp = x6_split(d, groups, c);
     kx.full = sp.tiles; kx.rem = 0; kx.ksplit = 1; kx.ws = nullptr; kx.ctr = nullptr;
     if (x6_splits(sp, ws != nullptr)) {
@@ -546,6 +580,11 @@
         kx.full = sp.full; kx.rem = sp.rem; kx.ksplit = sp.ksplit; kx.ws = ws;
         kx.ctr = (unsigned*)(ws + (long long)sp.rem * sp.ksplit * c.bm * c.bn);
     }
+    if (km) {
+        if (c.bm == 64 && c.bn == 128) return launch_x6<64, 128, 2, 2, true>(kx, (hipStream_t)s);
+        if (c.bm == 128) return launch_x6<128, 64, 4, 1, true>(kx, (hipStream_t)s);
+        return launch_x6<64, 64, 2, 2, true>(kx, (hipStream_t)s);
+    }
     if (c.bm == 256) return launch_x6<256, 128, 8, 1>(kx, (hipStream_t)s);
     if (c.bm == 128 && c.bn == 64) return launch_x6<128, 64, 4, 1>(kx, (hipStream_t)s);
     if (c.bm == 128 && c.bn == 32) return launch_x6<128, 32, 4, 1>(kx, (hipStream_t)s);
diff --git a/pi-consistency-activity-detection_amd/csrc/wino.hip b/pi-consistency-activity-detection_amd/csrc/wino.hip
--- a/pi-consistency-activity-detection_amd/csrc/wino.hip
+++ b/pi-consistency-activity-detection_amd/csrc/wino.hip
@@ -1,4 +1,5 @@
 #include "common.h"
+#include "wino_wt.h"
 #include <stdlib.h>
 #include <type_traits>
 
@@ -36,37 +37,8 @@
 __global__ void wino_weights_kernel(const float* __restrict__ w, long long sO, long long sT, long long sI, int O, int I, int KT, int flip,
                                     float* __restrict__ U, int nct, int nc8) {
     const long long e = (long long)blockIdx.x * blockDim.x + threadIdx.x;
-    const long long total = (long long)KT * nct * 64 * I;
-    if (e >= total) return;
-    const int i = (int)(e % I);
-    long long r = e / I;
-    const int o = (int)(r % (nct * 64));
-    const int kt = (int)(r / (nct * 64));
-    float g[3][3];
-#pragma unroll
-    for (int a = 0; a < 3; ++a)
-#pragma unroll
-        for (int b = 0; b < 3; ++b) {
-            const int ks = flip ? KT - 1 - kt : kt, as = flip ? 2 - a : a, bs = flip ? 2 - b : b;
-            g[a][b] = o < O ? w[(long long)o * sO + (long long)((ks * 3 + as) * 3 + bs) * sT + (long long)i * sI] : 0.f;
-        }
-    float t[4][3];
-#pragma unroll
-    for (int b = 0; b < 3; ++b) {
-        t[0][b] = g[0][b];
-        t[1][b] = 0.5f * (g[0][b] + g[1][b] + g[2][b]);
-        t[2][b] = 0.5f * (g[0][b] - g[1][b] + g[2][b]);
-        t[3][b] = g[2][b];
-    }
-    float* dst = U + ((((long long)kt * nct + o / 64) * nc8 + i / 8) * 16) * (2 * 64 * 4) + ((long long)((i & 7) >> 2) * 64 + (o & 63)) * 4 + (i & 3);
-#pragma unroll
-    for (int x = 0; x < 4; ++x) {
-        const float u0 = t[x][0], u1 = 0.5f * (t[x][0] + t[x][1] + t[x][2]), u2 = 0.5f * (t[x][0] - t[x][1] + t[x][2]), u3 = t[x][2];
-        dst[(x * 4 + 0) * (2 * 64 * 4)] = u0;
-        dst[(x * 4 + 1) * (2 * 64 * 4)] = u1;
-        dst[(x * 4 + 2) * (2 * 64 * 4)] = u2;
-        dst[(x * 4 + 3) * (2 * 64 * 4)] = u3;
-    }
+    if (e >= (long long)KT * nct * 64 * I) return;
+    wino2_weights_elem(e, w, sO, sT, sI, O, I, KT, flip, U, nct, nc8);
 }
 
 constexpr int RMAX = 12;
diff --git a/pi-consistency-activity-detection_amd/csrc/wino4.hip b/pi-consistency-activity-detection_amd/csrc/wino4.hip
--- a/pi-consistency-activity-detection_amd/csrc/wino4.hip
+++ b/pi-consistency-activity-detection_amd/csrc/wino4.hip
@@ -1,4 +1,5 @@
 #include "common.h"
+#include "wino_wt.h"
 #include <stdlib.h>
 #include <type_traits>
 
@@ -46,11 +47,8 @@
 constexpr int RPIECES = 12;
 constexpr int RPLANE = RPIECES * 256;
 
-__global__ void wino4_weights_kernel(const float* __restrict__ w, long long sO, long long sT, long long sI, int O, int I, int KT, int flip,
-                                     float* __restrict__ U, int nct, int nc4) {
-    const long long e = (long long)blockIdx.x * blockDim.x + threadIdx.x;
-    const long long total = (long long)KT * nct * 64 * I;
-    if (e >= total) return;
+__device__ __forceinline__ void wino4_weights_elem(long long e, const float* __restrict__ w, long long sO, long long sT, long long sI, int O, int I, int KT, int flip,
+                                                   float* __restrict__ U, int nct, int nc4) {
     const int i = (int)(e % I);
     long long r = e / I;
     const int o = (int)(r % (nct * 64));
@@ -93,6 +91,26 @@
             dst[(P >> 1) * (2 * 64 * 4) + (P & 1) * 2] = (float)u[nu];
         }
     }
+}
+
+__global__ void wino4_weights_kernel(const float* __restrict__ w, long long sO, long long sT, long long sI, int O, int I, int KT, int flip,
+                                     float* __restrict__ U, int nct, int nc4) {
+    const long long e = (long long)blockIdx.x * blockDim.x + threadIdx.x;
+    if (e >= (long long)KT * nct * 64 * I) return;
+    wino4_weights_elem(e, w, sO, sT, sI, O, I, KT, flip, U, nct, nc4);
+}
+
+constexpr int WW_JOBS = 32;
+struct WinoWJobK { const float* w; float* U; long long sO, sT, sI; int O, I, KT, flip, m, nct, ncc; };
+struct WinoWPack { WinoWJobK j[WW_JOBS]; int first[WW_JOBS + 1]; int n; };
+__global__ __launch_bounds__(256) void wino_weights_multi_kernel(const WinoWPack pk) {
+    int k = 0;
+    while (k + 1 < pk.n && (int)blockIdx.x >= pk.first[k + 1]) ++k;
+    const WinoWJobK& J = pk.j[k];
+    const long long e = (long long)((int)blockIdx.x - pk.first[k]) * 256 + threadIdx.x;
+    if (e >= (long long)J.KT * J.nct * 64 * J.I) return;
+    if (J.m == 4) wino4_weights_elem(e, J.w, J.sO, J.sT, J.sI, J.O, J.I, J.KT, J.flip, J.U, J.nct, J.ncc);
+    else wino2_weights_elem(e, J.w, J.sO, J.sT, J.sI, J.O, J.I, J.KT, J.flip, J.U, J.nct, J.ncc);
 }
 
 template <int VAR>
@@ -538,6 +556,31 @@
     return PC_OK;
 }
 
+extern "C" int pc_wino_weights_multi(const pc_wino_weights_job* jobs, int njobs, pc_stream s) {
+    PC_CHECK_ARG(jobs && njobs >= 1, "pc_wino_weights_multi: bad args");
+    for (int j0 = 0; j0 < njobs; j0 += WW_JOBS) {
+        WinoWPack pk;
+        pk.n = njobs - j0 < WW_JOBS ? njobs - j0 : WW_JOBS;
+        long long blocks = 0;
+        for (int q = 0; q < pk.n; ++q) {
+            const pc_wino_weights_job& a = jobs[j0 + q];
+            PC_CHECK_ARG(a.w && a.U && a.O >= 1 && a.I >= 8 && a.I % 8 == 0 && (a.KT == 1 || a.KT == 3) && (a.m == 0 || a.m == 2 || a.m == 4) && (a.flip == 0 || a.flip == 1),
+                         "pc_wino_weights_multi: bad job %d (O=%d I=%d KT=%d m=%d flip=%d)", j0 + q, a.O, a.I, a.KT, a.m, a.flip);
+            WinoWJobK& J = pk.j[q];
+            J.w = (const float*)(uintptr_t)a.w; J.U = (float*)(uintptr_t)a.U; J.sO = a.sO; J.sT = a.sT; J.sI = a.sI;
+            J.O = a.O; J.I = a.I; J.KT = a.KT; J.flip = a.flip; J.m = a.m == 4 ? 4 : 2;
+            J.nct = cdiv(a.O, 64); J.ncc = J.m == 4 ? a.I / XK : a.I / 8;
+            pk.first[q] = (int)blocks;
+            blocks += ((long long)a.KT * J.nct * 64 * a.I + 255) / 256;
+            PC_CHECK_ARG(blocks < (1ll << 31), "pc_wino_weights_multi: too many elements");
+        }
+        pk.first[pk.n] = (int)blocks;
+        hipLaunchKernelGGL(wino_weights_multi_kernel, dim3((unsigned)blocks), dim3(256), 0, (hipStream_t)s, pk);
+        PC_CHECK_LAUNCH("wino_weights_multi_kernel");
+    }
+    return PC_OK;
+}
+
 int pc_wino4_bnpart_rows_impl(const pc_wino_desc* d) {
     Wino4K k;
     if (fill(d, k) != PC_OK) return -1;
diff --git a/pi-consistency-activity-detection_amd/csrc/wino_wt.h b/pi-consistency-activity-detection_amd/csrc/wino_wt.h
--- /dev/null
+++ b/pi-consistency-activity-detection_amd/csrc/wino_wt.h
@@ -0,0 +1,39 @@
+#pragma once
+#include "common.h"
+
+namespace {
+
+__device__ __forceinline__ void wino2_weights_elem(long long e, const float* __restrict__ w, long long sO, long long sT, long long sI, int O, int I, int KT, int flip,
+                                                   float* __restrict__ U, int nct, int nc8) {
+    const int i = (int)(e % I);
+    long long r = e / I;
+    const int o = (int)(r % (nct * 64));
+    const int kt = (int)(r / (nct * 64));
+    float g[3][3];
+#pragma unroll
+    for (int a = 0; a < 3; ++a)
+#pragma unroll
+        for (int b = 0; b < 3; ++b) {
+            const int ks = flip ? KT - 1 - kt : kt, as = flip ? 2 - a : a, bs = flip ? 2 - b : b;
+            g[a][b] = o < O ? w[(long long)o * sO + (long long)((ks * 3 + as) * 3 + bs) * sT + (long long)i * sI] : 0.f;
+        }
+    float t[4][3];
+#pragma unroll
+    for (int b = 0; b < 3; ++b) {
+        t[0][b] = g[0][b];
+        t[1][b] = 0.5f * (g[0][b] + g[1][b] + g[2][b]);
+        t[2][b] = 0.5f * (g[0][b] - g[1][b] + g[2][b]);
+        t[3][b] = g[2][b];
+    }
+    float* dst = U + ((((long long)kt * nct + o / 64) * nc8 + i / 8) * 16) * (2 * 64 * 4) + ((long long)((i & 7) >> 2) * 64 + (o & 63)) * 4 + (i & 3);
+#pragma unroll
+    for (int x = 0; x < 4; ++x) {
+        const float u0 = t[x][0], u1 = 0.5f * (t[x][0] + t[x][1] + t[x][2]), u2 = 0.5f * (t[x][0] - t[x][1] + t[x][2]), u3 = t[x][2];
+        dst[(x * 4 + 0) * (2 * 64 * 4)] = u0;
+        dst[(x * 4 + 1) * (2 * 64 * 4)] = u1;
+        dst[(x * 4 + 2) * (2 * 64 * 4)] = u2;
+        dst[(x * 4 + 3) * (2 * 64 * 4)] = u3;
+    }
+}
+
+}
diff --git a/pi-consistency-activity-detection_amd/ops.py b/pi-consistency-activity-detection_amd/ops.py
--- a/pi-consistency-activity-detection_amd/ops.py
+++ b/pi-consistency-activity-detection_amd/ops.py
@@ -80,6 +80,13 @@
     U = out if out is not None else torch.empty(n, device=w.device, dtype=torch.float32)
     capi.call(fam + "_weights", ptr(w), int(sO), int(sT), int(sI), O, I, KT, int(flip), ptr(U), stream())
     return U
+
+
+def wino_weights_multi(jobs):
+    tab = np.zeros(len(jobs), dtype=capi.WWJOB_DTYPE)
+    for q, (w, U, st, O, I, KT, flip, m) in enumerate(jobs):
+        tab[q] = (w.data_ptr(), U.data_ptr(), st[0], st[1], st[2], O, I, KT, int(flip), m, 0)
+    capi.call("pc_wino_weights_multi", C.c_void_p(tab.ctypes.data), len(jobs), stream())
 
 
 def wino_conv(d, x, U, out, bias=None, bnpart=None):
diff --git a/pi-consistency-activity-detection_amd/plan.py b/pi-consistency-activity-detection_amd/plan.py
--- a/pi-consistency-activity-detection_amd/plan.py
+++ b/pi-consistency-activity-detection_amd/plan.py
@@ -920,6 +920,7 @@
         npose = spec.IN_CAPS * spec.POSE
         caps_in = self.tensor(N, (1, s20, s20), npose + spec.IN_CAPS, "caps_in")
         spectral_pc = self.spectral_pc and xd.thw[0] == 1
+        pc_dgrad_wv = False
         Cpc = npose + spec.IN_CAPS
         pc_names = [("primary_caps.pose.weight", 0, npose), ("primary_caps.a.weight", npose, spec.IN_CAPS)]
         if spectral_pc:
@@ -929,10 +930,15 @@
             nW = SL.G * SL.w_g
             x6_pc = self.x6 and sw.get("PICONS_SPLIT_SPECTRAL", "1") != "0" and all(capi.lib().pc_conv_x6_ok(_cdesc(dict(D.trim_conv(dd), flags=dd["flags"] | capi.F_X6))) for dd in [SL.conv()] + SL.dgrad())
             if x6_pc:
-                wpc = dict(wv=("V", 0), wvt=("V", 4 * nW))
-                pf, pt = self.alloc((3 * nW + 1) // 2), self.alloc((3 * nW + 1) // 2)
+                pc_dgrad_wv = sw.get("PICONS_PC_DGRAD_WV", "1") != "0" and all(
+                    capi.variant_ok("pc_conv_variant", _cdesc(dict(D.trim_conv(dd), flags=dd["flags"] | capi.F_X6)), 0)
+                    for dd in SL.dgrad(fwd_planes=True))
+                wpc = dict(wv=("V", 0), wvt=("V", 0 if pc_dgrad_wv else 4 * nW))
+                pf = self.alloc((3 * nW + 1) // 2)
+                pt = None if pc_dgrad_wv else self.alloc((3 * nW + 1) // 2)
                 self.wbufs.append(dict(ref=wpc["wv"], n=nW, lst=None, lane=None, planes=pf))
-                self.wbufs.append(dict(ref=wpc["wvt"], n=nW, lst=None, lane=None, planes=pt))
+                if pt is not None:
+                    self.wbufs.append(dict(ref=wpc["wvt"], n=nW, lst=None, lane=None, planes=pt))
                 for nm, a0, cnt in pc_names:
                     self.emit(capi.OP_WSPEC_MASTER_PLANES, i=[cnt, a0, Cpc, xd.C, KP, KP, SL.nu, SL.Ur], l=[nW], p=[self.P(nm), sm["tw"], pf, pt],
                               lst=self.prep_target, lane=pl)
@@ -1010,7 +1016,7 @@
             if spectral_pc:
                 dxpl = self.alloc(SL.G * SL.x_g)
                 self.alg_dgrad(SL.flops())
-                for dd in SL.dgrad():
+                for dd in SL.dgrad(fwd_planes=pc_dgrad_wv):
                     self.conv_op(dd, dtpl, wpc["wvt"], dxpl, alg=0)
                 self.emit(capi.OP_AXIS, i=D.flatten(SL.planes_to_dx(dx.ld, acc), capi.AXIS_FIELDS), p=[dxpl, sm["Ft"], None, dx.ref])
             elif xd.thw[0] == 1 and caps_in.thw[1] + KP - 1 == xd.thw[1]:
@@ -1367,7 +1373,7 @@
         return tab
 
     def _merge_prep_transposes(self, lst, bases, keep):
-        res, pending, splits = [], {}, {}
+        res, pending, splits, winos = [], {}, {}, {}
 
         def flush():
             for lane in sorted(pending):
@@ -1376,6 +1382,13 @@
                 keep.append(tab)
                 res.append((capi.OP_TRANSPOSE_MULTI, [len(jobs)], [], [("HOST", tab.ctypes.data)], [], lane))
             pending.clear()
+            for lane in sorted(winos):
+                tab = np.zeros(len(winos[lane]), dtype=capi.WWJOB_DTYPE)
+                for q, (_k, i, _f, p, l, _lane) in enumerate(winos[lane]):
+                    tab[q] = (bases[p[0][0]] + p[0][1], bases[p[1][0]] + p[1][1], l[0], l[1], l[2], i[0], i[1], i[2], i[3], i[4], 0)
+                keep.append(tab)
+                res.append((capi.OP_WINO_WEIGHTS_MULTI, [len(tab)], [], [("HOST", tab.ctypes.data)], [], lane))
+            winos.clear()
             for lane in sorted(splits):
                 res.append((capi.OP_SPLIT_PLANES_MULTI, [len(splits[lane])], [], [("SJOBS", splits[lane])], [], lane))
             splits.clear()
@@ -1384,6 +1397,8 @@
                 splits.setdefault(op[5], []).append((op[3][0], op[3][1], op[4][0], op[4][1]))
             elif op[0] == capi.OP_TRANSPOSE and op[3][0][0] == "P":
                 pending.setdefault(op[5], []).append(op)
+            elif op[0] == capi.OP_WINO_WEIGHTS and op[3][0][0] == "P":
+                winos.setdefault(op[5], []).append(op)
             elif op[0] in (capi.OP_FILL, capi.OP_FORK, capi.OP_WSPEC_MASTER_FWD, capi.OP_WSPEC_MASTER_PLANES, capi.OP_WINO_WEIGHTS):
                 res.append(op)
             else:
diff --git a/pi-consistency-activity-detection_amd/spectral.py b/pi-consistency-activity-detection_amd/spectral.py
--- a/pi-consistency-activity-detection_amd/spectral.py
+++ b/pi-consistency-activity-detection_amd/spectral.py
@@ -115,9 +115,10 @@
         d["wgstride"] = self.w_g
         return d
 
-    def dgrad(self):
+    def dgrad(self, fwd_planes=False):
         out = D.transposed_classes(self.G * self.N, (1, self.OH, 1), self.Co, self.Co, (1, self.H, 1), self.Ci, self.Ci,
-                                   (1, self.KY, 1), (1, 1, 1), (0, 0, 0), groups=self.G, ldw=self.Co, flags=capi.F_NFAST)
+                                   (1, self.KY, 1), (1, 1, 1), (0, 0, 0), groups=self.G, ldw=self.Ci if fwd_planes else self.Co,
+                                   flags=capi.F_NFAST | (capi.F_BKMAJOR if fwd_planes else 0))
         for d in out:
             d["wgstride"] = self.w_g
         return out
```

Result: faster. 437.2 (median of 6 runs) (+1.9%).
